# BEAMRobotics/beam_slam

Hardware: AMD Instinct MI355X
Metric: LM iterations/sec + ms/graph-solve, 200KF x 50k-landmark VIO window (higher is better)
Workload: dtype f64; 1 GPU; C2: 200-keyframe x 50000-landmark VIO window; n_obs=400690, n_imu_factors=199, solver_options=vio.yaml:7-17 (<= 10 iterations, tolerances 1.5e-7), max_solver_time lifted, parallelism=single GPU, n_ranks_seen=1

## Files before the change

beam_slam_amd/capi.py:

```python
import ctypes as C

import numpy as np

OK = 0
ERR_INVALID, ERR_DEVICE, ERR_UNSUPPORTED, ERR_NUMERIC = -1, -2, -3, -4

MANIFOLD_EUCLIDEAN, MANIFOLD_QUAT_RIGHT = 0, 1
LOSS_TRIVIAL, LOSS_CAUCHY, LOSS_HUBER = 0, 1, 2

F_REPROJ = 0
F_REPROJ_ONLINE_CALIB = 1
F_IMU_DELTA = 2
F_IMU_PRIOR = 3
F_RELPOSE_EXT = 4
F_RELPOSE = 5
F_ABSPOSE = 6
F_ABS_VEC3 = 7
F_REL_VEC3 = 8
F_GRAVITY = 9
F_IDP_REPROJ = 10
F_IDP_REPROJ_UNARY = 11
F_UNICYCLE = 12
F_NUM_TYPES = 13

LINEAR_AUTO, LINEAR_SCHUR_CHOLESKY, LINEAR_PCG, LINEAR_SCHUR_PCG = 0, 1, 2, 3
TR_LEVENBERG_MARQUARDT, TR_DOGLEG, TR_SUBSPACE_DOGLEG = 0, 1, 2
CONVERGENCE, NO_CONVERGENCE, FAILURE = 0, 1, 2


class Options(C.Structure):
    _fields_ = [
        ("max_num_iterations", C.c_int32),
        ("linear_solver_type", C.c_int32),
        ("jacobi_scaling", C.c_int32),
        ("max_num_consecutive_invalid_steps", C.c_int32),
        ("max_solver_time_in_seconds", C.c_double),
        ("function_tolerance", C.c_double),
        ("gradient_tolerance", C.c_double),
        ("parameter_tolerance", C.c_double),
        ("initial_trust_region_radius", C.c_double),
        ("max_trust_region_radius", C.c_double),
        ("min_trust_region_radius", C.c_double),
        ("min_relative_decrease", C.c_double),
        ("min_lm_diagonal", C.c_double),
        ("max_lm_diagonal", C.c_double),
        ("pcg_max_iterations", C.c_int32),
        ("trust_region_strategy_type", C.c_int32),
        ("pcg_tolerance", C.c_double),
    ]


class Summary(C.Structure):
    _fields_ = [
        ("termination_type", C.c_int32),
        ("is_solution_usable", C.c_int32),
        ("num_iterations", C.c_int32),
        ("num_successful_steps", C.c_int32),
        ("num_unsuccessful_steps", C.c_int32),
        ("num_parameters_tangent", C.c_int32),
        ("num_residuals", C.c_int32),
        ("linear_solver_used", C.c_int32),
        ("num_linear_solves", C.c_int32),
        ("num_inner_iterations", C.c_int32),
        ("initial_cost", C.c_double),
        ("final_cost", C.c_double),
        ("fixed_cost", C.c_double),
        ("total_time_in_seconds", C.c_double),
        ("device_time_in_seconds", C.c_double),
        ("time_eval_seconds", C.c_double),
        ("time_assemble_seconds", C.c_double),
        ("time_linear_solve_seconds", C.c_double),
        ("message", C.c_char * 160),
    ]


class Iteration(C.Structure):
    _fields_ = [
        ("iteration", C.c_int32),
        ("step_is_valid", C.c_int32),
        ("step_is_successful", C.c_int32),
        ("reserved0", C.c_int32),
        ("cost", C.c_double),
        ("cost_change", C.c_double),
        ("gradient_max_norm", C.c_double),
        ("gradient_norm", C.c_double),
        ("step_norm", C.c_double),
        ("relative_decrease", C.c_double),
        ("trust_region_radius", C.c_double),
        ("model_cost_change", C.c_double),
    ]


class Camera(C.Structure):
    _fields_ = [
        ("fx", C.c_double), ("fy", C.c_double), ("cx", C.c_double), ("cy", C.c_double),
        ("R_cam_baselink", C.c_double * 9),
        ("t_cam_baselink", C.c_double * 3),
    ]


SYMBOLS = [
    "nidx", "nconst", "nres", "options_default", "options_vio", "create", "create_error", "destroy",
    "last_error", "abi_version", "clear", "set_blocks", "set_values", "set_cameras", "add_factors", "add_factors_indirect", "sync_factors_indirect",
    "add_marginal",
    "finalize", "solve", "get_blocks", "reset_values", "num_iterations_recorded", "get_iteration",
    "evaluate", "num_residuals", "num_parameters_tangent", "tangent_offset", "covariance", "marginalize", "get_marginal",
    "reprojection_errors", "preintegrate", "triangulate", "time_reproj_jacobian_ms", "reproj_jacobian_bytes", "dense_solve", "plan_info",
    "profile_step", "time_eval_ms", "eval_bytes", "bsr_info", "covariance_joint", "update_marginal", "solve_batch", "batch_stats", "set_plan_preference",
    "covariance_requests", "localize_frames", "num_factorizations", "essential_ransac", "absolute_pose_ransac",
    "relative_pose_ransac", "inertial_alignment", "register_scans", "register_scans_error",
]

_dp = C.POINTER(C.c_double)
_ip = C.POINTER(C.c_int32)
_bp = C.POINTER(C.c_uint8)

RANSAC_OK, RANSAC_TOO_FEW, RANSAC_NO_MODEL = 0, 1, 2
RANSAC_MAX_MATCHES = 65536
ESSENTIAL_RANSAC_ARGTYPES = [C.c_void_p, C.c_int32, _ip, _dp, _dp, _dp, C.c_double, C.c_double, C.c_int32, C.c_uint64, _bp, _dp, _ip, _ip,
                             _ip, _ip]
ABSOLUTE_POSE_RANSAC_ARGTYPES = [C.c_void_p, C.c_int32, _ip, _dp, _dp, _ip, C.c_double, C.c_double, C.c_int32, C.c_uint64, C.c_int32, _bp,
                                 _dp, _dp, _dp, _ip, _ip, _ip, _ip]
RELATIVE_POSE_RANSAC_ARGTYPES = [C.c_void_p, C.c_int32, _ip, _dp, _dp, _ip, C.c_double, C.c_double, C.c_int32, C.c_uint64, C.c_int32,
                                 C.c_double, C.c_double, _bp, _dp, _dp, _dp, _dp, _bp, _dp, _ip, _ip, _ip, _ip, _ip]
ALIGN_OK, ALIGN_TOO_FEW_FRAMES, ALIGN_BAD_IMU, ALIGN_NOT_EXCITED, ALIGN_RANK_DEFICIENT, ALIGN_SCALE_REJECTED = 0, 1, 2, 3, 4, 5
ALIGN_MIN_EXCITATION, ALIGN_SCALE_MIN, ALIGN_SCALE_MAX, ALIGN_RANK_TOL = 0.25, 0.02, 1.0, 1e-10
INERTIAL_ALIGNMENT_ARGTYPES = [C.c_int, C.c_int32, _ip, _dp, _dp, _dp, _ip, _dp, _dp, _dp, C.c_int32, C.c_double, C.c_int32, C.c_double,
                               C.c_double, C.c_double, _dp, _dp, _dp, _dp, _ip, _dp, _dp, _dp, _dp, _ip]
ICP_MAX_ITERATIONS, ICP_TRANSFORM, ICP_ABS_MSE, ICP_REL_MSE, ICP_TOO_FEW_CORRESPONDENCES = 1, 2, 3, 4, 5
ICP_MAX_CELLS, ICP_MAX_ITER = 1 << 22, 1000
ICP_DEFAULTS = dict(max_corr=1.0, max_iter=50, t_eps=1e-8, fit_eps=1e-2, rotation_threshold=0.99999, rel_mse_eps=1e-5)
REGISTER_SCANS_ARGTYPES = [C.c_int, C.c_int32, _ip, _dp, _ip, _dp, _dp, C.c_double, C.c_int32, C.c_double, C.c_double, C.c_double,
                           C.c_double, _dp, _dp, _dp, _ip, _ip, _ip]


def _ptr(a, typ):
    return None if a is None else a.ctypes.data_as(typ)


class SolverError(RuntimeError):
    def __init__(self, code, msg):
        super().__init__(f"[{code}] {msg}")
        self.code = code


class Solver:

    def __init__(self, lib, prefix, device=0):
        self._lib, self._p = lib, prefix
        f = self._f
        f("create").restype = C.c_void_p
        f("create").argtypes = [C.c_int]
        f("destroy").argtypes = [C.c_void_p]
        f("last_error").restype = C.c_char_p
        f("last_error").argtypes = [C.c_void_p]
        f("set_blocks").argtypes = [C.c_void_p, C.c_int32, _dp, _ip, _bp, _bp, _bp]
        f("set_values").argtypes = [C.c_void_p, _dp, C.c_int64]
        f("set_cameras").argtypes = [C.c_void_p, C.c_int32, C.POINTER(Camera)]
        f("add_factors").argtypes = [C.c_void_p, C.c_int32, C.c_int32, _ip, _dp, _ip, _dp]
        f("add_marginal").argtypes = [C.c_void_p, C.c_int32, _ip, C.c_int32, _dp, _dp, _dp]
        f("marginalize").argtypes = [C.c_void_p, C.c_int32, _ip, _ip, _ip, _ip]
        f("get_marginal").argtypes = [C.c_void_p, _ip, _dp, _dp, _dp]
        f("finalize").argtypes = [C.c_void_p]
        f("clear").argtypes = [C.c_void_p]
        f("solve").argtypes = [C.c_void_p, C.POINTER(Options), C.POINTER(Summary)]
        f("get_blocks").argtypes = [C.c_void_p, _dp, C.c_int64]
        f("reset_values").argtypes = [C.c_void_p]
        f("num_iterations_recorded").argtypes = [C.c_void_p]
        f("get_iteration").argtypes = [C.c_void_p, C.c_int32, C.POINTER(Iteration)]
        f("evaluate").argtypes = [C.c_void_p, _dp, _dp, _dp, _dp]
        f("num_residuals").argtypes = [C.c_void_p]
        f("num_parameters_tangent").argtypes = [C.c_void_p]
        f("tangent_offset").argtypes = [C.c_void_p, C.c_int32]
        f("covariance").argtypes = [C.c_void_p, C.c_int32, C.c_int32, _dp]
        f("options_default").argtypes = [C.POINTER(Options)]
        f("options_vio").argtypes = [C.POINTER(Options)]
        self._ctx = f("create")(device)
        if not self._ctx:
            why = ""
            try:
                ce = f("create_error")
                ce.restype = C.c_char_p
                why = ce().decode()
            except AttributeError:
                pass
            raise SolverError(ERR_DEVICE, f"{prefix}create({device}) failed: {why}")
        self._nvalues = 0

    def _f(self, name):
        return getattr(self._lib, self._p + name)

    def has(self, name):
        return hasattr(self._lib, self._p + name)

    def _chk(self, rc):
        if rc != OK:
            raise SolverError(rc, self._f("last_error")(self._ctx).decode())

    def close(self):
        if getattr(self, "_ctx", None):
            self._f("destroy")(self._ctx)
            self._ctx = None

    def __del__(self):
        try:
            self.close()
        except Exception:
            pass

    def options_default(self):
        o = Options()
        self._f("options_default")(C.byref(o))
        return o

    def options_vio(self):
        o = Options()
        self._f("options_vio")(C.byref(o))
        return o

    def clear(self):
        self._chk(self._f("clear")(self._ctx))

    def set_blocks(self, values, offset, size, manifold, is_const):
        values = np.ascontiguousarray(values, np.float64)
        offset = np.ascontiguousarray(offset, np.int32)
        size = np.ascontiguousarray(size, np.uint8)
        manifold = np.ascontiguousarray(manifold, np.uint8)
        is_const = np.ascontiguousarray(is_const, np.uint8)
        self._nvalues = values.size
        self._chk(self._f("set_blocks")(self._ctx, offset.size, _ptr(values, _dp), _ptr(offset, _ip),
                                        _ptr(size, _bp), _ptr(manifold, _bp), _ptr(is_const, _bp)))

    def set_values(self, values):
        values = np.ascontiguousarray(values, np.float64)
        self._chk(self._f("set_values")(self._ctx, _ptr(values, _dp), values.size))

    def set_cameras(self, cams):
        arr = (Camera * len(cams))(*cams)
        self._chk(self._f("set_cameras")(self._ctx, len(cams), arr))

    def add_factors(self, ftype, block_idx, consts, loss_kind=None, loss_a=None):
        block_idx = np.ascontiguousarray(block_idx, np.int32)
        consts = np.ascontiguousarray(consts, np.float64)
        n = block_idx.shape[0] if block_idx.ndim == 2 else 0
        if loss_kind is not None:
            loss_kind = np.ascontiguousarray(np.broadcast_to(loss_kind, (n,)), np.int32)
        if loss_a is not None:
            loss_a = np.ascontiguousarray(np.broadcast_to(loss_a, (n,)), np.float64)
        self._chk(self._f("add_factors")(self._ctx, ftype, n, _ptr(block_idx, _ip), _ptr(consts, _dp),
                                         _ptr(loss_kind, _ip), _ptr(loss_a, _dp)))

    def add_factors_indirect(self, ftype, slot_idx, slot_to_block, consts, loss_kind=None, loss_a=None):
        slot_idx = np.ascontiguousarray(slot_idx, np.int32)
        slot_to_block = np.ascontiguousarray(slot_to_block, np.int32)
        consts = np.ascontiguousarray(consts, np.float64)
        n = slot_idx.shape[0] if slot_idx.ndim == 2 else 0
        if loss_kind is not None:
            loss_kind = np.ascontiguousarray(np.broadcast_to(loss_kind, (n,)), np.int32)
        if loss_a is not None:
            loss_a = np.ascontiguousarray(np.broadcast_to(loss_a, (n,)), np.float64)
        fn = self._f("add_factors_indirect")
        fn.argtypes = [C.c_void_p, C.c_int32, C.c_int32, _ip, C.c_int32, _ip, _dp, _ip, _dp]
        fn.restype = C.c_int
# ... 173 lines not shown
```

beam_slam_amd/csrc/bsgpu_api.cpp:

```cpp
#include <thread>

#include "bsgpu_ctx.h"
#include "bsgpu_env.h"

using namespace bsg;

namespace bsg {
int api_exception(bsgpu_ctx* c) noexcept {
  int code = BSGPU_ERR_INVALID;
  const char* what = "unexpected exception";
  try { throw; }
  catch (const std::bad_alloc&) { code = BSGPU_ERR_DEVICE; what = "out of host memory"; }
  catch (const std::exception& e) { what = e.what(); try { if (c) c->err = std::string("internal error: ") + what; } catch (...) {} return code; }
  catch (...) {}
  try { if (c) c->err = what; } catch (...) {}
  return code;
}
thread_local std::string g_create_error;
int invalidate_keep_values(bsgpu_ctx* c) {
  if (c->finalized && c->d_x && !c->h_x.empty()) {
    HIPCHK(c, hipSetDevice(c->device));
    HIPCHK(c, hipStreamSynchronize(c->stream));
    HIPCHK(c, hipMemcpy(c->h_x.data(), c->d_x, sizeof(double) * c->h_x.size(), hipMemcpyDeviceToHost));
  }
// ... 754 lines not shown

constexpr size_t kCovRowsBudget = (size_t)1 << 30;
int bsgpu_covariance_requests(bsgpu_ctx* c, int32_t n_req, const int32_t* pairs, int64_t* offsets, double* out) try {
  if (!c) return BSGPU_ERR_INVALID;
  if (n_req < 0 || (n_req > 0 && !pairs)) return fail(c, BSGPU_ERR_INVALID, "covariance_requests: bad argument");
  if (n_req == 0) { if (offsets) offsets[0] = 0; return BSGPU_OK; }
  int rc = finalize(c);
  if (rc != BSGPU_OK) return rc;
  for (int i = 0; i < 2 * n_req; ++i) {
    const int b = pairs[i];
    if (b < 0 || b >= c->nb) return fail(c, BSGPU_ERR_INVALID, "covariance_requests: block out of range");
    if (c->toff[b] < 0) return fail(c, BSGPU_ERR_INVALID, "covariance_requests: constant block");
    if (c->calib.on && c->is_lm[b])
      return fail(c, BSGPU_ERR_UNSUPPORTED, "covariance_requests: an eliminated landmark of a window with a free extrinsic pair (online calibration): "
                                            "pose-side blocks only");
  }
  std::vector<int64_t> off(n_req + 1, 0);
  for (int i = 0; i < n_req; ++i) off[i + 1] = off[i] + (int64_t)c->tsize[pairs[2 * i]] * c->tsize[pairs[2 * i + 1]];
  if (offsets) std::memcpy(offsets, off.data(), sizeof(int64_t) * off.size());
  if (!out) return BSGPU_OK;
  if (!c->dense_ok) return fail(c, BSGPU_ERR_UNSUPPORTED, "covariance_requests: reduced system above the dense limit (block-sparse PCG path has no factor)");
  const int n_pose = c->n_pose;
  auto kind_of = [&](int b) { return c->toff[b] < n_pose ? kCovUnit : (c->is_lm[b] == 2 ? kCovIdp : kCovLandmark); };
  auto lm_of = [&](int b) { return kind_of(b) == kCovIdp ? c->toff[b] - c->idp.to0 : (c->toff[b] - n_pose) / 3; };
  std::map<int, int> row_of;
  std::vector<CovRow> rows;
  std::vector<int> pass_entry{0}, pass_row{0};
  int n_rows = 0, in_pass = 0;
  for (int i = 0; i < 2 * n_req; ++i) {
    const int b = pairs[i];
    if (row_of.count(b)) continue;
    const int ts = c->tsize[b];
    if (in_pass + ts > 64) { pass_entry.push_back((int)rows.size()); pass_row.push_back(n_rows); in_pass = 0; }
    row_of[b] = n_rows;
    const int k = kind_of(b);
    if (k == kCovUnit) for (int r = 0; r < ts; ++r) rows.push_back(CovRow{kCovUnit, c->plan.spos(c->toff[b] + r), in_pass + r, 0});
    else rows.push_back(CovRow{k, lm_of(b), in_pass, 0});
    n_rows += ts; in_pass += ts;
  }
  pass_entry.push_back((int)rows.size()); pass_row.push_back(n_rows);
  const int n_pass = (int)pass_entry.size() - 1;
  const int ldy = c->npad, n_cols = c->plan.T * 64;
  if ((size_t)n_rows * ldy * sizeof(double) > kCovRowsBudget)
    return fail(c, BSGPU_ERR_UNSUPPORTED, "covariance_requests: the kept rows (" + std::to_string(n_rows) + " x " + std::to_string(ldy) +
                " doubles) exceed the 1 GiB device-memory budget of one call; split the requests");
  std::vector<CovReq> req(n_req);
  for (int i = 0; i < n_req; ++i) {
    const int a = pairs[2 * i], b = pairs[2 * i + 1];
    const int ka = kind_of(a), kb = kind_of(b);
    CovReq& q = req[i];
    q.ra = row_of[a]; q.ta = c->tsize[a]; q.rb = row_of[b]; q.tb = c->tsize[b];
    q.sign = ((ka != kCovUnit) != (kb != kCovUnit)) ? -1 : 1;
    q.lm_kind = (a == b && ka != kCovUnit) ? ka : kCovUnit;
    q.lm_index = q.lm_kind != kCovUnit ? lm_of(a) : 0;
    q.pad = 0;
    q.out = off[i];
  }
  HIPCHK(c, hipSetDevice(c->device));
  hipStream_t s = c->stream;
  const size_t y_bytes = (size_t)n_rows * ldy * sizeof(double), o_bytes = ((size_t)off[n_req] * sizeof(double) + 255) & ~(size_t)255;
  const size_t q_bytes = (sizeof(CovReq) * req.size() + 255) & ~(size_t)255, r_bytes = sizeof(CovRow) * rows.size();
  unsigned char* buf = nullptr;
  if (hipMalloc((void**)&buf, y_bytes + o_bytes + q_bytes + r_bytes) != hipSuccess) { (void)hipGetLastError(); return fail(c, BSGPU_ERR_DEVICE, "covariance_requests: out of device memory"); }
  struct Free { unsigned char* p; ~Free() { (void)hipFree(p); } } free_buf{buf};
  double* d_Y = reinterpret_cast<double*>(buf);
  double* d_out = reinterpret_cast<double*>(buf + y_bytes);
  CovReq* d_req = reinterpret_cast<CovReq*>(buf + y_bytes + o_bytes);
  CovRow* d_rows = reinterpret_cast<CovRow*>(buf + y_bytes + o_bytes + q_bytes);
  HIPCHK(c, hipMemcpyAsync(d_req, req.data(), sizeof(CovReq) * req.size(), hipMemcpyHostToDevice, s));
  HIPCHK(c, hipMemcpyAsync(d_rows, rows.data(), r_bytes, hipMemcpyHostToDevice, s));
  bsgpu_options o;
  bsgpu_options_default(&o);
  const bool was_pcg = c->use_pcg;
  c->use_pcg = false;
  *c->h_radius = 1e300;
  (void)hipMemcpyAsync(c->d_scal + SC_RADIUS, c->h_radius, sizeof(double), hipMemcpyHostToDevice, s);
  eval_all(c, c->d_x, true, SC_COST_X);
  c->spec_J = false;
  bool singular = false;
  for (int p = 0; p < n_pass && rc == BSGPU_OK && !singular; ++p) {
    const int n_ent = pass_entry[p + 1] - pass_entry[p], r0 = pass_row[p], nr = pass_row[p + 1] - r0;
    assemble(c, o, 1e300, true, true);
    for (int attempt = 0; attempt < 2; ++attempt) {
      launch_cov_rows(s, c->d_S, c->npad, c->plan.rhs_row, d_rows + pass_entry[p], n_ent, c->d_dpos, c->vis, c->idp);
      DenseDev D0{c->d_nreal, c->d_rows_flat, c->d_panels, c->d_Lp, c->d_Vinv,
                  c->d_bs_desc, c->d_chain_begin, c->d_chain_end, c->d_tile_sync, c->d_ftasks, c->d_fsync};
      D0.Winv = c->d_Winv; D0.tile_tot = c->d_tile_tot; D0.rhs_rows = nr;
      D0.ftasks_plain = c->d_ftasks_plain; D0.tile_tot_plain = c->d_tile_tot_plain; D0.n_ftasks_plain = c->n_ftasks_plain;
      dense_factor(s, c->plan, D0, c->d_S, c->d_scal);
      (void)hipMemcpyAsync(d_Y + (size_t)r0 * ldy, c->d_Lp + (size_t)c->plan.rhs_row * ldy, sizeof(double) * nr * ldy, hipMemcpyDeviceToDevice, s);
      rc = fetch_scalars(c);
      if (rc != BSGPU_OK || !(c->h_scal[SC_CHOL_FAIL] == 2.0 && c->d_ftasks)) break;
      c->d_ftasks = nullptr;
      assemble(c, o, 1e300, true, true);
    }
    if (rc == BSGPU_OK && c->h_scal[SC_CHOL_FAIL] > 0.0) singular = true;
  }
  c->use_pcg = was_pcg;
  if (rc != BSGPU_OK) return rc;
  if (singular) return fail(c, BSGPU_ERR_NUMERIC, "covariance_requests: J^T J is singular at the current values (gauge freedom or unobserved block)");
  launch_cov_gram(s, d_req, n_req, d_Y, ldy, n_cols, c->vis.Linv, c->idp.linv, d_out);
  HIPCHK(c, hipMemcpyAsync(out, d_out, sizeof(double) * off[n_req], hipMemcpyDeviceToHost, s));
  HIPCHK(c, hipStreamSynchronize(s));
  for (int64_t i = 0; i < off[n_req]; ++i)
    if (!std::isfinite(out[i])) return fail(c, BSGPU_ERR_NUMERIC, "covariance_requests: J^T J is singular at the current values (gauge freedom or unobserved block)");
  return BSGPU_OK;
} catch (...) { return api_exception(c); }

int bsgpu_update_marginal(bsgpu_ctx* c, int32_t index, int32_t n_rows, int32_t n_cols, int32_t n_xbar, const double* A, const double* b,
                          const double* xbar) try {
  if (!c) return BSGPU_ERR_INVALID;
  if (index < 0 || index >= (int)c->marginals.size() || !A || !b || !xbar) return fail(c, BSGPU_ERR_INVALID, "update_marginal: bad argument");
  HostMarginal& mg = c->marginals[index];
  if (n_rows != mg.rows || (size_t)n_rows * (size_t)std::max(0, n_cols) != mg.A.size() || (size_t)n_rows != mg.b.size() || (size_t)n_xbar != mg.xbar.size())
    return fail(c, BSGPU_ERR_INVALID, "update_marginal: the payload's shape is not that of the prior as it was added");
  std::memcpy(mg.A.data(), A, sizeof(double) * mg.A.size());
  std::memcpy(mg.b.data(), b, sizeof(double) * mg.b.size());
  std::memcpy(mg.xbar.data(), xbar, sizeof(double) * mg.xbar.size());
  if (!c->finalized) return BSGPU_OK;
  if (index >= (int)c->marg.size()) return fail(c, BSGPU_ERR_INVALID, "update_marginal: device table out of step");
  HIPCHK(c, hipSetDevice(c->device));
  const MargDev& d = c->marg[index].dev;
  HIPCHK(c, hipStreamSynchronize(c->stream));
  HIPCHK(c, hipMemcpy(const_cast<double*>(d.A), mg.A.data(), sizeof(double) * mg.A.size(), hipMemcpyHostToDevice));
  HIPCHK(c, hipMemcpy(const_cast<double*>(d.b), mg.b.data(), sizeof(double) * mg.b.size(), hipMemcpyHostToDevice));
  HIPCHK(c, hipMemcpy(const_cast<double*>(d.xbar), mg.xbar.data(), sizeof(double) * mg.xbar.size(), hipMemcpyHostToDevice));
  c->spec_J = false;
  return BSGPU_OK;
} catch (...) { return api_exception(c); }

int bsgpu_reprojection_errors(bsgpu_ctx* c, double* err) try {
  if (!c) return BSGPU_ERR_INVALID;
  if (!err) return fail(c, BSGPU_ERR_INVALID, "null argument");
  int rc = finalize(c);
  if (rc != BSGPU_OK) return rc;
  HIPCHK(c, hipSetDevice(c->device));
  const Visual& V = c->vis;
  if ((rc = ensure_vis_src(c)) != BSGPU_OK) return rc;
  const SmallGroup& D = c->small[T_REPROJ_DENSE];
  const int n0 = c->groups[BSGPU_F_REPROJ].n;
  if (V.n + D.n == 0) return BSGPU_OK;
  double* d_out = nullptr;
  HIPCHK(c, hipMalloc((void**)&d_out, sizeof(double) * (size_t)(V.n + D.n)));
  if (c->calib.on) launch_calib_refresh(c->stream, c->calib, c->d_x, c->d_cams);
  launch_reproj_errors(c->stream, V, D, c->d_x, c->d_cams, d_out, d_out + V.n);
  std::vector<double> h((size_t)V.n + D.n);
  const hipError_t e = hipMemcpyAsync(h.data(), d_out, sizeof(double) * h.size(), hipMemcpyDeviceToHost, c->stream);
  const hipError_t e2 = hipStreamSynchronize(c->stream);
  (void)hipFree(d_out);
  if (e != hipSuccess || e2 != hipSuccess) return fail(c, BSGPU_ERR_DEVICE, "reprojection_errors: device error");
  auto slot = [&](int src) { const int t = src >> 28, f = src & ((1 << 28) - 1); return (t == BSGPU_F_REPROJ ? 0 : n0) + f; };
  for (int i = 0; i < V.n; ++i) err[slot(c->vis_src[i])] = h[i];
  for (int i = 0; i < D.n; ++i) err[slot(c->dense_src[i])] = h[(size_t)V.n + i];
  return BSGPU_OK;
} catch (...) { return api_exception(c); }

double bsgpu_time_reproj_jacobian_ms(bsgpu_ctx* c, int32_t reps) {
  if (!c) return -1.0;
  if (finalize(c) != BSGPU_OK || c->vis.n == 0 || reps <= 0) return -1.0;
  if (hipSetDevice(c->device) != hipSuccess) return -1.0;
  hipEvent_t e0, e1;
  if (hipEventCreate(&e0) != hipSuccess || hipEventCreate(&e1) != hipSuccess) return -1.0;
  launch_reproj_jacobian_only(c->stream, c->vis, c->d_x, c->d_cams, c->d_losses);
  (void)hipEventRecord(e0, c->stream);
  for (int i = 0; i < reps; ++i) launch_reproj_jacobian_only(c->stream, c->vis, c->d_x, c->d_cams, c->d_losses);
  (void)hipEventRecord(e1, c->stream);
  if (hipEventSynchronize(e1) != hipSuccess) return -1.0;
  float ms = 0.f;
  (void)hipEventElapsedTime(&ms, e0, e1);
  (void)hipEventDestroy(e0); (void)hipEventDestroy(e1);
  return (double)ms / reps;
}
double bsgpu_time_eval_ms(bsgpu_ctx* c, int32_t reps) {
  if (!c) return -1.0;
  if (finalize(c) != BSGPU_OK || reps <= 0) return -1.0;
  if (hipSetDevice(c->device) != hipSuccess) return -1.0;
  hipEvent_t e0, e1;
  if (hipEventCreate(&e0) != hipSuccess || hipEventCreate(&e1) != hipSuccess) return -1.0;
  eval_all(c, c->d_x, true, SC_COST_X);
  (void)hipEventRecord(e0, c->stream);
  for (int i = 0; i < reps; ++i) eval_all(c, c->d_x, true, SC_COST_X);
  (void)hipEventRecord(e1, c->stream);
  if (hipEventSynchronize(e1) != hipSuccess) return -1.0;
  float ms = 0.f;
  (void)hipEventElapsedTime(&ms, e0, e1);
  (void)hipEventDestroy(e0); (void)hipEventDestroy(e1);
  c->spec_J = false;
  return (double)ms / reps;
}
int64_t bsgpu_eval_bytes(const bsgpu_ctx* c) {
  if (!c) return -1;
  static const struct { int idx, consts, res, jcols; } L[BSGPU_F_NUM_TYPES] = {
      {4, 3, 2, 9}, {6, 3, 2, 9}, {10, 287, 15, 30}, {5, 241, 15, 15}, {6, 43, 6, 12}, {4, 43, 6, 12}, {2, 43, 6, 6}, {1, 12, 3, 3},
      {2, 12, 3, 6}, {1, 7, 2, 3}, {6, 6, 2, 13}, {4, 6, 2, 7}, {10, 226, 15, 30}};
  int64_t b = (int64_t)c->vis.n * (c->vis.ja == kJACompact ? 152 : 200) + (int64_t)c->h_x.size() * 8;
  for (int t = 2; t < BSGPU_F_NUM_TYPES && t < kNumInternal; ++t)
    b += (int64_t)c->small[t].n * (4 * L[t].idx + 8 * (L[t].consts + L[t].res + L[t].res * L[t].jcols));
  return b;
}
int bsgpu_bsr_info(bsgpu_ctx* c, int32_t* block_rows, int32_t* nnz_blocks) try {
  if (!c) return BSGPU_ERR_INVALID;
  const int rc = finalize(c);
  if (rc != BSGPU_OK) return rc;
  if (block_rows) *block_rows = c->use_pcg ? c->nbr : 0;
  if (nnz_blocks) *nnz_blocks = c->use_pcg ? c->nblk : 0;
  return BSGPU_OK;
} catch (...) { return api_exception(c); }
int bsgpu_profile_step(bsgpu_ctx* c, const bsgpu_options* o, int32_t reps, double* ms_out, double* work_out) try {
  if (!c) return BSGPU_ERR_INVALID;
  if (!o || !ms_out || reps <= 0) return fail(c, BSGPU_ERR_INVALID, "profile_step: bad argument");
  return profile_step(c, *o, reps, ms_out, work_out);
} catch (...) { return api_exception(c); }
int64_t bsgpu_reproj_jacobian_bytes(const bsgpu_ctx* c) {
  if (!c) return -1;
  return (int64_t)c->vis.n * (c->vis.ja == kJACompact ? 152 : 200) + (int64_t)c->h_x.size() * 8;
}

int bsgpu_dense_solve(int device, int32_t n, const double* A, const double* b, double* x, int32_t max_chains, double* ms_out) try {
  if (n <= 0 || !A || !b || !x) return BSGPU_ERR_INVALID;
  if (hipSetDevice(device) != hipSuccess) return BSGPU_ERR_DEVICE;
  chol_prepare();
  const int T = (n + 63) / 64;
  std::vector<uint8_t> adj((size_t)T * T, 0);
  for (int i = 0; i < n; ++i) for (int j = 0; j < n; ++j) if (A[(size_t)i * n + j] != 0.0) adj[(size_t)(i / 64) * T + j / 64] = 1;
  DensePlan P;
  P.build(n, adj, std::max(1, (int)max_chains), 1, env_shared());
  const int npad = P.npad;
  std::vector<double> hS((size_t)npad * npad, 0.0);
  for (int i = 0; i < n; ++i) for (int j = 0; j < n; ++j) hS[(size_t)P.spos(i) * npad + P.spos(j)] = A[(size_t)i * n + j];
  for (int j = 0; j < n; ++j) hS[(size_t)P.rhs_row * npad + P.spos(j)] = b[j];
  std::vector<uint8_t> real(npad, 0);
  for (int j = 0; j < n; ++j) real[P.spos(j)] = 1;
  for (int i = 0; i < npad; ++i) if (!real[i]) hS[(size_t)i * npad + i] = 1.0;
  double *dS = nullptr, *dLp = nullptr, *dV = nullptr, *dy = nullptr, *dscal = nullptr;
  int *dnreal = nullptr, *drows = nullptr;
  PanelDesc *dpan = nullptr, *dsep = nullptr;
  int *dpot2 = nullptr, *dcb = nullptr, *dce = nullptr, *dsync = nullptr, *dfsync = nullptr, *dtot = nullptr;
  double* dW = nullptr;
  FusedTask* dft = nullptr;
  const bool fused = env_chol_fused() && !P.ftasks.empty();
  hipStream_t s;
  if (hipStreamCreate(&s) != hipSuccess) return BSGPU_ERR_DEVICE;
  auto up = [](const void* src, size_t bytes, void** dst) {
    if (hipMalloc(dst, bytes ? bytes : 8) != hipSuccess) return false;
    return bytes == 0 || hipMemcpy(*dst, src, bytes, hipMemcpyHostToDevice) == hipSuccess;
  };
  bool ok = hipMalloc(&dS, sizeof(double) * hS.size()) == hipSuccess && hipMalloc(&dLp, sizeof(double) * hS.size()) == hipSuccess && hipMemset(dLp, 0, sizeof(double) * hS.size()) == hipSuccess &&
            hipMalloc(&dV, sizeof(double) * chol_vinv_stride() * std::max(1, T)) == hipSuccess && hipMalloc(&dy, sizeof(double) * npad) == hipSuccess &&
            hipMalloc(&dscal, sizeof(double) * SC_NUM) == hipSuccess;
  std::vector<int> rf = P.rows_flat; if (rf.empty()) rf.push_back(0);
  ok = ok && up(P.nreal.data(), sizeof(int) * P.nreal.size(), (void**)&dnreal) &&
       up(rf.data(), sizeof(int) * rf.size(), (void**)&drows) &&
       up(P.panels.data(), sizeof(PanelDesc) * P.panels.size(), (void**)&dpan) &&
       up(P.bs_desc.data(), sizeof(int) * P.bs_desc.size(), (void**)&dpot2) &&
       up(P.chain_begin.data(), sizeof(int) * P.chain_begin.size(), (void**)&dcb) && up(P.chain_end.data(), sizeof(int) * P.chain_end.size(), (void**)&dce) &&
       up(P.tile_sync.data(), sizeof(int) * P.tile_sync.size(), (void**)&dsync);
  if (ok && fused) {
    const std::vector<int> zeros((size_t)P.fused_sync_words, 0);
    ok = up(P.ftasks.data(), sizeof(FusedTask) * P.ftasks.size(), (void**)&dft) && up(zeros.data(), sizeof(int) * zeros.size(), (void**)&dfsync) &&
         up(P.tile_tot.data(), sizeof(int) * P.tile_tot.size(), (void**)&dtot) && hipMalloc((void**)&dW, sizeof(double) * 4096 * std::max(1, T)) == hipSuccess;
  }
  int rc = BSGPU_OK;
  int *dbc = nullptr, *drc = nullptr, *dbu = nullptr, *dbur = nullptr;
  if (ok) {
    (void)hipMemcpy(dS, hS.data(), sizeof(double) * hS.size(), hipMemcpyHostToDevice);
    (void)hipMemset(dscal, 0, sizeof(double) * SC_NUM);
    hipEvent_t e0, e1;
    (void)hipEventCreate(&e0); (void)hipEventCreate(&e1);
    (void)hipEventRecord(e0, s);
    DenseDev D{dnreal, drows, dpan, dLp, dV, dpot2, dcb, dce, dsync, dft, dfsync};
    D.Winv = dW; D.tile_tot = dtot;
    if (P.bs_level_sync && !env_backsolve_legacy() &&
        up(P.bs_desc_chain.data(), sizeof(int) * P.bs_desc_chain.size(), (void**)&dbc) && up(P.rows_flat_chain.data(), sizeof(int) * P.rows_flat_chain.size(), (void**)&drc) &&
        up(P.bs_upd.data(), sizeof(int) * P.bs_upd.size(), (void**)&dbu) && up(P.bs_upd_rows.data(), sizeof(int) * P.bs_upd_rows.size(), (void**)&dbur)) {
      D.bs_desc_chain = dbc; D.rows_flat_chain = drc; D.bs_upd = dbu; D.bs_upd_rows = dbur;
    }
    dense_factor_solve(s, P, D, dS, dy, dscal);
    (void)hipEventRecord(e1, s);
    if (hipEventSynchronize(e1) != hipSuccess || hipGetLastError() != hipSuccess) rc = BSGPU_ERR_DEVICE;
    float ms = 0.f;
    (void)hipEventElapsedTime(&ms, e0, e1);
    if (ms_out) *ms_out = ms;
    double hscal[SC_NUM];
    std::vector<double> hy(npad);
    (void)hipMemcpy(hscal, dscal, sizeof(hscal), hipMemcpyDeviceToHost);
    (void)hipMemcpy(hy.data(), dy, sizeof(double) * npad, hipMemcpyDeviceToHost);
    for (int j = 0; j < n; ++j) x[j] = hy[P.spos(j)];
    if (rc == BSGPU_OK && hscal[SC_CHOL_FAIL] > 0.0) rc = BSGPU_ERR_NUMERIC;
    (void)hipEventDestroy(e0); (void)hipEventDestroy(e1);
  } else rc = BSGPU_ERR_DEVICE;
  (void)hipFree(dS); (void)hipFree(dLp); (void)hipFree(dV); (void)hipFree(dy); (void)hipFree(dscal);
  (void)hipFree(dnreal); (void)hipFree(drows); (void)hipFree(dpan);
  (void)hipFree(dsep); (void)hipFree(dpot2); (void)hipFree(dcb); (void)hipFree(dce); (void)hipFree(dsync);
  (void)hipFree(dft); (void)hipFree(dfsync); (void)hipFree(dtot); (void)hipFree(dW);
  (void)hipFree(dbc); (void)hipFree(drc); (void)hipFree(dbu); (void)hipFree(dbur);
  (void)hipStreamDestroy(s);
  return rc;
} catch (...) { return api_exception(nullptr); }

int bsgpu_plan_info(const bsgpu_ctx* c, int32_t* n_chains, int32_t* n_steps, int32_t* n_tiles) try {
  if (!c) return BSGPU_ERR_INVALID;
  if (!c->finalized) return BSGPU_ERR_INVALID;
  if (n_chains) *n_chains = c->plan.n_pieces;
  if (n_steps) *n_steps = c->plan.n_steps();
  if (n_tiles) *n_tiles = c->plan.T;
  return BSGPU_OK;
// ... 12 lines not shown
```

beam_slam_amd/csrc/bsgpu_finalize.cpp:

```cpp
#include <atomic>

#include "bsgpu_ctx.h"
#include "bsgpu_env.h"
#include "band_plan.h"
#include "dim_order.h"

namespace bsg {

int band_part_forced() {
  return env_int("BSGPU_BAND_PART", 0);
}

namespace {
void eigen_quat_to_rot(const double* q, double* R) {
  const double tx = 2 * q[1], ty = 2 * q[2], tz = 2 * q[3];
  const double twx = tx * q[0], twy = ty * q[0], twz = tz * q[0], txx = tx * q[1], txy = ty * q[1], txz = tz * q[1];
  const double tyy = ty * q[2], tyz = tz * q[2], tzz = tz * q[3];
  R[0] = 1 - (tyy + tzz); R[1] = txy - twz; R[2] = txz + twy;
  R[3] = txy + twz; R[4] = 1 - (txx + tzz); R[5] = tyz - twx;
  R[6] = txz - twy; R[7] = tyz + twx; R[8] = 1 - (txx + tyy);
}

}

// ... 326 lines not shown
      lap("count pair entries");
      const int chunk = pair_chunk(n_ent);
      for (uint64_t key = 0; key < ncp * ncp; ++key)
        for (int p0 = start[key]; p0 < start[key + 1]; p0 += chunk) { seg_ci.push_back((int)(key / ncp)); seg_cj.push_back((int)(key % ncp)); seg_start.push_back(p0); }
      std::vector<int> pos(start.begin(), start.end() - 1);
      for (int l = 0; l < nl; ++l) {
        if (b_cmin[l] >= 0) continue;
        for (int a = lm_start[l]; a < lm_start[l + 1]; ++a) {
          const uint64_t ra = (uint64_t)cam_pose[a] * ncp;
          for (int b = lm_start[l]; b < lm_start[l + 1]; ++b)
            if (cam_pose[a] <= cam_pose[b]) { const int p = pos[ra + cam_pose[b]]++; ent_fa[p] = a; ent_fb[p] = b; }
        }
      }
      for (int f = n_elim; f < nv; ++f) { const int p = pos[(uint64_t)cam_pose[f] * ncp + cam_pose[f]]++; ent_fa[p] = f; ent_fb[p] = f; }
      lap("fill pair entries");
    } else {
      struct Ent { uint64_t key; int fa, fb; };
      std::vector<Ent> ents;
      ents.reserve((size_t)nv * 5);
      for (int l = 0; l < nl; ++l) {
        if (b_cmin[l] >= 0) continue;
        for (int a = lm_start[l]; a < lm_start[l + 1]; ++a)
          for (int b = lm_start[l]; b < lm_start[l + 1]; ++b)
            if (cam_pose[a] <= cam_pose[b]) ents.push_back({(uint64_t)cam_pose[a] * ncp + cam_pose[b], a, b});
      }
      for (int f = n_elim; f < nv; ++f) ents.push_back({(uint64_t)cam_pose[f] * ncp + cam_pose[f], f, f});
      std::stable_sort(ents.begin(), ents.end(), [](const Ent& x, const Ent& y) { return x.key < y.key; });
      ent_fa.resize(ents.size()); ent_fb.resize(ents.size());
      const int chunk = pair_chunk(ents.size());
      for (size_t i = 0; i < ents.size(); ++i) {
        if (i == 0 || ents[i].key != ents[i - 1].key || (int)i - seg_start.back() >= chunk) {
          seg_ci.push_back((int)(ents[i].key / ncp)); seg_cj.push_back((int)(ents[i].key % ncp)); seg_start.push_back((int)i);
        }
        ent_fa[i] = ents[i].fa; ent_fb[i] = ents[i].fb;
      }
      lap("sort pair entries");
    }
    seg_start.push_back((int)ent_fa.size());
    V.n_seg = (int)seg_ci.size(); V.n_ent = (int)ent_fa.size();
    V.n_seg_c = 0; V.seg_ci_c = V.seg_cj_c = V.seg_start_c = nullptr;
    lap("segments");
    V.fac = c->upload(fac); V.pix = c->upload(pix); V.w = c->upload(w);
    V.cam_pose = c->upload(cam_pose); V.lm_of = c->upload(lm_of); V.lm_start = c->upload(lm_start);
    V.cp_tq = c->upload(cp_tq); V.cp_tp = c->upload(cp_tp);
    V.seg_ci = c->upload(seg_ci); V.seg_cj = c->upload(seg_cj); V.seg_start = c->upload(seg_start);
    V.ent_fa = c->upload(ent_fa); V.ent_fb = c->upload(ent_fb);
    V.band_lm = c->upload(b_lm); V.band_unit_start = c->upload(bu.unit_start); V.band_unit_cam = c->upload(bu.unit_cam);
    V.band_lm_id = c->upload(bu.lm);
    const int T = (c->n_pose + 63) / 64;
    c->tile_adj.assign((size_t)T * T, 0);
    auto touch = [&](int ra, int rb) {
      if (ra < 0 || rb < 0) return;
      for (int a = ra; a < ra + 3; a += 2) for (int b = rb; b < rb + 3; b += 2) {
        c->tile_adj[(size_t)(a / 64) * T + b / 64] = 1; c->tile_adj[(size_t)(b / 64) * T + a / 64] = 1;
      }
      if (bg.nbk) bg.add(ra, rb);
    };
    for (int s = 0; s < V.n_seg; ++s) {
      const int i = seg_ci[s], j = seg_cj[s];
      const int ri[2] = {cp_tq[i], cp_tp[i]}, rj[2] = {cp_tq[j], cp_tp[j]};
      for (int a = 0; a < 2; ++a) for (int b = 0; b < 2; ++b) touch(ri[a], rj[b]);
    }
    for (int i = 0; i < V.n_cam_pose && V.n_band_lm > 0; ++i)
      for (int d = 0; d < kBandCams; ++d) {
        if (!((bu.adj[i] >> d) & 1u)) continue;
        const int j = i + d;
        const int ri[2] = {cp_tq[i], cp_tp[i]}, rj[2] = {cp_tq[j], cp_tp[j]};
        for (int a = 0; a < 2; ++a) for (int b = 0; b < 2; ++b) touch(ri[a], rj[b]);
      }
    if (has_calib) {
      Calib& cb = c->calib;
      cb.on = 1;
      cb.xq = c->off[calib_bq]; cb.xp = c->off[calib_bp];
      cb.tq = c->toff[calib_bq]; cb.tp = c->toff[calib_bp];
      cb.n_cam = (int)calib_cams.size();
      cb.cam_id = c->upload(calib_cams);
      std::vector<unsigned char> has(std::max(1, nv), 0);
      for (int i = 0; i < nv; ++i) has[i] = vf[i].calib ? 1 : 0;
      cb.has = c->upload(has);
      std::vector<int> cnt(k + 1, 0), by_cp(nv);
      for (int i = 0; i < nv; ++i) cnt[cam_pose[i] + 1]++;
      for (int i = 0; i < k; ++i) cnt[i + 1] += cnt[i];
      {
        std::vector<int> pos(cnt.begin(), cnt.end() - 1);
        for (int i = 0; i < nv; ++i) by_cp[pos[cam_pose[i]]++] = i;
      }
      std::vector<int> sg_cp, sg_start;
      for (int i = 0; i < k; ++i)
        for (int p0 = cnt[i]; p0 < cnt[i + 1]; p0 += 256) { sg_cp.push_back(i); sg_start.push_back(p0); }
      sg_start.push_back(nv);
      cb.n_seg = (int)sg_cp.size();
      cb.seg_cp = c->upload(sg_cp); cb.seg_start = c->upload(sg_start); cb.seg_fac = c->upload(by_cp);
      const int re[2] = {cb.tq, cb.tp};
      for (int a = 0; a < 2; ++a) {
        for (int b = 0; b < 2; ++b) touch(re[a], re[b]);
        for (int i = 0; i < k; ++i) { touch(cp_tq[i], re[a]); touch(cp_tp[i], re[a]); }
      }
    }
  }
    return BSGPU_OK;
  };
  bool flattened_on_device = false;
  {
    const bool force_dev = env_flatten_is("device"), force_host = env_flatten_is("host");
    const HostGroup& g0 = c->groups[BSGPU_F_REPROJ];
    SlotMirror& mir = c->mirror0;
    const bool resident = mir.active && !mir.materialized && mir.dev_valid;
    if (!force_host && c->groups[BSGPU_F_REPROJ_ONLINE_CALIB].n == 0 && g0.n > 0 && (force_dev || g0.n >= kDeviceFlattenMin)) {
      bool ok = true;
      if (mir.active && !mir.materialized && !resident) { const int rc_m = materialize_mirror(c); if (rc_m != BSGPU_OK) return rc_m; }
      if (resident) { for (const auto& u : mir.loss_use) if (u.rows > 0 && ok) { get_loss(u.kind, u.a); ok = losses.size() <= 8; } }
      else for (int f = 0; f < g0.n && ok; ++f) { get_loss(g0.loss_kind[f], g0.loss_a[f]); ok = losses.size() <= 8; }
      if (ok) {
        std::vector<int> bx(c->off.begin(), c->off.end());
        std::vector<unsigned char> bc(c->is_const.begin(), c->is_const.end());
        const int* d_bx = c->upload(bx); const int* d_bt = c->upload(c->toff);
        const unsigned char* d_bc = c->upload(bc); const int* d_bl = c->upload(lm_index);
        const int T = (c->n_pose + 63) / 64;
        bool all_const = false;
        FlattenSegsHost segs_host;
        auto dalloc = [&](size_t bytes) -> void* { return c->alloc<unsigned char>(bytes); };
        const FlattenResident res = {mir.d_idx, mir.d_consts, mir.d_lk, mir.d_la, mir.d_s2b};
        const int st = flatten_visual_device(c->stream, dalloc, g0.n, g0.idx.data(), g0.consts.data(), g0.loss_kind.data(), g0.loss_a.data(),
                                             losses, nb, d_bx, d_bt, d_bc, d_bl, nl, T, c->vis, &c->d_vis_src, c->tile_adj, &all_const,
                                             resident ? &res : nullptr, bg.nbk ? &segs_host : nullptr, band_on);
        if (st < 0) return fail(c, BSGPU_ERR_DEVICE, "device error while flattening the reprojection factors");
        if (st == 0) {
          flattened_on_device = true;
          if (bg.nbk)
            for (size_t sgi = 0; sgi < segs_host.seg_ci.size(); ++sgi) {
              const int i = segs_host.seg_ci[sgi], j = segs_host.seg_cj[sgi];
              const int ri[2] = {segs_host.cp_tq[i], segs_host.cp_tp[i]}, rj[2] = {segs_host.cp_tq[j], segs_host.cp_tp[j]};
              for (int a = 0; a < 2; ++a) for (int b = 0; b < 2; ++b) if (ri[a] >= 0 && rj[b] >= 0) bg.add(ri[a], rj[b]);
            }
          if (all_const) { c->any_inactive = true; c->vis_any_inactive = true; }
          if (c->vis.n_cam_pose >= (1 << 20)) return fail(c, BSGPU_ERR_UNSUPPORTED, "too many camera poses");
        } else {
          c->vis = Visual();
        }
      }
    }
  }
  if (flattened_on_device) lap("flatten on device");
  else { const int rc_host = host_visual(); if (rc_host != BSGPU_OK) return rc_host; }
  Visual& V = c->vis;
  {
    const int nv = V.n;
    V.r = c->alloc<double2>(nv); V.J = c->alloc<double>((size_t)nv * (kJAStride + 6)); V.JB = V.J ? V.J + (size_t)nv * kJAStride : nullptr; V.CR = c->alloc<double>((size_t)nv * 8);
    V.Linv = c->alloc<double>((size_t)std::max(1, nl) * kLmRec); V.z = V.Linv ? V.Linv + 6 : nullptr;
    V.n_cost_part = (nv + 255) / 256;
    V.cost_part = c->alloc<double>(V.n_cost_part);
    V.cost_part_cand = c->alloc<double>(V.n_cost_part);
    V.mcc_part = c->alloc<double>(std::max(1, backsub_mcc_groups(V)));
    if (!V.J || !V.CR || !V.r) return fail(c, BSGPU_ERR_DEVICE, "out of device memory (visual tables)");
    if (c->calib.on) {
      c->calib.E = c->alloc<double>((size_t)std::max(1, nv) * 12); c->calib.Et = c->alloc<double>((size_t)std::max(1, nv) * 12);
      c->calib.part = c->alloc<double>((size_t)std::max(1, calib_border_blocks(V)) * kCalibPartStride);
      if (!c->calib.E || !c->calib.Et || !c->calib.part) return fail(c, BSGPU_ERR_DEVICE, "out of device memory (extrinsic border tables)");
    }
    V.no_cr = !env_zero("BSGPU_NO_CR") && V.n_band_units > 0 && V.n_seg == 0 && V.n_ent == 0 && V.n == V.n_elim && V.band_lm_id != nullptr && V.Linv && V.z;
    V.ja = V.no_cr && !env_zero("BSGPU_COMPACT_J") ? kJACompact : kJAStride;
  }
  lap("visual upload + alloc");
  size_t part_max = std::max<size_t>(V.n_cost_part, 2 * ((size_t)nb + 255) / 256 + 2);
  int* d_toff_asm[kNumInternal] = {nullptr};
  for (int t = 2; t < kNumInternal; ++t) {
    const HostGroup& g = c->groups[t];
    const TypeInfo& ti = kTypes[t];
    SmallGroup& sg = c->small[t];
    sg = SmallGroup();
    sg.type = t; sg.n = g.n; sg.m = ti.m; sg.nv = ti.nvar; sg.nc = ti.nconst;
    sg.w_last = ti.amb[ti.nvar - 1] == 4 ? 3 : ti.amb[ti.nvar - 1];
    if (!g.n) continue;
    std::vector<int> xoff((size_t)g.n * ti.nvar), toff((size_t)g.n * ti.nvar), loss(g.n);
    std::vector<unsigned char> active(g.n, 0), inactive(g.n, 0);
    for (int f = 0; f < g.n; ++f) {
      const int32_t* idx = &g.idx[(size_t)f * ti.nidx];
      for (int sl = 0; sl < ti.nvar; ++sl) {
        xoff[(size_t)f * ti.nvar + sl] = c->off[idx[sl]];
        toff[(size_t)f * ti.nvar + sl] = c->toff[idx[sl]];
        if (c->toff[idx[sl]] >= c->n_pose && !(c->is_lm[idx[sl]] == 2 && sl == ti.nvar - 1 && (t == BSGPU_F_IDP_REPROJ || t == BSGPU_F_IDP_REPROJ_UNARY)))
          return fail(c, BSGPU_ERR_UNSUPPORTED, "internal: landmark in a pose-only factor");
        if (!c->is_const[idx[sl]]) active[f] = 1;
      }
      inactive[f] = !active[f];
      if (!active[f]) c->any_inactive = true;
      loss[f] = get_loss(g.loss_kind[f], g.loss_a[f]);
      if (active[f] && !skip_generic_assembly(t)) {
        const int T = (c->n_pose + 63) / 64;
        for (int sa = 0; sa < ti.nvar; ++sa)
          for (int sb = 0; sb < ti.nvar; ++sb) {
            const int ra = c->toff[idx[sa]], rb = c->toff[idx[sb]];
            if (ra < 0 || rb < 0 || ra >= c->n_pose || rb >= c->n_pose) continue;
            const int wa = c->tsize[idx[sa]], wb = c->tsize[idx[sb]];
            for (int a = ra; a < ra + wa; a += std::max(1, wa - 1)) for (int b = rb; b < rb + wb; b += std::max(1, wb - 1)) c->tile_adj[(size_t)(a / 64) * T + b / 64] = 1;
            if (bg.nbk && sb < sa) bg.add(ra, rb);
          }
      }
    }
    if (timing && g.n > 10000) lap("  group: per-factor loop");
    sg.xoff = c->upload(xoff); sg.toff = c->upload(toff); sg.consts = c->upload(g.consts); sg.loss = c->upload(loss);
    d_toff_asm[t] = nullptr;
    if (n_rho > 0 && (t == BSGPU_F_IDP_REPROJ || t == BSGPU_F_IDP_REPROJ_UNARY)) {
      std::vector<int> tm(toff);
      bool any = false;
      for (int& v : tm) if (v >= c->n_pose) { v = -1; any = true; }
      if (any) d_toff_asm[t] = c->upload(tm);
    }
    sg.active = c->upload(active);
    if (has_camera(t)) {
      std::vector<int> camv(g.n);
      for (int f = 0; f < g.n; ++f) camv[f] = g.idx[(size_t)f * ti.nidx + ti.nvar];
      sg.cam = c->upload(camv);
    }
    c->d_small_inactive[t] = c->upload(inactive);
    c->h_small_active[t] = active;
    if (timing && g.n > 10000) lap("  group: uploads");
    sg.r = c->alloc<double>((size_t)g.n * ti.m);
    sg.J = c->alloc<double>((size_t)g.n * ti.m * 3 * ti.nvar);
    c->d_small_part[t] = c->alloc<double>((size_t)g.n * ti.m);
    c->d_small_part_cand[t] = c->alloc<double>(g.n);
    c->d_small_part_mcc[t] = c->alloc<double>((size_t)g.n * ti.m);
    part_max = std::max(part_max, (size_t)g.n * ti.m);
    if (timing && g.n > 10000) lap("  group: allocations");
  }
  lap("pose-only group tables");
  {
    constexpr int kSegChunk = 64;
    struct Contrib { int ra, rb, tf, ss; };
    std::vector<Contrib> cl, tmp;
    std::vector<int> cnt;
    std::vector<AsmGroup> asm_grp;
    size_t asm_nfac = 0;
    auto sort_by_block = [&](size_t lo, size_t hi) {
      const size_t n = hi - lo;
      if (n < 2) return;
      tmp.resize(n);
      for (int pass = 0; pass < 2; ++pass) {
        cnt.assign((size_t)c->n_pose + 2, 0);
        for (size_t i = lo; i < hi; ++i) cnt[(pass == 0 ? cl[i].rb : cl[i].ra) + 1]++;
        for (size_t k = 1; k < cnt.size(); ++k) cnt[k] += cnt[k - 1];
        for (size_t i = lo; i < hi; ++i) tmp[cnt[pass == 0 ? cl[i].rb : cl[i].ra]++] = cl[i];
        std::copy(tmp.begin(), tmp.begin() + n, cl.begin() + lo);
      }
    };
    for (int t = 0; t < kNumInternal; ++t) {
      c->small_factorwise[t] = c->small[t];
      if (t < 2) c->small_factorwise[t].n = 0;
      if (d_toff_asm[t]) c->small_factorwise[t].toff = d_toff_asm[t];
      if (skip_generic_assembly(t)) c->small_factorwise[t].n = 0;
    }
    for (int t = 2; t < kNumInternal; ++t) {
      const SmallGroup& sg = c->small[t];
      if (!sg.n || skip_generic_assembly(t)) continue;
      const int nv = sg.nv;
      std::vector<int> toffs((size_t)sg.n * nv);
      HIPCHK(c, hipStreamSynchronize(c->stream));
      HIPCHK(c, hipMemcpy(toffs.data(), sg.toff, sizeof(int) * toffs.size(), hipMemcpyDeviceToHost));
      for (int& v : toffs) if (v >= c->n_pose) v = -1;
      std::vector<uint8_t> grouped(sg.n, 0);
      bool any_group = false;
      constexpr int kGroupMin = 4;
      if (sg.w_last == 3 && nv * 3 <= 18 && sg.m <= 6 && (sg.m * nv * 3) % 2 == 0 && sg.n >= 64 && !env_set("BSGPU_NO_GROUP_ASSEMBLY")) {
        std::vector<int> order;
        order.reserve(sg.n);
        for (int f = 0; f < sg.n; ++f) if (c->h_small_active[t][f]) order.push_back(f);
        auto key_less = [&](int a, int b) {
          const int* ka = &toffs[(size_t)a * nv]; const int* kb = &toffs[(size_t)b * nv];
          for (int i = 0; i < nv; ++i) if (ka[i] != kb[i]) return ka[i] < kb[i];
          return a < b;
        };
        std::sort(order.begin(), order.end(), key_less);
        for (size_t i = 0; i < order.size();) {
          size_t j = i + 1;
          while (j < order.size() && std::equal(&toffs[(size_t)order[i] * nv], &toffs[(size_t)order[i] * nv] + nv, &toffs[(size_t)order[j] * nv])) ++j;
          if ((int)(j - i) >= kGroupMin) {
            const size_t n_in = j - i, pieces = (n_in + kAsmGroupMax - 1) / kAsmGroupMax;
            size_t q0 = i;
            for (size_t pc = 0; pc < pieces; ++pc) {
              AsmGroup rec{};
              rec.type = t; rec.count = (int)(n_in / pieces + (pc < n_in % pieces ? 1 : 0)); rec.m = sg.m; rec.nv = nv;
              rec.te = 0;
              for (int sl = 0; sl < 6; ++sl) {
                rec.toff[sl] = sl < nv ? toffs[(size_t)order[i] * nv + sl] : -1;
                if (rec.toff[sl] >= 0) rec.te = 3 * (sl + 1);
              }
              rec.J = sg.J; rec.r = sg.r;
              for (int q = 0; q < kAsmGroupMax; ++q) rec.fac[q] = order[q0 + std::min(q, rec.count - 1)];
              asm_grp.push_back(rec);
              q0 += rec.count;
            }
            for (size_t q = i; q < j; ++q) grouped[order[q]] = 1;
            asm_nfac += j - i;
            any_group = true;
          }
          i = j;
        }
      }
      const size_t first = cl.size();
      for (int f = 0; f < sg.n; ++f) {
        if (!c->h_small_active[t][f] || grouped[f]) continue;
        for (int sa = 0; sa < nv; ++sa) for (int sb = 0; sb < nv; ++sb) {
          const int ra = toffs[(size_t)f * nv + sa], rb = toffs[(size_t)f * nv + sb];
          if (ra < 0 || rb < 0) continue;
          if (ra < rb) continue;
          cl.push_back({ra, rb, (t << 24) | f, (sa << 8) | sb});
        }
// ... 719 lines not shown
```

beam_slam_amd/csrc/bsgpu_internal.h:

```cpp
#pragma once
#include <hip/hip_runtime.h>
#include <stdint.h>

#include <functional>
#include <cstring>
#include <vector>

#include "dense_plan.h"

struct bsgpu_options;

namespace bsg {

struct DevCamera {
  double fx, fy, cx, cy;
  double R[9];
  double t[3];
};
struct DevLoss {
  int kind;
  int pad;
  double a;
};

constexpr int kJAStride = 12;
constexpr int kJACompact = 6;

constexpr int kPairChunk = 256;
inline int pair_chunk(size_t n_ent) { return n_ent <= 100000 ? 64 : n_ent <= 1000000 ? 128 : kPairChunk; }
constexpr int kBandCams = 13;
constexpr int kBandMinFactors = 150000;

constexpr int kMetaCamBits = 12, kMetaLossBits = 12;
constexpr int kLmRec = 10;
constexpr int kFlagQConst = 1, kFlagPConst = 2, kFlagLConst = 4;
__host__ __device__ inline int meta_pack(int cam, int loss, int flags) {
  return cam | (loss << kMetaCamBits) | (flags << (kMetaCamBits + kMetaLossBits));
}

enum {
  SC_COST_X = 0,
  SC_COST_CAND = 1,
  SC_MCC = 2,
  SC_STEP_NORM2 = 3,
  SC_X_NORM2 = 4,
  SC_GRAD_MAX = 5,
  SC_GRAD_NORM2 = 6,
  SC_CHOL_FAIL = 7,
  SC_FIXED_COST = 8,
  SC_CHOL_FAIL_SEEN = 9,
  SC_RADIUS = 12,
  SC_DEC_GO = 13,
  SC_DEC_RADIUS = 14,
  SC_SEQ = 15,
  SC_NUM = 16
};

struct SmallGroup {
  int type = 0, n = 0, m = 0, nv = 0, nc = 0;
  int* xoff = nullptr;
  int* toff = nullptr;
  double* consts = nullptr;
  int* loss = nullptr;
  unsigned char* active = nullptr;
  double* r = nullptr;
  double* J = nullptr;
  int w_last = 3;
  int* cam = nullptr;
  const DevCamera* cams = nullptr;
};

constexpr int kSetMax = 4;
struct SmallGroupSet {
  SmallGroup g[kSetMax];
  double* part[kSetMax];
  int first[kSetMax + 1];
  int n;
};

struct MargDev {
  int rows = 0, cols = 0, nblk = 0;
  const int* blk_xoff = nullptr;
  const int* blk_size = nullptr;
  const int* blk_quat = nullptr;
  const int* blk_col = nullptr;
  const int* blk_amb = nullptr;
  const int* col_t = nullptr;
  const int* col_blk = nullptr;
  const double* A = nullptr;
  const double* b = nullptr;
  const double* xbar = nullptr;
  double* delta = nullptr;
  double* D = nullptr;
  double* r = nullptr;
  double* J = nullptr;
};

struct Visual {
  int n = 0;
  int n_elim = 0;
  int n_lm = 0;
  int4* fac = nullptr;
  double2* pix = nullptr;
  double* w = nullptr;
  int* cam_pose = nullptr;
  int* lm_of = nullptr;
  int* lm_start = nullptr;
  int n_cam_pose = 0;
  int* cp_tq = nullptr;
  int* cp_tp = nullptr;
  int n_seg = 0, n_ent = 0;
  int* seg_ci = nullptr; int* seg_cj = nullptr; int* seg_start = nullptr;
  int* ent_fa = nullptr; int* ent_fb = nullptr;
  int n_seg_c = 0;
  int* seg_ci_c = nullptr; int* seg_cj_c = nullptr; int* seg_start_c = nullptr;
  int n_band_units = 0, n_band_lm = 0;
  int* band_unit_start = nullptr; int* band_unit_cam = nullptr; int4* band_lm = nullptr;
  int* band_lm_id = nullptr;
  bool no_cr = false;
  int ja = kJAStride;
  double2* r = nullptr;
  double* J = nullptr;
  double* JB = nullptr;
  double* CR = nullptr;
  double* Linv = nullptr;
  double* z = nullptr;
  double* cost_part = nullptr;
  double* cost_part_cand = nullptr;
  double* mcc_part = nullptr;
  int n_cost_part = 0;
};

constexpr int kCalibPartStride = 40;
struct Calib {
  int on = 0;
  int xq = 0, xp = 0;
  int tq = -1, tp = -1;
  int n_cam = 0;
  const int* cam_id = nullptr;
  const unsigned char* has = nullptr;
  double* E = nullptr;
  double* Et = nullptr;
  double* part = nullptr;
  int n_seg = 0;
  const int* seg_cp = nullptr; const int* seg_start = nullptr; const int* seg_fac = nullptr;
};
void launch_calib_refresh(hipStream_t s, const Calib& cb, const double* x, DevCamera* cams);
void launch_calib_E(hipStream_t s, const Visual& v, const Calib& cb, const double* x, const DevCamera* cams, const DevLoss* losses);
int calib_border_blocks(const Visual& v);
void launch_calib_border(hipStream_t s, const Visual& v, const Calib& cb, double* S, int ld, int rhs_row, double* grad, double* hdiag, const int* perm,
                         bool grad_only);
void launch_calib_backsub_mcc(hipStream_t s, const Visual& v, const Calib& cb, int n_pose, const double* y_pose, double* delta, double* mcc_part);

struct IdpElim {
  int n_lm = 0;
  int to0 = 0;
  int n_fac = 0;
  int n_view = 0;
  int* order = nullptr;
  int* lm_start = nullptr;
  int* view_start = nullptr;
  int2* fview = nullptr;
  int* view_lm = nullptr;
  int* view_cp = nullptr;
  int* view_code = nullptr;
  int direct = 0;
  int n_cam_pose = 0;
  int* cp_tq = nullptr;
  int* cp_tp = nullptr;
  int n_seg = 0, n_ent = 0;
  int* seg_ci = nullptr; int* seg_cj = nullptr; int* seg_start = nullptr;
  int* ent_va = nullptr; int* ent_vb = nullptr; int* ent_code = nullptr;
  double* U = nullptr;
  double* VD = nullptr;
  double* linv = nullptr;
  double* z = nullptr;
  double* C = nullptr;
};
void launch_idp_landmark(hipStream_t s, const IdpElim& e, const SmallGroup& g, const double* radius_ptr, double radius_val, int compute_scale,
                         int compute_dcl, int jacobi, double lm_lo, double lm_hi, double* scale, double* dcl, double* grad);
void launch_idp_pairs(hipStream_t s, const IdpElim& e, const SmallGroup& g, double* S, int ld, int rhs_row, double* grad, double* hdiag,
                      const int* perm, bool grad_only);
void launch_idp_backsub(hipStream_t s, const IdpElim& e, const double* y_pose, double* delta);

struct UpdateRide {
  int n_blocks = 0;
  const int* blocks = nullptr;
  const int* xoff = nullptr; const int* toff = nullptr; const unsigned char* size = nullptr; const unsigned char* manifold = nullptr;
  const int* lm_xoff = nullptr;
  const double* x = nullptr; double* x_cand = nullptr;
  double* part = nullptr;
};
struct ReduceEntry {
  const double* ptr;
  int n, stride, offset, slot;
  int op = 0;
};

struct LmDecide {
  int on = 0;
  int check_grad = 0;
  int x_from_scal = 0;
  double radius = 0.0, x_cost = 0.0;
  double min_relative_decrease = 0.0, max_radius = 0.0, function_tolerance = 0.0, parameter_tolerance = 0.0, gradient_tolerance = 0.0;
};
constexpr int kDecSlots = 256, kDecStride = 520;
struct GoWord { const double* p = nullptr; };

struct ReduceRide {
  const ReduceEntry* entries = nullptr;
  int n_entries = 0, n_slots = 0;
  double* scal = nullptr; double* host_scal = nullptr; int* counter = nullptr;
  double seq = 0.0;
  int skip_slot = -1;
  int defer_slot = -1;
  int only_slot = -1;
  ReduceEntry early[4];
  int n_early = 0;
  double* dec = nullptr;
  double* dec_next = nullptr;
  LmDecide lmd;
};

struct LaunchCtx {
  hipStream_t stream;
};

void launch_reproj_eval(hipStream_t s, const Visual& v, const double* x, const DevCamera* cams,
                        const DevLoss* losses, bool with_J, double* cost_part_out, bool count_inactive = false);
void launch_visual_imu_eval(hipStream_t s, const Visual& v, const SmallGroup& delta, const SmallGroup& prior, const double* x, const DevCamera* cams,
                            const DevLoss* losses, bool with_J, double* cost_part_vis, double* part_delta, double* part_prior,
                            const ReduceRide* red = nullptr );
void launch_relpose_imu_eval(hipStream_t s, const SmallGroup& g, const SmallGroup& delta, const SmallGroup& prior, const double* x,
                             const DevLoss* losses, bool with_J, double* cost_part, double* part_delta, double* part_prior, const ReduceRide* red = nullptr);
void launch_imu_eval(hipStream_t s, const SmallGroup& delta, const SmallGroup& prior, const double* x, const DevLoss* losses, bool with_J,
                     double* part_delta, double* part_prior);
int small_cost_parts(const SmallGroup& g);
void launch_small_eval(hipStream_t s, const SmallGroup& g, const double* x, const DevLoss* losses, bool with_J,
                       double* cost_part );
bool launch_small_eval_set(hipStream_t s, const SmallGroup* groups, double* const* parts, int n_groups, const double* x, const DevLoss* losses, bool with_J);
bool launch_small_eval_set_marg(hipStream_t s, const SmallGroup* groups, double* const* parts, int n_groups, const double* x, const DevLoss* losses, bool with_J,
                                const MargDev& m, double* marg_part);
constexpr int kBatchMaxWin = 64;
enum { BL_ALL = 0, BL_FULL = 1, BL_ACC = 2, BL_REJ = 3, BL_BS_FUSED = 4 , BL_BS_CHAIN = 6 , BL_DIAG = 8 , BL_CLEAR = 9 , BL_NUM = 10 };
struct BatchDyn {
  int n[BL_NUM];
  int idx[BL_NUM][kBatchMaxWin];
  double radius[kBatchMaxWin];
  double seq[kBatchMaxWin];
  int first[kBatchMaxWin], new_J[kBatchMaxWin], grad_only[kBatchMaxWin];
};
struct LmDiag {
  const double* hdiag = nullptr;
  double* scale = nullptr; double* dcl = nullptr;
  const int* inat = nullptr;
  double inv_radius = 0.0, lm_lo = 0.0, lm_hi = 0.0;
  int compute_scale = 0, compute_dcl = 0, jacobi = 0;
};
struct GradNormRide {
  int nb = 0;
  const int* xoff = nullptr; const int* toff = nullptr; const unsigned char* size = nullptr; const unsigned char* manifold = nullptr;
  const double* x = nullptr; const double* grad = nullptr; double* gpart = nullptr;
};
struct DenseDev {
  const int *nreal, *rows_flat;
  const PanelDesc* panels;
  double *Lp, *Vinv;
  const int *bs_desc, *chain_begin, *chain_end;
  int* tile_sync;
  const FusedTask* ftasks = nullptr;
  int* fsync = nullptr;
  const int *bs_desc_chain = nullptr, *rows_flat_chain = nullptr, *bs_upd = nullptr, *bs_upd_rows = nullptr;
  const int *bs_chain_group = nullptr, *bs_grp_nchains = nullptr, *bs_grp_nitems = nullptr, *bs_items4 = nullptr, *bs_tile_updated = nullptr;
  int* bs_sync = nullptr;
  double* scal = nullptr;
  double* Winv = nullptr;
  const int* bs_order = nullptr;
  const int* tile_tot = nullptr;
  int rhs_rows = 0;
  LmDiag diag;
  GradNormRide gn;
  const FusedTask* ftasks_plain = nullptr; const int* tile_tot_plain = nullptr; int n_ftasks_plain = 0;
};
struct BatchArgTable {
  std::vector<unsigned char> host;
  size_t stride = 0, lds = 0;
  int max_grid = 0;
  void* dev = nullptr;
  template <class A> void push(const A& a) {
    stride = sizeof(A);
    const size_t o = host.size();
    host.resize(o + sizeof(A));
    std::memcpy(&host[o], &a, sizeof(A));
    if (a.bsg_grid > max_grid) max_grid = a.bsg_grid;
  }
};
struct ZeroStep {
  double* S = nullptr; int ld = 0; const int* tiles = nullptr; int n_tiles = 0;
  double* a = nullptr; int na = 0; double* b = nullptr; int nb = 0; double* c = nullptr; int nc = 0;
  double* radius_slot = nullptr; double radius = 0.0;
};
struct Visual; struct SmallGroup; struct SmallGroupSet; struct UpdateRide; struct ReduceEntry; struct DevCamera; struct DevLoss;
void batchargs_visual_imu_eval(BatchArgTable& t, const Visual& v, const SmallGroup& delta, const SmallGroup& prior, const double* x, const DevCamera* cams,
                               const DevLoss* losses, double* cost_part_vis, double* part_delta, double* part_prior);
void launch_visual_imu_eval_batch(hipStream_t s, const BatchArgTable& t, const BatchDyn* dyn, int list, int n, bool with_J);
void batchargs_landmark(BatchArgTable& t, BatchArgTable& t_tail, const Visual& v, int n_pose, int jacobi, double lm_lo, double lm_hi, double* scale, double* dcl,
                        double* grad, const ZeroStep& zero);
void launch_landmark_batch(hipStream_t s, const BatchArgTable& t, const BatchArgTable& t_tail, const BatchDyn* dyn, int list, int n);
void batchargs_pairs(BatchArgTable& t, const Visual& v, double* S, int ld, int rhs_row, double* grad, double* hdiag, const int* perm, const SmallGroupSet* small,
                     int n_small_units);
void launch_pairs_batch(hipStream_t s, const BatchArgTable& t, const BatchDyn* dyn, int list, int n);
void batchargs_pairs_band(BatchArgTable& t, const Visual& v, double* S, int ld, int rhs_row, double* grad, double* hdiag, const int* perm, const SmallGroupSet* small,
                          int n_small_units);
void launch_pairs_band_batch(hipStream_t s, const BatchArgTable& t, const BatchDyn* dyn, int list, int n);
void batchargs_backsub_mcc(BatchArgTable& t, const Visual& v, int n_pose, const double* y_pose, double* delta, double* mcc_part, const SmallGroupSet* small,
                           int n_small_units, const UpdateRide* upd);
void launch_backsub_mcc_batch(hipStream_t s, const BatchArgTable& t, const BatchDyn* dyn, int list, int n);
void batchargs_grad_norms_pose_diag(BatchArgTable& t, int nb, const int* blk_xoff, const int* blk_toff, const unsigned char* blk_size,
                                    const unsigned char* blk_manifold, const double* x, const double* grad, double* gpart, int n_pose, double* S, int ld,
                                    const double* hdiag, int jacobi, double lm_lo, double lm_hi, double* scale, double* dcl, int npad, const int* iperm);
void launch_grad_norms_pose_diag_batch(hipStream_t s, const BatchArgTable& t, const BatchDyn* dyn, int list, int n);
void batchargs_final_reduce(BatchArgTable& t, const ReduceEntry* entries, int n_entries, int n_slots, double* scal, double* host_scal, int* counter);
void launch_final_reduce_batch(hipStream_t s, const BatchArgTable& t, const BatchDyn* dyn, int list, int n);
void batchargs_copy(BatchArgTable& t, const double* src, double* dst, int64_t n);
void launch_copy_batch(hipStream_t s, const BatchArgTable& t, const BatchDyn* dyn, int list, int n);
void batchargs_chol_fused(BatchArgTable& t, double* S, double* Lp, int ld, const FusedTask* tasks_dev, int n_tasks, const int* tile_tot_dev, const int* nreal_dev,
                          double* Vinv, double* scal, int* sync_dev, double* Winv, int rhs_rows, const LmDiag& diag, const GradNormRide& gn, bool diag_tasks_in_list);
void launch_chol_fused_batch(hipStream_t s, const BatchArgTable& t, const BatchDyn* dyn, int list, int n);
struct AsmGroup;
void batchargs_relpose_imu_eval(BatchArgTable& t, const SmallGroup* g, const SmallGroup& delta, const SmallGroup& prior, const double* x, const DevLoss* losses,
                                double* cost_part, double* part_delta, double* part_prior);
void launch_relpose_imu_eval_batch(hipStream_t s, const BatchArgTable& t, const BatchDyn* dyn, int list, int n, bool with_J);
bool batchargs_small_eval_set(BatchArgTable& t, const SmallGroup* groups, double* const* parts, int n_groups, const double* x, const DevLoss* losses);
void launch_small_eval_set_batch(hipStream_t s, const BatchArgTable& t, const BatchDyn* dyn, int list, int n, bool with_J);
void batchargs_unicycle_eval(BatchArgTable& t, const SmallGroup& g, const double* x, const DevLoss* losses, double* part);
void launch_unicycle_eval_batch(hipStream_t s, const BatchArgTable& t, const BatchDyn* dyn, int list, int n, bool with_J);
bool batchargs_small_assemble_set(BatchArgTable& t, const SmallGroup* groups, int n_groups, double* S, int ld, int rhs_row, double* grad, double* hdiag, const int* perm);
void launch_small_assemble_set_batch(hipStream_t s, const BatchArgTable& t, const BatchDyn* dyn, int list, int n);
void batchargs_small_assemble_seg(BatchArgTable& t, const SmallGroup* groups_dev, int n_seg, const int* seg_start, const int* seg_ra, const int* seg_rb, const int2* contrib,
                                  double* S, int ld, int rhs_row, double* grad, double* hdiag, const int* perm, const SmallGroupSet* fw, int n_fw_units, int n_grp,
                                  const AsmGroup* grp);
void launch_small_assemble_seg_batch(hipStream_t s, const BatchArgTable& t, const BatchDyn* dyn, int list, int n);
bool batchargs_small_mcc(BatchArgTable& t, const SmallGroup* groups, double* const* parts, int n_groups, const double* delta, const UpdateRide* upd, const ZeroStep* zero);
void launch_small_mcc_batch(hipStream_t s, const BatchArgTable& t, const BatchDyn* dyn, int list, int n);
void batchargs_zero_tiles_multi(BatchArgTable& t, const ZeroStep* zs);
void launch_zero_tiles_multi_batch(hipStream_t s, const BatchArgTable& t, const BatchDyn* dyn, int list, int n);
struct MargDev;
bool batchargs_marg_eval(BatchArgTable& t, const MargDev* m, const double* x, double* cost_part);
void launch_marg_eval_batch(hipStream_t s, const BatchArgTable& t, const BatchDyn* dyn, int list, int n, bool with_J);
void batchargs_marg_assemble(BatchArgTable& t, const MargDev* m, double* S, int ld, int rhs_row, double* grad, double* hdiag, const int* perm);
void launch_marg_assemble_batch(hipStream_t s, const BatchArgTable& t, const BatchDyn* dyn, int list, int n);
void batchargs_marg_mcc(BatchArgTable& t, const MargDev* m, const double* delta_tan, double* part);
void launch_marg_mcc_batch(hipStream_t s, const BatchArgTable& t, const BatchDyn* dyn, int list, int n);
struct IdpElim;
void batchargs_idp_landmark(BatchArgTable& t, BatchArgTable& t_view, const IdpElim& e, const SmallGroup& g, int jacobi, double lm_lo, double lm_hi, double* scale, double* dcl, double* grad);
void launch_idp_landmark_batch(hipStream_t s, const BatchArgTable& t, const BatchArgTable& t_view, const BatchDyn* dyn, int list, int n);
void batchargs_idp_pairs(BatchArgTable& t, const IdpElim& e, const SmallGroup& g, double* S, int ld, int rhs_row, double* grad, double* hdiag, const int* perm);
void launch_idp_pairs_batch(hipStream_t s, const BatchArgTable& t, const BatchDyn* dyn, int list, int n);
void batchargs_idp_backsub(BatchArgTable& t, const IdpElim& e, const double* y_pose, double* delta);
void launch_idp_backsub_batch(hipStream_t s, const BatchArgTable& t, const BatchDyn* dyn, int list, int n);
int batchargs_backsolve(BatchArgTable* tabs, const DensePlan& P, const DenseDev& D, double* y, const int* iperm, int n_pose, double* y_tan, double* delta);
void launch_backsolve_batch(hipStream_t s, const BatchArgTable* tabs, const BatchDyn* dyn, const int* n_in_form);
void launch_landmark(hipStream_t s, const Visual& v, int n_pose, const double* radius_ptr, int compute_scale,
                     int compute_dcl, int jacobi, double lm_lo, double lm_hi, double* scale, double* dcl,
                     double* grad, const ZeroStep* zero = nullptr, double radius_val = 0.0, const ReduceRide* red = nullptr );
void launch_pairs(hipStream_t s, const Visual& v, double* S, int ld, int rhs_row, double* grad, double* hdiag, const int* perm,
                  bool grad_only, const SmallGroupSet* small = nullptr, int n_small_units = 0, GoWord go = GoWord());
bool band_available();
void launch_pairs_band(hipStream_t s, const Visual& v, double* S, int ld, int rhs_row, double* grad, double* hdiag, const int* perm,
                       bool grad_only, const SmallGroupSet* small = nullptr, int n_small_units = 0, bool lower_only = false ,
                       GoWord go = GoWord());
int small_assemble_first_set(const SmallGroup* groups, int n_groups, SmallGroupSet* set, int* n_taken);
void launch_small_assemble_set(hipStream_t s, const SmallGroup* groups, int n_groups, double* S, int ld, int rhs_row, double* grad,
                               double* hdiag, const int* perm);
constexpr int kAsmGroupMax = 24;
struct AsmGroup {
  int type, count, m, nv;
  int toff[6];
  int te;
  int pad;
  const double* J;
  const double* r;
  int fac[kAsmGroupMax];
};
bool launch_small_assemble_seg(hipStream_t s, const SmallGroup* groups_dev, int n_seg, const int* seg_start, const int* seg_ra, const int* seg_rb,
                               const int2* contrib, double* S, int ld, int rhs_row, double* grad, double* hdiag, const int* perm,
                               const SmallGroupSet* fw = nullptr, int n_fw_units = 0, int n_grp = 0, const AsmGroup* grp = nullptr,
                               const MargDev* marg = nullptr, const ReduceRide* red = nullptr ,
                               bool* red_carried = nullptr);
void launch_pose_diag(hipStream_t s, int n_pose, double* S, int ld, const double* hdiag, const double* radius_ptr,
                      int compute_scale, int compute_dcl, int jacobi, double lm_lo, double lm_hi, double* scale,
                      double* dcl, int npad, const int* iperm, double radius_val = 0.0 );
void launch_grad_norms(hipStream_t s, int nb, const int* blk_xoff, const int* blk_toff, const unsigned char* blk_size,
                       const unsigned char* blk_manifold, const double* x, const double* grad, double* gpart );
void launch_grad_norms_pose_diag(hipStream_t s, int nb, const int* blk_xoff, const int* blk_toff, const unsigned char* blk_size,
                                 const unsigned char* blk_manifold, const double* x, const double* grad, double* gpart, int n_pose, double* S,
                                 int ld, const double* hdiag, const double* radius_ptr, int compute_scale, int compute_dcl, int jacobi,
                                 double lm_lo, double lm_hi, double* scale, double* dcl, int npad, const int* iperm, double radius_val = 0.0);
struct PanelDesc;
struct FusedTask;
void launch_chol_fused(hipStream_t s, double* S, double* Lp, int ld, const FusedTask* tasks_dev, int n_tasks, const int* tile_tot_dev, const int* nreal_dev,
                       double* Vinv, double* scal, int* sync_dev, double* Winv, int rhs_rows ,
                       const LmDiag& diag = LmDiag(), const GradNormRide& gn = GradNormRide(),
                       bool diag_tasks_in_list = false );
void launch_chol_potrf_tiles(hipStream_t s, double* S, double* Lp, int ld, const int* tiles_dev, int n_tiles, const int* nreal_dev,
                             double* Vinv, double* scal);
void launch_chol_panel_step(hipStream_t s, double* S, double* Lp, int ld, const PanelDesc* descs_dev, int n_panels, int max_rows,
                            const int* rows_flat_dev, const int* nreal_dev, double* Vinv, double* scal, int* tile_sync_dev,
                            const PanelDesc* descs_host = nullptr, const int* rows_flat_host = nullptr);
void launch_chol_backsolve_chains(hipStream_t s, const double* S, const double* Lp, const double* Vinv, int ld,
                                  const int* bs_desc_dev, const int* chain_begin_dev,
                                  const int* chain_end_dev, int n_chains, const int* rows_flat_dev, double* y,
                                  int npad, int max_chain_len, const double* y_init = nullptr, const int* iperm_dev = nullptr, int n_pose = 0,
                                  double* y_tan = nullptr, double* delta = nullptr, int max_rows = 0, const double* Winv = nullptr);
void launch_chol_backsolve_update(hipStream_t s, const double* Lp, int ld, const int* items_dev, int n_items, const int* upd_rows_dev, double* y);
bool launch_chol_backsolve_fused(hipStream_t s, const double* Lp, const double* Winv, int ld, const int* bs_desc_dev, const int* chain_begin_dev,
                                 const int* chain_end_dev, const int* rows_flat_dev, int n_chains, const int* chain_group_dev,
                                 const int* grp_nchains_dev, const int* grp_nitems_dev, int G, const int* items_dev, int n_items,
                                 const int* upd_rows_dev, const int* tile_updated_dev, double* y, int npad, int max_chain_len, int max_rows,
                                 const double* y_init, const int* iperm_dev, int n_pose, double* y_tan, double* delta, int* sync_dev, double* scal,
                                 const int* order_dev);
size_t chol_backsolve_chain_lds(int npad, int max_chain_len);
void launch_marg_schur(hipStream_t s, const double* S, int ld, int rhs_row, const int* spos_dev, int n, int m, double rel_tol,
                       double* M, double* g, double* diag0, int* pivot_ok, double* status, double* A, double* b);
void launch_cov_units(hipStream_t s, double* S, int ld, int rhs_row, const int* cols_dev, int n);
void launch_cov_dots(hipStream_t s, const double* Lp, int ld, int rhs_row, int n_cols, int ta, int row_b0, int tb, double* out);
enum CovRowKind { kCovUnit = 0, kCovLandmark = 1, kCovIdp = 2 };
struct CovRow {
  int kind;
  int index;
  int row;
  int pad;
};
struct CovReq {
  int ra, ta, rb, tb;
  int sign;
  int lm_kind;
  int lm_index;
  int pad;
  int64_t out;
};
void launch_cov_rows(hipStream_t s, double* S, int ld, int rhs_row, const CovRow* rows, int n_rows, const int* dpos, const Visual& v, const IdpElim& e);
void launch_cov_gram(hipStream_t s, const CovReq* req, int n_req, const double* Y, int ldy, int n_cols, const double* lm_linv, const double* idp_linv,
                     double* out);
void launch_marg_eval(hipStream_t s, const MargDev& m, const double* x, bool with_J, double* cost_part );
void launch_marg_assemble(hipStream_t s, const MargDev& m, double* S, int ld, int rhs_row, double* grad, double* hdiag, const int* perm);
void launch_marg_mcc(hipStream_t s, const MargDev& m, const double* delta_tan, double* part );
void launch_reproj_errors(hipStream_t s, const Visual& v, const SmallGroup& dense, const double* x, const DevCamera* cams, double* out_vis,
                          double* out_dense);
void launch_preintegrate(hipStream_t s, int n_int, const int* sample_start, const double* ts, const double* wm, const double* am,
                         const double* t_end, const double* bg, const double* ba, const double* covs, double info_weight, double* out);
void launch_inertial_alignment(hipStream_t s, int n_paths, const int* frame_start, const double* t_frame, const double* q_frame,
                               const double* p_frame, const int* imu_range, const double* t, const double* w, const double* a,
                               int bridge_gap, double min_excitation, int apply_scale, double scale_min, double scale_max, double rank_tol,
                               double* gravity, double* bg, double* scale, double* excitation, int* gyro_rank, double* velocity,
                               double* q_out, double* p_out, double* v_out, int* status, int* own, double* fs, double* ps);
struct IcpGrid; struct IcpParams;
constexpr int kIcpScanTile = 1024;
void launch_register_scans(hipStream_t s, int n_pairs, int max_targets, int n_targets, int max_chunks, int n_tiles, const int* ref_start,
                           const double* ref, const int* tgt_start, const double* tgt, const double* T_init, const int* chunk_start,
                           const IcpGrid* grids, double max_corr, const IcpParams& P, double* T, double* T_ref_tgt, double* mse, int* n_corr,
                           int* n_iters, int* status, double* tq, int* tcell, int* cells, int* tile_sum, double* rec, double* part,
                           double* mse_prev, int* done);
void launch_triangulate(hipStream_t s, int n_tracks, const int* track_start, const int2* pose_off, const double2* pix, const double* x,
                        const DevCamera& cam, bool truncate, double max_dist, double max_reproj, double* points, int* status);
constexpr int kLocOutStride = 45;
void launch_localize(hipStream_t s, int n_frames, const int* obs_start, const double2* pix, const double* pts, const int* pt_off,
                     const double* x, const DevCamera* cams, const int* cam_of, const double* pose_in, int loss_kind, double loss_a,
                     double sqrt_info, int truncate, int min_points, int width, int height, const bsgpu_options& opt, double* out,
                     int* out_i);
constexpr int kRansacOutInts = 8;
void launch_essential_ransac(hipStream_t s, int n_sets, const int* match_start, const double2* px_prev, const double2* px_cur,
                             const double* K, double prob, double threshold_px, int max_iters, uint64_t seed, unsigned char* mask,
                             double* out_E, int* out_i);
constexpr int kP3pOutDoubles = 19;
constexpr int kP3pOutInts = 6;
void launch_absolute_pose_ransac(hipStream_t s, int n_frames, const int* obs_start, const double2* pix, const double* pts,
                                 const DevCamera* cams, const int* cam_of, double prob, double threshold_px, int max_iters, uint64_t seed,
                                 int truncate, unsigned char* mask, double* out_d, int* out_i);
constexpr int kRelposeOutDoubles = 27;
constexpr int kRelposeOutInts = 11;
void launch_relative_pose_ransac(hipStream_t s, int n_sets, const int* match_start, const double2* pix_first, const double2* pix_last,
                                 const DevCamera* cams, const int* cam_of, double prob, double threshold_px, int max_iters, uint64_t seed,
                                 int truncate, double validate_px, double min_inlier_ratio, unsigned char* mask, unsigned char* valid_mask,
                                 double* points, double* out_d, int* out_i);
struct FlattenResident { const int* idx; const double* consts; const int* loss_kind; const double* loss_a; const int* slot_map; };
struct FlattenSegsHost { std::vector<int> seg_ci, seg_cj, cp_tq, cp_tp; };
void launch_patch_factor_rows(hipStream_t s, int n_ch, const int* rows, const int* idx4, const double* consts3, const int* lk, const double* la,
                              int* dst_idx, double* dst_consts, int* dst_lk, double* dst_la);
int flatten_visual_device(hipStream_t s, const std::function<void*(size_t)>& dalloc, int n, const int* h_idx, const double* h_consts,
                          const int* h_loss_kind, const double* h_loss_a, const std::vector<DevLoss>& losses, int nb, const int* d_blk_xoff,
                          const int* d_blk_toff, const unsigned char* d_blk_const, const int* d_blk_lm, int nl, int T, Visual& V,
                          int** d_vis_src, std::vector<unsigned char>& tile_adj, bool* any_all_const, const FlattenResident* res = nullptr,
                          FlattenSegsHost* segs_out = nullptr, bool band_enabled = true);
int chol_vinv_stride();
void chol_prepare();
void launch_bsr_assemble(hipStream_t s, const SmallGroup& g, const int* slots, double* val);
void launch_bsr_assemble_seg(hipStream_t s, const SmallGroup* groups_dev, int n_seg, const int* seg_start, const int* seg_slot, const int* seg_row,
                             const int2* contrib, double* val, double* rhs, double* grad, double* hdiag);
void launch_bsr_finish_diag(hipStream_t s, int nbr, const int* diag_slot, const int* pair_slot, double* val, const double* hdiag, double radius,
                            int compute_scale, int compute_dcl, int jacobi, double lm_lo, double lm_hi, double* scale,
                            double* dcl, double* Minv);
int pcg_spmv_grid(int nbr);
struct PcgPersistDev {
  int G = 0, max_cols = 0;
  int paired = 0;
  const int *wg_row = nullptr, *wg_colptr = nullptr, *wg_cols = nullptr, *lcol = nullptr;
  unsigned long long* slots = nullptr;
  int* abort_w = nullptr;
  double* zg = nullptr;
  size_t sync_bytes = 0;
  int n_coarse = 0;
  const int4* co = nullptr;
  double centre[3] = {0.0, 0.0, 0.0};
  double *W = nullptr, *E = nullptr, *Einv = nullptr;
  unsigned* counter = nullptr;
};
size_t pcg_coarse_scratch_doubles(int nbr);
void launch_pcg_coarse(hipStream_t s, const PcgPersistDev& P, int nbr, const int* row_ptr, const int* col, const double* val, const double* x);
size_t pcg_persistent_lds(int max_cols);
size_t pcg_persistent_lds_limit();
int pcg_persistent_max_rows();
size_t pcg_persistent_slot_words(int G);
size_t pcg_persistent_z_words(int nbr);
bool launch_pcg_persistent(hipStream_t s, const PcgPersistDev& P, int nbr, const int* row_ptr, const double* val, const double* Minv, const double* b,
                           double* x, double* zg, double* sc, double tol2, int max_it);
void launch_pcg_init(hipStream_t s, int nbr, const double* b, const double* Minv, double* x, double* r, double* z, double* p0, double* p1,
                     double* part, double* sc);
void launch_pcg_iteration(hipStream_t s, int k, int nbr, const int* row_ptr, const int* col, const double* val, const double* Minv,
                          double* x, double* r, double* z, double* p0, double* p1, double* q, double* part_pq, double* part, double* sc,
                          double tol2);
int pcg_num_scalars();
int pcg_rows_grid(int nbr);
void launch_spcg_prepare(hipStream_t s, int T, const double* S, int ld, double* Minv);
void launch_spcg_init(hipStream_t s, int T, const double* b, const double* Minv, double* x, double* r, double* z, double* p0, double* p1,
                      double* part, double* sc);
void launch_spcg_iteration(hipStream_t s, int k, int T, const double* S, int ld, int n_chunks, const int* chunk_row, const int* chunk_ptr,
                           const int* row_chunk_ptr, const int* tcol, const double* Minv, double* x, double* r, double* z, double* p0,
                           double* p1, double* qpart, double* part_pq, double* part, double* sc, double tol2);
int spcg_chunk_tiles();
void launch_spcg_finish(hipStream_t s, int T, const double* x, const int* iperm, int n_pose, double* y_tan, double* delta);
int pcg_done_slot();
int pcg_iters_slot();
int backsub_mcc_groups(const Visual& v);
bool launch_backsub_mcc(hipStream_t s, const Visual& v, int n_pose, const double* y_pose, double* delta, double* mcc_part,
                        const SmallGroupSet* small = nullptr, int n_small_units = 0, const UpdateRide* upd = nullptr, const MargDev* marg = nullptr,
                        double* marg_part = nullptr);
int small_mcc_first_set(const SmallGroup* groups, double* const* parts, int n_groups, SmallGroupSet* set, int* n_taken);
void launch_negate_pose(hipStream_t s, int n_pose, const double* y, double* delta);
void launch_update_ride_only(hipStream_t s, const double* delta, const UpdateRide& upd);
bool launch_small_mcc_set(hipStream_t s, const SmallGroup* groups, double* const* parts, int n_groups, const double* delta, const UpdateRide* upd = nullptr,
                          const ZeroStep* zero = nullptr );
void launch_update(hipStream_t s, int nb, const int* blk_xoff, const int* blk_toff, const unsigned char* blk_size,
                   const unsigned char* blk_manifold, const double* x, const double* delta, double* x_cand,
                   double* part , int* n_part);
void launch_sum(hipStream_t s, const double* part, int n, double* out, int accumulate);
void launch_zero(hipStream_t s, double* p, int64_t n);
void launch_dl_vec(hipStream_t s, int n_tan, const double* g, const double* dcl, const double* delta_gn, double* v, double* gn_keep, double* part,
                   double* out3 );
void launch_dl_step(hipStream_t s, int n_tan, const double* v, const double* gn, double a, double b, const double* dcl, double* delta, double* part,
                    double* out1 );
int dl_jv_records(const Visual& vis, const SmallGroup* small, int n_small, const MargDev* marg, int n_marg);
void launch_dl_jv(hipStream_t s, const Visual& vis, int n_pose, const SmallGroup* small, int n_small, const MargDev* marg, int n_marg, const double* u,
                  double* part, double* out2 );
void launch_dl_sum(hipStream_t s, const double* part, int n, int k, double* out);
void launch_zero4(hipStream_t s, double* p0, int64_t n0, double* p1, int64_t n1, double* p2, int64_t n2, double* p3, int64_t n3);
void launch_zero_tiles_multi(hipStream_t s, double* S, int ld, const int* tiles_dev, int n_tiles, double* a, int na, double* b, int nb, double* c,
                             int nc, double* radius_slot, double radius);
void launch_copy(hipStream_t s, const double* src, double* dst, int64_t n, int nzero_after);
void launch_final_reduce(hipStream_t s, const ReduceEntry* entries, int n_entries, int n_slots, double* scal, double* host_scal,
                         int* counter = nullptr, double seq = 0.0);

void launch_reproj_jacobian_only(hipStream_t s, const Visual& v, const double* x, const DevCamera* cams,
                                 const DevLoss* losses);

}
```

beam_slam_amd/csrc/k_reproj.hip:

```cpp
#include "bsgpu_device.h"
#include "marg_body.h"
#include "reproj_body.h"

namespace bsg {

template <bool WITH_J>
__global__ __launch_bounds__(256) void reproj_eval_kernel(int n, const int4* __restrict__ fac,
                                                          const double2* __restrict__ pix,
                                                          const double* __restrict__ wgt, const double* __restrict__ x,
                                                          const DevCamera* __restrict__ cams,
                                                          const DevLoss* __restrict__ losses,
                                                          double2* __restrict__ r_out, double* __restrict__ J_out, int ja,
                                                          double* __restrict__ JB_out, double* __restrict__ cost_part, int count_inactive) {
  __shared__ __attribute__((aligned(16))) double sJ[kReprojStage<WITH_J>];
  reproj_eval_body<WITH_J>((int)blockIdx.x, n, fac, pix, wgt, x, cams, losses, r_out, J_out, ja, JB_out, cost_part, count_inactive, sJ);
}

void launch_reproj_eval(hipStream_t s, const Visual& v, const double* x, const DevCamera* cams,
                        const DevLoss* losses, bool with_J, double* cost_part_out, bool count_inactive) {
  if (v.n == 0) return;
  const int grid = (v.n + 255) / 256;
  if (with_J)
    hipLaunchKernelGGL(reproj_eval_kernel<true>, dim3(grid), dim3(256), 0, s, v.n, v.fac, v.pix, v.w, x, cams, losses,
                       v.r, v.J, v.ja, v.JB, cost_part_out, count_inactive ? 1 : 0);
// ... 323 lines not shown
#pragma unroll
      for (int it = 0; it < 6; ++it) { sAa[it * 64 + lane] = va[it]; sAb[it * 64 + lane] = vb[it]; }
#pragma unroll
      for (int it = 0; it < 4; ++it) sCa[it * 64 + lane] = vc[it];
#pragma unroll
      for (int it = 0; it < 3; ++it) sCb[it * 64 + lane] = vd[it];
    }
    __builtin_amdgcn_wave_barrier();
    const double2* Ja = sAa + lane * 6;
    const double2* Jb = sAb + lane * 6;
    const double2* Ca2 = sCa + lane * 4;
    const double2* Cb2 = sCb + lane * 3;
    double A0[6], A1[6], B0[6], B1[6], Ca[8], Cb[6];
    {
      const double2 a0 = Ja[0], a1 = Ja[1], a2 = Ja[2], a3 = Ja[3], a4 = Ja[4], a5 = Ja[5];
      A0[0] = a0.x; A0[1] = a0.y; A0[2] = a1.x; A0[3] = a1.y; A0[4] = a2.x; A0[5] = a2.y;
      A1[0] = a3.x; A1[1] = a3.y; A1[2] = a4.x; A1[3] = a4.y; A1[4] = a5.x; A1[5] = a5.y;
      const double2 b0 = Jb[0], b1 = Jb[1], b2 = Jb[2], b3 = Jb[3], b4 = Jb[4], b5 = Jb[5];
      B0[0] = b0.x; B0[1] = b0.y; B0[2] = b1.x; B0[3] = b1.y; B0[4] = b2.x; B0[5] = b2.y;
      B1[0] = b3.x; B1[1] = b3.y; B1[2] = b4.x; B1[3] = b4.y; B1[4] = b5.x; B1[5] = b5.y;
      const double2 c0 = Ca2[0], c1 = Ca2[1], c2 = Ca2[2], c3 = Ca2[3];
      Ca[0] = c0.x; Ca[1] = c0.y; Ca[2] = c1.x; Ca[3] = c1.y; Ca[4] = c2.x; Ca[5] = c2.y; Ca[6] = c3.x; Ca[7] = c3.y;
      const double2 d0 = Cb2[0], d1 = Cb2[1], d2 = Cb2[2];
      Cb[0] = d0.x; Cb[1] = d0.y; Cb[2] = d1.x; Cb[3] = d1.y; Cb[4] = d2.x; Cb[5] = d2.y;
    }
    __builtin_amdgcn_wave_barrier();
    if (!live) continue;
    const double same = (fa == fb) ? 1.0 : 0.0;
    const double t00 = same - (Ca[0] * Cb[0] + Ca[1] * Cb[1] + Ca[2] * Cb[2]);
    const double t01 = -(Ca[0] * Cb[3] + Ca[1] * Cb[4] + Ca[2] * Cb[5]);
    const double t10 = -(Ca[3] * Cb[0] + Ca[4] * Cb[1] + Ca[5] * Cb[2]);
    const double t11 = same - (Ca[3] * Cb[3] + Ca[4] * Cb[4] + Ca[5] * Cb[5]);
#pragma unroll
    for (int c = 0; c < 6; ++c) {
      const double u0 = t00 * B0[c] + t01 * B1[c];
      const double u1 = t10 * B0[c] + t11 * B1[c];
#pragma unroll
      for (int a = 0; a < 6; ++a) blk[a * 6 + c] += A0[a] * u0 + A1[a] * u1;
    }
    if (fa == fb) {
      const double2 rf = r[fa];
      const double p0 = Ca[6], p1 = Ca[7];
#pragma unroll
      for (int a = 0; a < 6; ++a) {
        gr[a] += A0[a] * p0 + A1[a] * p1;
        gg[a] += A0[a] * rf.x + A1[a] * rf.y;
        hd[a] += A0[a] * A0[a] + A1[a] * A1[a];
      }
    }
  }
  double v[64];
#pragma unroll
  for (int i = 0; i < 36; ++i) v[i] = blk[i];
#pragma unroll
  for (int i = 0; i < 6; ++i) { v[36 + i] = gr[i]; v[42 + i] = gg[i]; v[48 + i] = hd[i]; }
#pragma unroll
  for (int i = 54; i < 64; ++i) v[i] = 0.0;
  wave_sum_transpose64(v);
  const double total = v[0];
  const int tqi = cp_tq[ci], tpi = cp_tp[ci], tqj = cp_tq[cj], tpj = cp_tp[cj];
  if (lane < 36) {
    const int a = lane / 6, c = lane % 6;
    const int row = (a < 3) ? (tqi < 0 ? -1 : tqi + a) : (tpi < 0 ? -1 : tpi + a - 3);
    const int col = (c < 3) ? (tqj < 0 ? -1 : tqj + c) : (tpj < 0 ? -1 : tpj + c - 3);
    if (row >= 0 && col >= 0) {
      const int sr = perm[row], sc = perm[col];
      atomicAdd(&S[(size_t)sr * ld + sc], total);
      if (!diag) atomicAdd(&S[(size_t)sc * ld + sr], total);
    }
  } else if (diag && lane < 54) {
    const int a = (lane - 36) % 6, which = (lane - 36) / 6;
    const int row = (a < 3) ? (tqi < 0 ? -1 : tqi + a) : (tpi < 0 ? -1 : tpi + a - 3);
    if (row >= 0) {
      if (which == 0) atomicAdd(&S[(size_t)rhs_row * ld + perm[row]], total);
      else if (which == 1) atomicAdd(&grad[row], total);
      else atomicAdd(&hdiag[row], total);
    }
  }
}
__global__ __launch_bounds__(64) void pairs_kernel(int n_seg, const int* __restrict__ seg_ci, const int* __restrict__ seg_cj, const int* __restrict__ seg_start, const int* __restrict__ ent_fa, const int* __restrict__ ent_fb, const double* __restrict__ J, const double2* __restrict__ r, const double* __restrict__ CR, const int* __restrict__ cp_tq, const int* __restrict__ cp_tp, double* __restrict__ S, int ld, int rhs_row, double* __restrict__ grad, double* __restrict__ hdiag, const int* __restrict__ perm, int grad_only, int n_pair_blocks, SmallGroupSet small, int n_small_units, GoWord go) {
  if (go.p && !(__hip_atomic_load(go.p, __ATOMIC_RELAXED, __HIP_MEMORY_SCOPE_AGENT) > 0.0)) return;
  pairs_kernel_body((int)blockIdx.x, (int)gridDim.x, n_seg, seg_ci, seg_cj, seg_start, ent_fa, ent_fb, J, r, CR, cp_tq, cp_tp, S, ld, rhs_row, grad, hdiag, perm, grad_only, n_pair_blocks, small, n_small_units);
}
struct pairs_kernel_Args {
  int bsg_grid;
  int n_seg;
  const int* seg_ci;
  const int* seg_cj;
  const int* seg_start;
  const int* ent_fa;
  const int* ent_fb;
  const double* J;
  const double2* r;
  const double* CR;
  const int* cp_tq;
  const int* cp_tp;
  double* S;
  int ld;
  int rhs_row;
  double* grad;
  double* hdiag;
  const int* perm;
  int grad_only;
  int n_pair_blocks;
  SmallGroupSet small;
  int n_small_units;
};
struct pairs_kernel_ArgsG {
  int bsg_grid;
  int n_seg;
  const int __attribute__((address_space(1)))* seg_ci;
  const int __attribute__((address_space(1)))* seg_cj;
  const int __attribute__((address_space(1)))* seg_start;
  const int __attribute__((address_space(1)))* ent_fa;
  const int __attribute__((address_space(1)))* ent_fb;
  const double __attribute__((address_space(1)))* J;
  const double2 __attribute__((address_space(1)))* r;
  const double __attribute__((address_space(1)))* CR;
  const int __attribute__((address_space(1)))* cp_tq;
  const int __attribute__((address_space(1)))* cp_tp;
  double __attribute__((address_space(1)))* S;
  int ld;
  int rhs_row;
  double __attribute__((address_space(1)))* grad;
  double __attribute__((address_space(1)))* hdiag;
  const int __attribute__((address_space(1)))* perm;
  int grad_only;
  int n_pair_blocks;
  SmallGroupSet small;
  int n_small_units;
};
static_assert(sizeof(pairs_kernel_ArgsG) == sizeof(pairs_kernel_Args), "layout");

__global__ __launch_bounds__(64) __attribute__((amdgpu_waves_per_eu(2, 2))) void pairs_kernel_batch(const pairs_kernel_Args* __restrict__ bsg_A, const BatchDyn* __restrict__ bsg_dyn, int bsg_list) {
  const int bsg_w = bsg_dyn->idx[bsg_list][blockIdx.y];
  const pairs_kernel_ArgsG& a = reinterpret_cast<const pairs_kernel_ArgsG*>(bsg_A)[bsg_w];
  if ((int)blockIdx.x >= a.bsg_grid) return;
  pairs_kernel_body((int)blockIdx.x, a.bsg_grid, a.n_seg, (const int*)a.seg_ci, (const int*)a.seg_cj, (const int*)a.seg_start, (const int*)a.ent_fa, (const int*)a.ent_fb, (const double*)a.J, (const double2*)a.r, (double*)a.CR, (const int*)a.cp_tq, (const int*)a.cp_tp, (double*)a.S, a.ld, a.rhs_row, (double*)a.grad, (double*)a.hdiag, (const int*)a.perm, bsg_dyn->grad_only[bsg_w], a.n_pair_blocks, a.small, a.n_small_units);
}

constexpr size_t kPairsLds = sizeof(double2) * 64 * (6 + 6 + 4 + 3) + sizeof(int) * 128;
void launch_pairs(hipStream_t s, const Visual& v, double* S, int ld, int rhs_row, double* grad, double* hdiag, const int* perm,
                  bool grad_only, const SmallGroupSet* small, int n_small_units, GoWord go) {
  if (v.n_seg == 0) return;
  const int pair_blocks = 8 * ((v.n_seg + 7) / 8);
  SmallGroupSet none;
  none.n = 0;
  const int small_blocks = small ? 8 * ((n_small_units * kPairRiderParts + 7) / 8) : 0;
  hipLaunchKernelGGL(pairs_kernel, dim3(pair_blocks + small_blocks), dim3(64), kPairsLds, s, v.n_seg, v.seg_ci, v.seg_cj, v.seg_start, v.ent_fa,
                     v.ent_fb, v.J, v.r, v.CR, v.cp_tq, v.cp_tp, S, ld, rhs_row, grad, hdiag, perm, grad_only ? 1 : 0, pair_blocks, small ? *small : none,
                     small_blocks, go);
}

BSG_DEV void pose_part(const double* __restrict__ Jf_row, int tq, int tp, const double* __restrict__ y_pose, double& j0, double& j1) {
  const double2* J2 = reinterpret_cast<const double2*>(Jf_row);
  const double2 v0 = J2[0], v1 = J2[1], v2 = J2[2], v3 = J2[3], v4 = J2[4], v5 = J2[5];
  const double Jf[12] = {v0.x, v0.y, v1.x, v1.y, v2.x, v2.y, v3.x, v3.y, v4.x, v4.y, v5.x, v5.y};
  j0 = 0.0; j1 = 0.0;
  if (tq >= 0) {
#pragma unroll
    for (int k = 0; k < 3; ++k) { const double yv = y_pose[tq + k]; j0 += Jf[k] * yv; j1 += Jf[6 + k] * yv; }
  }
  if (tp >= 0) {
#pragma unroll
    for (int k = 0; k < 3; ++k) { const double yv = y_pose[tp + k]; j0 += Jf[3 + k] * yv; j1 += Jf[9 + k] * yv; }
  }
}
BSG_DEV void pose_part_compact(const double* __restrict__ Jf_row, const double (&B)[6], int tq, int tp, const double* __restrict__ y_pose, double& j0, double& j1) {
  const double2* J2 = reinterpret_cast<const double2*>(Jf_row);
  const double2 v0 = J2[0], v1 = J2[1], v2 = J2[2];
  const double Jf[6] = {v0.x, v0.y, v1.x, v1.y, v2.x, v2.y};
  j0 = 0.0; j1 = 0.0;
  if (tq >= 0) {
#pragma unroll
    for (int k = 0; k < 3; ++k) { const double yv = y_pose[tq + k]; j0 += Jf[k] * yv; j1 += Jf[3 + k] * yv; }
  }
  if (tp >= 0) {
#pragma unroll
    for (int k = 0; k < 3; ++k) { const double yv = y_pose[tp + k]; j0 += (-B[k]) * yv; j1 += (-B[3 + k]) * yv; }
  }
}
__device__ __forceinline__ void backsub_mcc_kernel_body(const int bsg_bx, const int bsg_gx, int n_lm, int n_lm_groups, int n_elim, int n, const int* __restrict__ lm_start, const double* __restrict__ J, int ja, const double* __restrict__ JB, const double2* __restrict__ r, const double* __restrict__ CR, const int* __restrict__ cam_pose, const int* __restrict__ cp_tq, const int* __restrict__ cp_tp, const double* __restrict__ Linv, const double* __restrict__ z, int n_pose, const double* __restrict__ y_pose, double* __restrict__ delta, double* __restrict__ mcc_part, int n_vis_blocks, const SmallGroupSet& small, int n_small_units, const UpdateRide& up, int first_update_block) {
  __shared__ double sred[4];
  if (up.n_blocks > 0 && bsg_bx >= first_update_block) {
    const int unit = bsg_bx - first_update_block, i = unit * 256 + (int)threadIdx.x;
    double d2 = 0.0, x2 = 0.0;
    if (i < up.n_blocks) update_block(up.blocks[i], up.xoff, up.toff, up.size, up.manifold, up.x, delta, up.x_cand, d2, x2);
    const double a = block_sum_256(d2, sred);
    const double c = block_sum_256(x2, sred);
    if (threadIdx.x == 0) { up.part[2 * unit] = a; up.part[2 * unit + 1] = c; }
    return;
  }
  if (bsg_bx >= n_vis_blocks) {
    const int unit = 2 * (bsg_bx - n_vis_blocks) + ((int)threadIdx.x >> 7);
    if (unit < n_small_units) small_mcc_unit(small, unit, threadIdx.x & 127, delta, sred + 2 * (threadIdx.x >> 7));
    else __syncthreads();
    return;
  }
  double acc = 0.0, upd_d2 = 0.0, upd_x2 = 0.0;
  if (bsg_bx < n_lm_groups) {
    const int gid = bsg_bx * 256 + threadIdx.x;
    const int l = gid >> 3, sub = gid & 7;
    const bool valid = l < n_lm;
    int beg = 0, end = 0;
    if (valid) { beg = lm_start[l]; end = lm_start[l + 1]; }
    const int lc = valid ? l : 0;
    const double* Li = Linv + (size_t)lc * kLmRec;
    const double Li0 = Li[0], Li1 = Li[1], Li2 = Li[2], Li3 = Li[3], Li4 = Li[4], Li5 = Li[5];
    const double* zl = z + (size_t)lc * kLmRec;
    const double zl0 = zl[0], zl1 = zl[1], zl2 = zl[2];
    double a0 = 0, a1 = 0, a2 = 0;
    double jk0[2] = {0.0, 0.0}, jk1[2] = {0.0, 0.0};
    int it = 0;
    const bool no_cr = CR == nullptr;
    const bool compact = ja == kJACompact;
    for (int f = beg + sub; f < end; f += 8, ++it) {
      const double2* C2 = no_cr ? reinterpret_cast<const double2*>(JB + (size_t)f * 6) : reinterpret_cast<const double2*>(CR + (size_t)f * 8);
      const double2 ca = C2[0], cb = C2[1], cc = C2[2];
      const double C[6] = {ca.x, ca.y, cb.x, cb.y, cc.x, cc.y};
      const int cp = cam_pose[f];
      double j0, j1;
      if (compact) pose_part_compact(J + (size_t)f * kJACompact, C, cp_tq[cp], cp_tp[cp], y_pose, j0, j1);
      else pose_part(J + (size_t)f * kJAStride, cp_tq[cp], cp_tp[cp], y_pose, j0, j1);
      if (it == 0) { jk0[0] = j0; jk1[0] = j1; } else if (it == 1) { jk0[1] = j0; jk1[1] = j1; }
      a0 += C[0] * j0 + C[3] * j1; a1 += C[1] * j0 + C[4] * j1; a2 += C[2] * j0 + C[5] * j1;
    }
#pragma unroll
    for (int o = 4; o > 0; o >>= 1) { a0 += __shfl_xor(a0, o, 8); a1 += __shfl_xor(a1, o, 8); a2 += __shfl_xor(a2, o, 8); }
    if (no_cr) {
      const double b0 = a0, b1 = a1, b2 = a2;
      a0 = Li0 * b0; a1 = Li1 * b0 + Li2 * b1; a2 = Li3 * b0 + Li4 * b1 + Li5 * b2;
    }
    if (valid) {
      const double w0 = zl0 - a0, w1 = zl1 - a1, w2 = zl2 - a2;
      const double y0 = Li0 * w0 + Li1 * w1 + Li3 * w2;
      const double y1 = Li2 * w1 + Li4 * w2;
      const double y2 = Li5 * w2;
      if (sub == 0) {
        const int to = n_pose + 3 * l;
        delta[to] = -y0; delta[to + 1] = -y1; delta[to + 2] = -y2;
        if (up.n_blocks > 0) {
          const int xo = up.lm_xoff[l];
          const double x0 = up.x[xo], x1 = up.x[xo + 1], x2v = up.x[xo + 2];
          const double c0 = x0 + (-y0), c1 = x1 + (-y1), c2 = x2v + (-y2);
          up.x_cand[xo] = c0; up.x_cand[xo + 1] = c1; up.x_cand[xo + 2] = c2;
          const double e0 = x0 - c0, e1 = x1 - c1, e2 = x2v - c2;
          upd_d2 = e0 * e0 + e1 * e1 + e2 * e2; upd_x2 = x0 * x0 + x1 * x1 + x2v * x2v;
        }
      }
      it = 0;
      for (int f = beg + sub; f < end; f += 8, ++it) {
        const double2* B2 = reinterpret_cast<const double2*>(JB + (size_t)f * 6);
        const double2 ba = B2[0], bb = B2[1], bc = B2[2];
        const double Bf[6] = {ba.x, ba.y, bb.x, bb.y, bc.x, bc.y};
        double j0, j1;
        if (it == 0) { j0 = jk0[0]; j1 = jk1[0]; }
        else if (it == 1) { j0 = jk0[1]; j1 = jk1[1]; }
        else if (compact) { const int cp = cam_pose[f]; pose_part_compact(J + (size_t)f * kJACompact, Bf, cp_tq[cp], cp_tp[cp], y_pose, j0, j1); }
        else { const int cp = cam_pose[f]; pose_part(J + (size_t)f * kJAStride, cp_tq[cp], cp_tp[cp], y_pose, j0, j1); }
        const double d0 = -(j0 + Bf[0] * y0 + Bf[1] * y1 + Bf[2] * y2), d1 = -(j1 + Bf[3] * y0 + Bf[4] * y1 + Bf[5] * y2);
        const double2 rf = r[f];
        acc -= d0 * (rf.x + 0.5 * d0) + d1 * (rf.y + 0.5 * d1);
      }
    }
  } else {
    const int f = n_elim + (bsg_bx - n_lm_groups) * 256 + (int)threadIdx.x;
    if (f < n) {
      const int cp = cam_pose[f];
      double j0, j1;
      pose_part(J + (size_t)f * kJAStride, cp_tq[cp], cp_tp[cp], y_pose, j0, j1);
      const double2 rf = r[f];
      acc = -((-j0) * (rf.x - 0.5 * j0) + (-j1) * (rf.y - 0.5 * j1));
    }
  }
  const double tot = block_sum_256(acc, sred);
  if (threadIdx.x == 0) mcc_part[bsg_bx] = tot;
  if (up.n_blocks > 0 && bsg_bx < n_lm_groups) {
    const double a = block_sum_256(upd_d2, sred);
    const double c = block_sum_256(upd_x2, sred);
    const int slot = (up.n_blocks + 255) / 256 + bsg_bx;
    if (threadIdx.x == 0) { up.part[2 * slot] = a; up.part[2 * slot + 1] = c; }
  }
}
__global__ __launch_bounds__(256) void backsub_mcc_kernel(int n_lm, int n_lm_groups, int n_elim, int n, const int* __restrict__ lm_start, const double* __restrict__ J, int ja, const double* __restrict__ JB, const double2* __restrict__ r, const double* __restrict__ CR, const int* __restrict__ cam_pose, const int* __restrict__ cp_tq, const int* __restrict__ cp_tp, const double* __restrict__ Linv, const double* __restrict__ z, int n_pose, const double* __restrict__ y_pose, double* __restrict__ delta, double* __restrict__ mcc_part, int n_vis_blocks, SmallGroupSet small, int n_small_units, UpdateRide up, int first_update_block) {
  backsub_mcc_kernel_body((int)blockIdx.x, (int)gridDim.x, n_lm, n_lm_groups, n_elim, n, lm_start, J, ja, JB, r, CR, cam_pose, cp_tq, cp_tp, Linv, z, n_pose, y_pose, delta, mcc_part, n_vis_blocks, small, n_small_units, up, first_update_block);
}
struct backsub_mcc_kernel_Args {
  int bsg_grid;
  int n_lm;
  int n_lm_groups;
  int n_elim;
  int n;
  const int* lm_start;
  const double* J;
  int ja;
  const double* JB;
  const double2* r;
  const double* CR;
  const int* cam_pose;
  const int* cp_tq;
  const int* cp_tp;
  const double* Linv;
  const double* z;
  int n_pose;
  const double* y_pose;
  double* delta;
  double* mcc_part;
  int n_vis_blocks;
  SmallGroupSet small;
  int n_small_units;
  UpdateRide up;
  int first_update_block;
};
struct backsub_mcc_kernel_ArgsG {
  int bsg_grid;
  int n_lm;
  int n_lm_groups;
  int n_elim;
  int n;
  const int __attribute__((address_space(1)))* lm_start;
  const double __attribute__((address_space(1)))* J;
  int ja;
  const double __attribute__((address_space(1)))* JB;
  const double2 __attribute__((address_space(1)))* r;
  const double __attribute__((address_space(1)))* CR;
  const int __attribute__((address_space(1)))* cam_pose;
  const int __attribute__((address_space(1)))* cp_tq;
  const int __attribute__((address_space(1)))* cp_tp;
  const double __attribute__((address_space(1)))* Linv;
  const double __attribute__((address_space(1)))* z;
  int n_pose;
  const double __attribute__((address_space(1)))* y_pose;
  double __attribute__((address_space(1)))* delta;
  double __attribute__((address_space(1)))* mcc_part;
  int n_vis_blocks;
  SmallGroupSet small;
  int n_small_units;
  UpdateRide up;
  int first_update_block;
};
static_assert(sizeof(backsub_mcc_kernel_ArgsG) == sizeof(backsub_mcc_kernel_Args), "layout");

__global__ __launch_bounds__(256) void backsub_mcc_kernel_batch(const backsub_mcc_kernel_Args* __restrict__ bsg_A, const BatchDyn* __restrict__ bsg_dyn, int bsg_list) {
  const int bsg_w = bsg_dyn->idx[bsg_list][blockIdx.y];
  const backsub_mcc_kernel_ArgsG& a = reinterpret_cast<const backsub_mcc_kernel_ArgsG*>(bsg_A)[bsg_w];
  if ((int)blockIdx.x >= a.bsg_grid) return;
  backsub_mcc_kernel_body((int)blockIdx.x, a.bsg_grid, a.n_lm, a.n_lm_groups, a.n_elim, a.n, (const int*)a.lm_start, (const double*)a.J, a.ja, (const double*)a.JB, (const double2*)a.r, (double*)a.CR, (const int*)a.cam_pose, (const int*)a.cp_tq, (const int*)a.cp_tp, (const double*)a.Linv, (const double*)a.z, a.n_pose, (const double*)a.y_pose, (double*)a.delta, (double*)a.mcc_part, a.n_vis_blocks, a.small, a.n_small_units, a.up, a.first_update_block);
}

void batchargs_landmark(BatchArgTable& t, BatchArgTable& t_tail, const Visual& v, int n_pose, int jacobi, double lm_lo, double lm_hi, double* scale, double* dcl,
                        double* grad, const ZeroStep& zero ) {
  landmark_kernel_Args a;
  const int grid = (v.n_lm * 8 + 255) / 256, zero_blocks = std::max(1, std::min(zero.n_tiles, 1024));
  a.bsg_grid = v.n_lm > 0 ? grid + zero_blocks : 0;
  a.n_lm = v.n_lm; a.lm_start = v.lm_start; a.JB = v.JB; a.r = v.r; a.n_pose = n_pose; a.radius_ptr = nullptr; a.compute_scale = 0; a.compute_dcl = 0;
  a.jacobi = jacobi; a.lm_lo = lm_lo; a.lm_hi = lm_hi; a.scale = scale; a.dcl = dcl; a.grad = grad; a.Linv_out = v.Linv; a.z_out = v.z; a.CR = v.no_cr ? nullptr : v.CR;
  a.lm_blocks = grid; a.zs = zero; a.radius_val = 0.0;
  t.push(a);
  landmark_tail_kernel_Args b;
  b.bsg_grid = v.n > v.n_elim ? (v.n - v.n_elim + 255) / 256 : 0;
  b.first = v.n_elim; b.n = v.n; b.r = v.r; b.CR = v.CR;
  t_tail.push(b);
}
void launch_landmark_batch(hipStream_t s, const BatchArgTable& t, const BatchArgTable& t_tail, const BatchDyn* dyn, int list, int n) {
  if (n <= 0) return;
  if (t.max_grid > 0) hipLaunchKernelGGL(landmark_kernel_batch, dim3(t.max_grid, n), dim3(256), 0, s, static_cast<const landmark_kernel_Args*>(t.dev), dyn, list);
  if (t_tail.max_grid > 0) hipLaunchKernelGGL(landmark_tail_kernel_batch, dim3(t_tail.max_grid, n), dim3(256), 0, s, static_cast<const landmark_tail_kernel_Args*>(t_tail.dev), dyn, list);
}
void batchargs_pairs(BatchArgTable& t, const Visual& v, double* S, int ld, int rhs_row, double* grad, double* hdiag, const int* perm, const SmallGroupSet* small,
                     int n_small_units) {
  pairs_kernel_Args a;
  const int pair_blocks = 8 * ((v.n_seg + 7) / 8), small_blocks = small ? 8 * ((n_small_units * kPairRiderParts + 7) / 8) : 0;
  SmallGroupSet none;
  none.n = 0;
  a.bsg_grid = v.n_seg > 0 ? pair_blocks + small_blocks : 0;
  a.n_seg = v.n_seg; a.seg_ci = v.seg_ci; a.seg_cj = v.seg_cj; a.seg_start = v.seg_start; a.ent_fa = v.ent_fa; a.ent_fb = v.ent_fb; a.J = v.J; a.r = v.r; a.CR = v.CR;
  a.cp_tq = v.cp_tq; a.cp_tp = v.cp_tp; a.S = S; a.ld = ld; a.rhs_row = rhs_row; a.grad = grad; a.hdiag = hdiag; a.perm = perm; a.grad_only = 0;
  a.n_pair_blocks = pair_blocks; a.small = small ? *small : none; a.n_small_units = small_blocks;
  t.push(a);
}
void launch_pairs_batch(hipStream_t s, const BatchArgTable& t, const BatchDyn* dyn, int list, int n) {
  if (n <= 0 || t.max_grid <= 0) return;
  hipLaunchKernelGGL(pairs_kernel_batch, dim3(t.max_grid, n), dim3(64), kPairsLds, s, static_cast<const pairs_kernel_Args*>(t.dev), dyn, list);
}
int backsub_mcc_groups(const Visual& v);
void batchargs_backsub_mcc(BatchArgTable& t, const Visual& v, int n_pose, const double* y_pose, double* delta, double* mcc_part, const SmallGroupSet* small,
                           int n_small_units, const UpdateRide* upd) {
  backsub_mcc_kernel_Args a;
  const int g_lm = (v.n_lm * 8 + 255) / 256, grid = backsub_mcc_groups(v);
  const int extra = small ? (n_small_units + 1) / 2 : 0;
  const int upd_units = (upd && upd->n_blocks > 0) ? (upd->n_blocks + 255) / 256 : 0;
  a.bsg_grid = grid > 0 ? grid + extra + upd_units : 0;
  a.n_lm = v.n_lm; a.n_lm_groups = g_lm; a.n_elim = v.n_elim; a.n = v.n; a.lm_start = v.lm_start; a.J = v.J; a.ja = v.ja; a.JB = v.JB; a.r = v.r; a.CR = v.no_cr ? nullptr : v.CR; a.cam_pose = v.cam_pose;
  a.cp_tq = v.cp_tq; a.cp_tp = v.cp_tp; a.Linv = v.Linv; a.z = v.z; a.n_pose = n_pose; a.y_pose = y_pose; a.delta = delta; a.mcc_part = mcc_part; a.n_vis_blocks = grid;
  a.small = small ? *small : SmallGroupSet(); a.n_small_units = small ? n_small_units : 0; a.up = upd_units ? *upd : UpdateRide(); a.first_update_block = grid + extra;
  t.push(a);
}
void launch_backsub_mcc_batch(hipStream_t s, const BatchArgTable& t, const BatchDyn* dyn, int list, int n) {
  if (n <= 0 || t.max_grid <= 0) return;
  hipLaunchKernelGGL(backsub_mcc_kernel_batch, dim3(t.max_grid, n), dim3(256), 0, s, static_cast<const backsub_mcc_kernel_Args*>(t.dev), dyn, list);
}
int backsub_mcc_groups(const Visual& v) { return (v.n_lm * 8 + 255) / 256 + (v.n - v.n_elim + 255) / 256; }
__global__ __launch_bounds__(256) void backsub_mcc_marg_kernel(int n_lm, int n_lm_groups, int n_elim, int n, const int* __restrict__ lm_start, const double* __restrict__ J, int ja, const double* __restrict__ JB, const double2* __restrict__ r, const double* __restrict__ CR, const int* __restrict__ cam_pose, const int* __restrict__ cp_tq, const int* __restrict__ cp_tp, const double* __restrict__ Linv, const double* __restrict__ z, int n_pose, const double* __restrict__ y_pose, double* __restrict__ delta, double* __restrict__ mcc_part, int n_vis_blocks, SmallGroupSet small, int n_small_units, UpdateRide up, int first_update_block, MargDev m, double* __restrict__ marg_part, int first_marg_block) {
  if ((int)blockIdx.x >= first_marg_block) { marg_mcc_kernel_body(4 * ((int)blockIdx.x - first_marg_block), m, delta, marg_part); return; }
  backsub_mcc_kernel_body((int)blockIdx.x, first_marg_block, n_lm, n_lm_groups, n_elim, n, lm_start, J, ja, JB, r, CR, cam_pose, cp_tq, cp_tp, Linv, z, n_pose, y_pose, delta, mcc_part, n_vis_blocks, small, n_small_units, up, first_update_block);
}
bool launch_backsub_mcc(hipStream_t s, const Visual& v, int n_pose, const double* y_pose, double* delta, double* mcc_part,
                        const SmallGroupSet* small, int n_small_units, const UpdateRide* upd, const MargDev* marg, double* marg_part) {
  const int g_lm = (v.n_lm * 8 + 255) / 256, grid = backsub_mcc_groups(v);
  if (grid == 0) return false;
  const int extra = small ? (n_small_units + 1) / 2 : 0;
  const int upd_units = (upd && upd->n_blocks > 0) ? (upd->n_blocks + 255) / 256 : 0;
  if (marg && marg_part && marg->rows > 0) {
    const int own = grid + extra + upd_units;
    hipLaunchKernelGGL(backsub_mcc_marg_kernel, dim3(own + (marg->rows + 3) / 4), dim3(256), 0, s, v.n_lm, g_lm, v.n_elim, v.n, v.lm_start, v.J, v.ja, v.JB, v.r, v.no_cr ? nullptr : v.CR, v.cam_pose,
                       v.cp_tq, v.cp_tp, v.Linv, v.z, n_pose, y_pose, delta, mcc_part, grid, small ? *small : SmallGroupSet(), small ? n_small_units : 0,
                       upd_units ? *upd : UpdateRide(), grid + extra, *marg, marg_part, own);
    return true;
  }
  hipLaunchKernelGGL(backsub_mcc_kernel, dim3(grid + extra + upd_units), dim3(256), 0, s, v.n_lm, g_lm, v.n_elim, v.n, v.lm_start, v.J, v.ja, v.JB, v.r, v.no_cr ? nullptr : v.CR, v.cam_pose,
                     v.cp_tq, v.cp_tp, v.Linv, v.z, n_pose, y_pose, delta, mcc_part, grid, small ? *small : SmallGroupSet(), small ? n_small_units : 0,
                     upd_units ? *upd : UpdateRide(), grid + extra);
  return false;
}

}
```

beam_slam_amd/gpu.py:

```python
import ctypes
import os

from . import capi

_HERE = os.path.dirname(os.path.abspath(__file__))
LIB_PATH = os.path.join(_HERE, "csrc", "libbsgpu.so")
_LIB = None


class GpuLibraryMissing(RuntimeError):
    pass


def lib():
    global _LIB
    if _LIB is None:
        if not os.path.exists(LIB_PATH):
            raise GpuLibraryMissing(
                f"{LIB_PATH} is missing: build it with `python -c 'import __graft_entry__ as g; g.build()'` "
                "(hipcc --offload-arch=gfx950).  beam_slam_amd has no CPU fallback.")
        _LIB = ctypes.CDLL(LIB_PATH)
        _LIB.bsgpu_time_reproj_jacobian_ms.restype = ctypes.c_double
        _LIB.bsgpu_time_reproj_jacobian_ms.argtypes = [ctypes.c_void_p, ctypes.c_int32]
        _LIB.bsgpu_time_eval_ms.restype = ctypes.c_double
        _LIB.bsgpu_time_eval_ms.argtypes = [ctypes.c_void_p, ctypes.c_int32]
        _LIB.bsgpu_eval_bytes.restype = ctypes.c_int64
        _LIB.bsgpu_eval_bytes.argtypes = [ctypes.c_void_p]
        _LIB.bsgpu_reproj_jacobian_bytes.restype = ctypes.c_int64
        _LIB.bsgpu_reproj_jacobian_bytes.argtypes = [ctypes.c_void_p]
        _LIB.bsgpu_dense_solve.argtypes = [ctypes.c_int, ctypes.c_int32, ctypes.c_void_p, ctypes.c_void_p, ctypes.c_void_p,
                                           ctypes.c_int32, ctypes.POINTER(ctypes.c_double)]
    return _LIB


def dense_solve(A, b, device=0, max_chains=4):
    import numpy as np
    A = np.ascontiguousarray(A, np.float64)
    b = np.ascontiguousarray(b, np.float64)
    x = np.empty_like(b)
    ms = ctypes.c_double(0.0)
    rc = lib().bsgpu_dense_solve(device, A.shape[0], A.ctypes.data, b.ctypes.data, x.ctypes.data, int(max_chains),
                                 ctypes.byref(ms))
    if rc != 0:
        raise capi.SolverError(rc, "bsgpu_dense_solve failed")
    return x, ms.value


def preintegrate(sample_start, t, w, a, t_end, bg, ba, cov_w, cov_a, cov_bg, cov_ba, info_weight=1.0, device=0):
    import numpy as np
    f64 = lambda x: np.ascontiguousarray(x, np.float64)
    ss = np.ascontiguousarray(sample_start, np.int32)
    n = ss.size - 1
    t, w, a, t_end, bg, ba = f64(t), f64(w), f64(a), f64(t_end), f64(bg), f64(ba)
    covs = [f64(np.asarray(c, float) * (np.eye(3) if np.ndim(c) == 0 else 1.0)) for c in (cov_w, cov_a, cov_bg, cov_ba)]
    out = np.empty((n, 287))
    fn = lib().bsgpu_preintegrate
    fn.argtypes = [ctypes.c_int, ctypes.c_int32] + [ctypes.c_void_p] * 11 + [ctypes.c_double, ctypes.c_void_p]
    rc = fn(device, n, ss.ctypes.data, t.ctypes.data, w.ctypes.data, a.ctypes.data, t_end.ctypes.data, bg.ctypes.data, ba.ctypes.data,
            covs[0].ctypes.data, covs[1].ctypes.data, covs[2].ctypes.data, covs[3].ctypes.data, float(info_weight), out.ctypes.data)
    if rc != 0:
        raise capi.SolverError(rc, "bsgpu_preintegrate failed")
    return out


def inertial_alignment(frame_start, t_frame, q_frame, p_frame, imu_range, t, w, a, bridge_gap=False,
                       min_excitation=capi.ALIGN_MIN_EXCITATION, apply_scale=True, scale_min=capi.ALIGN_SCALE_MIN,
                       scale_max=capi.ALIGN_SCALE_MAX, rank_tol=capi.ALIGN_RANK_TOL, device=0):
    import numpy as np
    f64 = lambda x, shape: np.ascontiguousarray(x, np.float64).reshape(shape)
    fs = np.ascontiguousarray(frame_start, np.int32).reshape(-1)
    P = fs.size - 1
    ir = np.ascontiguousarray(imu_range, np.int32).reshape(-1, 2)
    tf, qf, pf = f64(t_frame, (-1,)), f64(q_frame, (-1, 4)), f64(p_frame, (-1, 3))
    t, w, a = f64(t, (-1,)), f64(w, (-1, 3)), f64(a, (-1, 3))
    F = tf.size
    if P < 0 or ir.shape[0] != P or qf.shape[0] != F or pf.shape[0] != F or w.shape[0] != t.size or a.shape[0] != t.size:
        raise capi.SolverError(capi.ERR_INVALID, "inertial_alignment: array sizes do not agree")
    if P > 0 and (int(fs.max()) > F or int(ir.max()) > t.size):
        raise capi.SolverError(capi.ERR_INVALID, "inertial_alignment: frame_start / imu_range name more frames or samples than were passed")
    out = dict(gravity=np.zeros((P, 3)), bg=np.zeros((P, 3)), scale=np.zeros(P), excitation=np.zeros(P), gyro_rank=np.zeros(P, np.int32),
               velocity=np.zeros((F, 3)), q_out=np.zeros((F, 4)), p_out=np.zeros((F, 3)), v_out=np.zeros((F, 3)), status=np.zeros(P, np.int32))
    fn = lib().bsgpu_inertial_alignment
    fn.argtypes = capi.INERTIAL_ALIGNMENT_ARGTYPES
    _dp, _ip = capi._dp, capi._ip
    d = lambda x: x.ctypes.data_as(_dp)
    rc = fn(device, P, fs.ctypes.data_as(_ip), d(tf), d(qf), d(pf), ir.ctypes.data_as(_ip), d(t), d(w), d(a), int(bool(bridge_gap)),
            float(min_excitation), int(bool(apply_scale)), float(scale_min), float(scale_max), float(rank_tol), d(out["gravity"]),
            d(out["bg"]), d(out["scale"]), d(out["excitation"]), out["gyro_rank"].ctypes.data_as(_ip), d(out["velocity"]), d(out["q_out"]),
            d(out["p_out"]), d(out["v_out"]), out["status"].ctypes.data_as(_ip))
    if rc != 0:
        raise capi.SolverError(rc, "bsgpu_inertial_alignment failed")
    return out


def register_scans(ref_start, ref_points, tgt_start, tgt_points, T_init=None, max_corr=capi.ICP_DEFAULTS["max_corr"],
                   max_iter=capi.ICP_DEFAULTS["max_iter"], t_eps=capi.ICP_DEFAULTS["t_eps"], fit_eps=capi.ICP_DEFAULTS["fit_eps"],
                   rotation_threshold=capi.ICP_DEFAULTS["rotation_threshold"], rel_mse_eps=capi.ICP_DEFAULTS["rel_mse_eps"], device=0):
    import numpy as np
    rs = np.ascontiguousarray(ref_start, np.int32).reshape(-1)
    ts = np.ascontiguousarray(tgt_start, np.int32).reshape(-1)
    rp = np.ascontiguousarray(ref_points, np.float64).reshape(-1, 3)
    tp = np.ascontiguousarray(tgt_points, np.float64).reshape(-1, 3)
    P = rs.size - 1
    ti = None if T_init is None else np.ascontiguousarray(T_init, np.float64).reshape(-1, 3, 4)
    if P < 0 or ts.size != P + 1 or (ti is not None and ti.shape[0] != P):
        raise capi.SolverError(capi.ERR_INVALID, "register_scans: array sizes do not agree")
    if int(rs.max()) > rp.shape[0] or int(ts.max()) > tp.shape[0]:
        raise capi.SolverError(capi.ERR_INVALID, "register_scans: ref_start / tgt_start name more points than were passed")
    out = dict(T_refest_ref=np.zeros((P, 3, 4)), T_ref_tgt=np.zeros((P, 3, 4)), mse=np.zeros(P), n_corr=np.zeros(P, np.int32),
               n_iters=np.zeros(P, np.int32), status=np.zeros(P, np.int32))
    fn = lib().bsgpu_register_scans
    fn.argtypes = capi.REGISTER_SCANS_ARGTYPES
    _dp, _ip = capi._dp, capi._ip
    d = lambda x: None if x is None else x.ctypes.data_as(_dp)
    i = lambda x: x.ctypes.data_as(_ip)
    rc = fn(device, P, i(rs), d(rp), i(ts), d(tp), d(ti), float(max_corr), int(max_iter), float(t_eps), float(fit_eps),
            float(rotation_threshold), float(rel_mse_eps), d(out["T_refest_ref"]), d(out["T_ref_tgt"]), d(out["mse"]), i(out["n_corr"]),
            i(out["n_iters"]), i(out["status"]))
    if rc != 0:
        raise capi.SolverError(rc, register_scans_error())
    return out


def register_scans_error():
    fn = lib().bsgpu_register_scans_error
    fn.restype = ctypes.c_char_p
    fn.argtypes = []
    return fn().decode()


class GpuSolver(capi.Solver):

    def __init__(self, device=0):
        super().__init__(lib(), "bsgpu_", device)

    def reprojection_errors(self, n):
        import numpy as np
        out = np.zeros(n)
        fn = lib().bsgpu_reprojection_errors
        fn.argtypes = [ctypes.c_void_p, ctypes.c_void_p]
        self._chk(fn(self._ctx, out.ctypes.data))
        return out

    def triangulate(self, track_start, q_block, p_block, pixels, camera=0, truncate_pixels=True, max_dist=-1.0, max_reproj=-1.0):
        import numpy as np
        ts = np.ascontiguousarray(track_start, np.int32)
        qb, pb = np.ascontiguousarray(q_block, np.int32), np.ascontiguousarray(p_block, np.int32)
        px = np.ascontiguousarray(pixels, np.float64)
        n = ts.size - 1
        pts, st = np.zeros((n, 3)), np.zeros(n, np.int32)
        fn = lib().bsgpu_triangulate
        fn.argtypes = [ctypes.c_void_p, ctypes.c_int32] + [ctypes.c_void_p] * 4 + [ctypes.c_int32, ctypes.c_int32, ctypes.c_double,
                                                                                  ctypes.c_double, ctypes.c_void_p, ctypes.c_void_p]
        self._chk(fn(self._ctx, n, ts.ctypes.data, qb.ctypes.data, pb.ctypes.data, px.ctypes.data, int(camera), int(bool(truncate_pixels)),
                     float(max_dist), float(max_reproj), pts.ctypes.data, st.ctypes.data))
        return pts, st

    def essential_ransac(self, match_start, px_prev, px_cur, K, prob=0.99, threshold_px=1.0, max_iters=1000, seed=0):
        import numpy as np
        ms = np.ascontiguousarray(match_start, np.int32)
        S = ms.size - 1
        p1 = np.ascontiguousarray(px_prev, np.float64).reshape(-1, 2)
        p2 = np.ascontiguousarray(px_cur, np.float64).reshape(-1, 2)
        Ks = np.ascontiguousarray(np.broadcast_to(np.asarray(K, np.float64).reshape(-1, 4), (S, 4)))
        if p1.shape != p2.shape or (ms.size and p1.shape[0] < int(ms.max())):
            raise capi.SolverError(capi.ERR_INVALID, "essential_ransac: match_start names more matches than were passed")
        out = dict(mask=np.zeros(p1.shape[0], np.uint8), E=np.zeros((S, 3, 3)), n_inliers=np.zeros(S, np.int32), n_iters=np.zeros(S, np.int32),
                   best_sample=np.zeros((S, 5), np.int32), status=np.zeros(S, np.int32))
        fn = lib().bsgpu_essential_ransac
        fn.argtypes = capi.ESSENTIAL_RANSAC_ARGTYPES
        _dp, _ip, _bp = capi._dp, capi._ip, capi._bp
        self._chk(fn(self._ctx, S, ms.ctypes.data_as(_ip), p1.ctypes.data_as(_dp), p2.ctypes.data_as(_dp), Ks.ctypes.data_as(_dp),
                     float(prob), float(threshold_px), int(max_iters), int(seed) & ((1 << 64) - 1), out["mask"].ctypes.data_as(_bp),
                     out["E"].ctypes.data_as(_dp), out["n_inliers"].ctypes.data_as(_ip), out["n_iters"].ctypes.data_as(_ip),
                     out["best_sample"].ctypes.data_as(_ip), out["status"].ctypes.data_as(_ip)))
        return out

    def absolute_pose_ransac(self, obs_start, pixels, points, camera=0, prob=0.0, threshold_px=5.0, max_iters=100, seed=0,
                             truncate_pixels=False):
        import numpy as np
        os_ = np.ascontiguousarray(obs_start, np.int32)
        F = os_.size - 1
        pix = np.ascontiguousarray(pixels, np.float64).reshape(-1, 2)
        pts = np.ascontiguousarray(points, np.float64).reshape(-1, 3)
        cam = np.ascontiguousarray(np.broadcast_to(np.asarray(camera, np.int32), (F,)))
        if pix.shape[0] != pts.shape[0] or (os_.size and pix.shape[0] < int(os_.max())):
            raise capi.SolverError(capi.ERR_INVALID, "absolute_pose_ransac: obs_start names more pairs than were passed")
        out = dict(mask=np.zeros(pix.shape[0], np.uint8), q=np.zeros((F, 4)), p=np.zeros((F, 3)), T_cam_world=np.zeros((F, 3, 4)),
                   n_inliers=np.zeros(F, np.int32), n_iters=np.zeros(F, np.int32), best_sample=np.zeros((F, 3), np.int32),
                   status=np.zeros(F, np.int32))
        fn = lib().bsgpu_absolute_pose_ransac
        fn.argtypes = capi.ABSOLUTE_POSE_RANSAC_ARGTYPES
        _dp, _ip, _bp = capi._dp, capi._ip, capi._bp
        self._chk(fn(self._ctx, F, os_.ctypes.data_as(_ip), pix.ctypes.data_as(_dp), pts.ctypes.data_as(_dp), cam.ctypes.data_as(_ip),
                     float(prob), float(threshold_px), int(max_iters), int(seed) & ((1 << 64) - 1), int(bool(truncate_pixels)),
                     out["mask"].ctypes.data_as(_bp), out["q"].ctypes.data_as(_dp), out["p"].ctypes.data_as(_dp),
                     out["T_cam_world"].ctypes.data_as(_dp), out["n_inliers"].ctypes.data_as(_ip), out["n_iters"].ctypes.data_as(_ip),
                     out["best_sample"].ctypes.data_as(_ip), out["status"].ctypes.data_as(_ip)))
        return out

    def relative_pose_ransac(self, match_start, px_first, px_last, camera=0, prob=0.0, threshold_px=5.0, max_iters=100, seed=0,
                             truncate_pixels=False, validate_px=10.0, min_inlier_ratio=0.8):
        import numpy as np
        ms = np.ascontiguousarray(match_start, np.int32)
        S = ms.size - 1
        p0 = np.ascontiguousarray(px_first, np.float64).reshape(-1, 2)
        p1 = np.ascontiguousarray(px_last, np.float64).reshape(-1, 2)
        cam = np.ascontiguousarray(np.broadcast_to(np.asarray(camera, np.int32), (S,)))
        if p0.shape != p1.shape or (ms.size and p0.shape[0] < int(ms.max())):
            raise capi.SolverError(capi.ERR_INVALID, "relative_pose_ransac: match_start names more matches than were passed")
        n = p0.shape[0]
        out = dict(mask=np.zeros(n, np.uint8), T_last_first=np.zeros((S, 3, 4)), q=np.zeros((S, 2, 4)), p=np.zeros((S, 2, 3)),
                   points=np.zeros((n, 3)), valid_mask=np.zeros(n, np.uint8), inlier_ratio=np.zeros(S), pair_valid=np.zeros(S, np.int32),
                   n_inliers=np.zeros(S, np.int32), n_iters=np.zeros(S, np.int32), best_sample=np.zeros((S, 7), np.int32),
                   status=np.zeros(S, np.int32))
        fn = lib().bsgpu_relative_pose_ransac
        fn.argtypes = capi.RELATIVE_POSE_RANSAC_ARGTYPES
        _dp, _ip, _bp = capi._dp, capi._ip, capi._bp
        self._chk(fn(self._ctx, S, ms.ctypes.data_as(_ip), p0.ctypes.data_as(_dp), p1.ctypes.data_as(_dp), cam.ctypes.data_as(_ip),
                     float(prob), float(threshold_px), int(max_iters), int(seed) & ((1 << 64) - 1), int(bool(truncate_pixels)),
                     float(validate_px), float(min_inlier_ratio), out["mask"].ctypes.data_as(_bp), out["T_last_first"].ctypes.data_as(_dp),
                     out["q"].ctypes.data_as(_dp), out["p"].ctypes.data_as(_dp), out["points"].ctypes.data_as(_dp),
                     out["valid_mask"].ctypes.data_as(_bp), out["inlier_ratio"].ctypes.data_as(_dp), out["pair_valid"].ctypes.data_as(_ip),
                     out["n_inliers"].ctypes.data_as(_ip), out["n_iters"].ctypes.data_as(_ip), out["best_sample"].ctypes.data_as(_ip),
                     out["status"].ctypes.data_as(_ip)))
        return out

    @staticmethod
    def batch_stats():
        w, r = ctypes.c_int64(0), ctypes.c_int64(0)
        lib().bsgpu_batch_stats(ctypes.byref(w), ctypes.byref(r))
        return w.value, r.value

    def time_reproj_jacobian_ms(self, reps=20):
        ms = lib().bsgpu_time_reproj_jacobian_ms(self._ctx, int(reps))
        if ms < 0:
            raise capi.SolverError(capi.ERR_DEVICE, "bsgpu_time_reproj_jacobian_ms failed")
        return ms

    def time_eval_ms(self, reps=20):
        ms = lib().bsgpu_time_eval_ms(self._ctx, int(reps))
        if ms < 0:
            raise capi.SolverError(capi.ERR_DEVICE, "bsgpu_time_eval_ms failed")
        return ms

    def eval_bytes(self):
        return lib().bsgpu_eval_bytes(self._ctx)

    def bsr_info(self):
        a, b = ctypes.c_int32(0), ctypes.c_int32(0)
        self._chk(lib().bsgpu_bsr_info(ctypes.c_void_p(self._ctx), ctypes.byref(a), ctypes.byref(b)))
        return a.value, b.value

    PHASES = ("eval_reproj", "eval_other", "landmark", "pairs", "assemble_other", "factor", "backsolve", "backsub", "candidate")

    def profile_step(self, options=None, reps=10):
        import numpy as np
        opt = options if options is not None else self.options_default()
        ms, work = np.zeros(len(self.PHASES)), np.zeros(len(self.PHASES))
        fn = lib().bsgpu_profile_step
        fn.argtypes = [ctypes.c_void_p, ctypes.c_void_p, ctypes.c_int32, ctypes.c_void_p, ctypes.c_void_p]
        self._chk(fn(self._ctx, ctypes.byref(opt), int(reps), ms.ctypes.data, work.ctypes.data))
        return {name: (float(ms[i]), float(work[i])) for i, name in enumerate(self.PHASES)}

    def set_plan_preference(self, throughput):
        fn = lib().bsgpu_set_plan_preference
        fn.argtypes = [ctypes.c_void_p, ctypes.c_int32]
        self._chk(fn(self._ctx, 1 if throughput else 0))

    def plan_info(self):
        a, b, c = ctypes.c_int32(0), ctypes.c_int32(0), ctypes.c_int32(0)
        self.finalize()
        lib().bsgpu_plan_info(ctypes.c_void_p(self._ctx), ctypes.byref(a), ctypes.byref(b), ctypes.byref(c))
        return a.value, b.value, c.value

    def reproj_jacobian_bytes(self):
        return lib().bsgpu_reproj_jacobian_bytes(self._ctx)
```

include/bsgpu.h:

```cpp
#ifndef BSGPU_H_
#define BSGPU_H_

#include <stdint.h>

#ifdef __cplusplus
extern "C" {
#endif

#define BSGPU_ABI_VERSION 1

enum {
  BSGPU_OK = 0,
  BSGPU_ERR_INVALID = -1,
  BSGPU_ERR_DEVICE = -2,
  BSGPU_ERR_UNSUPPORTED = -3,
  BSGPU_ERR_NUMERIC = -4
};

enum {
  BSGPU_MANIFOLD_EUCLIDEAN = 0,
  BSGPU_MANIFOLD_QUAT_RIGHT = 1
};

enum {
// ... 22 lines not shown
int bsgpu_nidx(int type);
int bsgpu_nconst(int type);
int bsgpu_nres(int type);

enum {
  BSGPU_LINEAR_AUTO = 0,
  BSGPU_LINEAR_SCHUR_CHOLESKY = 1,
  BSGPU_LINEAR_PCG = 2,
  BSGPU_LINEAR_SCHUR_PCG = 3
};

enum {
  BSGPU_TR_LEVENBERG_MARQUARDT = 0,
  BSGPU_TR_DOGLEG = 1,
  BSGPU_TR_SUBSPACE_DOGLEG = 2
};

enum {
  BSGPU_CONVERGENCE = 0,
  BSGPU_NO_CONVERGENCE = 1,
  BSGPU_FAILURE = 2
};

typedef struct bsgpu_options {
  int32_t max_num_iterations;
  int32_t linear_solver_type;
  int32_t jacobi_scaling;
  int32_t max_num_consecutive_invalid_steps;
  double max_solver_time_in_seconds;
  double function_tolerance;
  double gradient_tolerance;
  double parameter_tolerance;
  double initial_trust_region_radius;
  double max_trust_region_radius;
  double min_trust_region_radius;
  double min_relative_decrease;
  double min_lm_diagonal;
  double max_lm_diagonal;
  int32_t pcg_max_iterations;
  int32_t trust_region_strategy_type;
  double pcg_tolerance;
} bsgpu_options;

void bsgpu_options_default(bsgpu_options* o);
void bsgpu_options_vio(bsgpu_options* o);

typedef struct bsgpu_summary {
  int32_t termination_type;
  int32_t is_solution_usable;
  int32_t num_iterations;
  int32_t num_successful_steps;
  int32_t num_unsuccessful_steps;
  int32_t num_parameters_tangent;
  int32_t num_residuals;
  int32_t linear_solver_used;
  int32_t num_linear_solves;
  int32_t num_inner_iterations;
  double initial_cost;
  double final_cost;
  double fixed_cost;
  double total_time_in_seconds;
  double device_time_in_seconds;
  double time_eval_seconds;
  double time_assemble_seconds;
  double time_linear_solve_seconds;
  char message[160];
} bsgpu_summary;

typedef struct bsgpu_iteration {
  int32_t iteration;
  int32_t step_is_valid;
  int32_t step_is_successful;
  int32_t reserved0;
  double cost;
  double cost_change;
  double gradient_max_norm;
  double gradient_norm;
  double step_norm;
  double relative_decrease;
  double trust_region_radius;
  double model_cost_change;
} bsgpu_iteration;

typedef struct bsgpu_camera {
  double fx, fy, cx, cy;
  double R_cam_baselink[9];
  double t_cam_baselink[3];
} bsgpu_camera;

typedef struct bsgpu_ctx bsgpu_ctx;

bsgpu_ctx* bsgpu_create(int device);
const char* bsgpu_create_error(void);
void bsgpu_destroy(bsgpu_ctx* ctx);
const char* bsgpu_last_error(const bsgpu_ctx* ctx);
int bsgpu_abi_version(void);

int bsgpu_clear(bsgpu_ctx* ctx);

int bsgpu_set_blocks(bsgpu_ctx* ctx, int32_t n_blocks, const double* values,
                     const int32_t* offset, const uint8_t* size,
                     const uint8_t* manifold, const uint8_t* is_const);

int bsgpu_set_values(bsgpu_ctx* ctx, const double* values, int64_t n_values);

int bsgpu_set_cameras(bsgpu_ctx* ctx, int32_t n_cameras, const bsgpu_camera* cams);

int bsgpu_add_factors(bsgpu_ctx* ctx, int32_t type, int32_t n,
                      const int32_t* block_idx, const double* consts,
                      const int32_t* loss_kind, const double* loss_a);
int bsgpu_add_factors_indirect(bsgpu_ctx* ctx, int32_t type, int32_t n, const int32_t* slot_idx, int32_t n_slots,
                               const int32_t* slot_to_block, const double* consts, const int32_t* loss_kind,
                               const double* loss_a);
int bsgpu_sync_factors_indirect(bsgpu_ctx* ctx, int32_t type, int32_t n, const int32_t* slot_idx, int32_t n_slots,
                                const int32_t* slot_to_block, const double* consts, const int32_t* loss_kind,
                                const double* loss_a, int32_t n_changed, const int32_t* changed_rows);

int bsgpu_add_marginal(bsgpu_ctx* ctx, int32_t n_blocks, const int32_t* blocks, int32_t n_rows,
                       const double* A, const double* b, const double* xbar);
int bsgpu_update_marginal(bsgpu_ctx* ctx, int32_t index, int32_t n_rows, int32_t n_cols, int32_t n_xbar, const double* A, const double* b,
                          const double* xbar);

int bsgpu_finalize(bsgpu_ctx* ctx);

int bsgpu_solve(bsgpu_ctx* ctx, const bsgpu_options* options, bsgpu_summary* summary);
int bsgpu_solve_batch(bsgpu_ctx* const* ctxs, int32_t n, const bsgpu_options* options, int32_t options_stride,
                      bsgpu_summary* summaries);
int bsgpu_batch_stats(int64_t* windows_batched, int64_t* rounds);

int bsgpu_get_blocks(bsgpu_ctx* ctx, double* values, int64_t n_values);

int bsgpu_reset_values(bsgpu_ctx* ctx);

int bsgpu_num_iterations_recorded(const bsgpu_ctx* ctx);
int bsgpu_get_iteration(const bsgpu_ctx* ctx, int32_t i, bsgpu_iteration* out);
int bsgpu_num_factorizations(const bsgpu_ctx* ctx);

int bsgpu_evaluate(bsgpu_ctx* ctx, double* cost, double* residuals,
                   double* gradient, double* jacobian);
int bsgpu_num_residuals(const bsgpu_ctx* ctx);
int bsgpu_num_parameters_tangent(const bsgpu_ctx* ctx);
int bsgpu_tangent_offset(const bsgpu_ctx* ctx, int32_t block);

int bsgpu_marginalize(bsgpu_ctx* ctx, int32_t n_marg, const int32_t* marg_blocks,
                      int32_t* n_kept, int32_t* n_rows, int32_t* n_cols);
int bsgpu_get_marginal(const bsgpu_ctx* ctx, int32_t* kept_blocks, double* A, double* b, double* xbar);

int bsgpu_covariance(bsgpu_ctx* ctx, int32_t block_a, int32_t block_b, double* out);
int bsgpu_covariance_joint(bsgpu_ctx* ctx, int32_t n_blocks, const int32_t* blocks, double* out);
int bsgpu_covariance_requests(bsgpu_ctx* ctx, int32_t n_requests, const int32_t* block_pairs, int64_t* offsets, double* out);

int bsgpu_reprojection_errors(bsgpu_ctx* ctx, double* err);

int bsgpu_preintegrate(int device, int32_t n_intervals, const int32_t* sample_start, const double* t, const double* w,
                       const double* a, const double* t_end, const double* bg, const double* ba, const double* cov_w,
                       const double* cov_a, const double* cov_bg, const double* cov_ba, double info_weight,
                       double* consts_out);

enum { BSGPU_ALIGN_OK = 0, BSGPU_ALIGN_TOO_FEW_FRAMES = 1, BSGPU_ALIGN_BAD_IMU = 2, BSGPU_ALIGN_NOT_EXCITED = 3,
       BSGPU_ALIGN_RANK_DEFICIENT = 4, BSGPU_ALIGN_SCALE_REJECTED = 5 };
int bsgpu_inertial_alignment(int device, int32_t n_paths, const int32_t* frame_start, const double* t_frame, const double* q_frame,
                             const double* p_frame, const int32_t* imu_range, const double* t, const double* w, const double* a,
                             int32_t bridge_gap, double min_excitation, int32_t apply_scale, double scale_min, double scale_max,
                             double rank_tol, double* gravity, double* bg, double* scale, double* excitation, int32_t* gyro_rank,
                             double* velocity, double* q_out, double* p_out, double* v_out, int32_t* status);

enum { BSGPU_ICP_MAX_ITERATIONS = 1, BSGPU_ICP_TRANSFORM = 2, BSGPU_ICP_ABS_MSE = 3, BSGPU_ICP_REL_MSE = 4,
       BSGPU_ICP_TOO_FEW_CORRESPONDENCES = 5 };
#define BSGPU_ICP_MAX_CELLS (1 << 22)
#define BSGPU_ICP_MAX_ITER 1000
int bsgpu_register_scans(int device, int32_t n_pairs, const int32_t* ref_start, const double* ref_points, const int32_t* tgt_start,
                         const double* tgt_points, const double* T_init, double max_corr, int32_t max_iter, double t_eps,
                         double fit_eps, double rotation_threshold, double rel_mse_eps, double* T_refest_ref, double* T_ref_tgt,
                         double* mse, int32_t* n_corr, int32_t* n_iters, int32_t* status);
const char* bsgpu_register_scans_error(void);

int bsgpu_triangulate(bsgpu_ctx* ctx, int32_t n_tracks, const int32_t* track_start, const int32_t* q_block,
                      const int32_t* p_block, const double* pixels, int32_t camera, int32_t truncate_pixels,
                      double max_dist, double max_reproj, double* points, int32_t* status);

int bsgpu_localize_frames(bsgpu_ctx* ctx, int32_t n_frames, const int32_t* obs_start, const double* pixels, const double* points,
                          const int32_t* lm_block, const int32_t* camera, const double* q_init, const double* p_init,
                          int32_t loss_kind, double loss_a, double sqrt_info, int32_t truncate_pixels, int32_t min_points,
                          int32_t image_width, int32_t image_height, const bsgpu_options* options, double* q_out, double* p_out,
                          double* cov_out, double* avg_reproj, double* final_cost, int32_t* iterations, int32_t* status);

enum { BSGPU_RANSAC_OK = 0, BSGPU_RANSAC_TOO_FEW = 1, BSGPU_RANSAC_NO_MODEL = 2 };
#define BSGPU_RANSAC_MAX_MATCHES 65536
int bsgpu_essential_ransac(bsgpu_ctx* ctx, int32_t n_sets, const int32_t* match_start, const double* px_prev, const double* px_cur,
                           const double* K, double prob, double threshold_px, int32_t max_iters, uint64_t seed, uint8_t* mask,
                           double* E, int32_t* n_inliers, int32_t* n_iters, int32_t* best_sample, int32_t* status);

int bsgpu_absolute_pose_ransac(bsgpu_ctx* ctx, int32_t n_frames, const int32_t* obs_start, const double* pixels,
                               const double* points, const int32_t* camera, double prob, double threshold_px,
                               int32_t max_iters, uint64_t seed, int32_t truncate_pixels, uint8_t* mask,
                               double* q_out, double* p_out, double* T_cam_world, int32_t* n_inliers,
                               int32_t* n_iters, int32_t* best_sample, int32_t* status);

int bsgpu_relative_pose_ransac(bsgpu_ctx* ctx, int32_t n_sets, const int32_t* match_start, const double* px_first,
                               const double* px_last, const int32_t* camera, double prob, double threshold_px,
                               int32_t max_iters, uint64_t seed, int32_t truncate_pixels, double validate_px,
                               double min_inlier_ratio, uint8_t* mask, double* T_last_first, double* q_out, double* p_out,
                               double* points, uint8_t* valid_mask, double* inlier_ratio, int32_t* pair_valid,
                               int32_t* n_inliers, int32_t* n_iters, int32_t* best_sample, int32_t* status);

double bsgpu_time_reproj_jacobian_ms(bsgpu_ctx* ctx, int32_t reps);
double bsgpu_time_eval_ms(bsgpu_ctx* ctx, int32_t reps);
int64_t bsgpu_eval_bytes(const bsgpu_ctx* ctx);
int bsgpu_bsr_info(bsgpu_ctx* ctx, int32_t* block_rows, int32_t* nnz_blocks);
int64_t bsgpu_reproj_jacobian_bytes(const bsgpu_ctx* ctx);
enum {
  BSGPU_PHASE_EVAL_REPROJ = 0,
  BSGPU_PHASE_EVAL_OTHER = 1,
  BSGPU_PHASE_LANDMARK = 2,
  BSGPU_PHASE_PAIRS = 3,
  BSGPU_PHASE_ASSEMBLE_OTHER = 4,
  BSGPU_PHASE_FACTOR = 5,
  BSGPU_PHASE_BACKSOLVE = 6,
  BSGPU_PHASE_BACKSUB = 7,
  BSGPU_PHASE_CANDIDATE = 8,
  BSGPU_PHASE_NUM = 9
};
int bsgpu_profile_step(bsgpu_ctx* ctx, const bsgpu_options* options, int32_t reps, double* ms_out, double* work_out);

int bsgpu_dense_solve(int device, int32_t n, const double* A, const double* b, double* x,
                      int32_t max_chains, double* ms_out);
int bsgpu_plan_info(const bsgpu_ctx* ctx, int32_t* n_chains, int32_t* n_steps, int32_t* n_tiles);
enum { BSGPU_PLAN_LATENCY = 0, BSGPU_PLAN_THROUGHPUT = 1 };
int bsgpu_set_plan_preference(bsgpu_ctx* ctx, int32_t preference);

#ifdef __cplusplus
}
#endif
#endif
```

Before: 3765 LM iterations/s.

## Precompute per-factor tangent offsets and stage pose update in LDS for back-substitution

Adds a per-factor int2 table built once at finalize, so back-substitution does one load instead of the cam_pose to cp_tq/cp_tp double indirection. The pose update vector y_pose is staged into dynamic shared memory when it fits (up to 4096 entries), which cuts scattered global reads. The first two observations per landmark are prefetched and pinned in registers with empty asm, and the marg kernel gets a waves-per-EU hint. The cost is extra device memory for the table, LDS use that may lower occupancy, a __syncthreads, and a new debug API for checking the table.

```diff
diff --git a/beam_slam_amd/capi.py b/beam_slam_amd/capi.py
--- a/beam_slam_amd/capi.py
+++ b/beam_slam_amd/capi.py
@@ -108,7 +108,7 @@
     "reprojection_errors", "preintegrate", "triangulate", "time_reproj_jacobian_ms", "reproj_jacobian_bytes", "dense_solve", "plan_info",
     "profile_step", "time_eval_ms", "eval_bytes", "bsr_info", "covariance_joint", "update_marginal", "solve_batch", "batch_stats", "set_plan_preference",
     "covariance_requests", "localize_frames", "num_factorizations", "essential_ransac", "absolute_pose_ransac",
-    "relative_pose_ransac", "inertial_alignment", "register_scans", "register_scans_error",
+    "relative_pose_ransac", "inertial_alignment", "register_scans", "register_scans_error", "backsub_tangent_table",
 ]
 
 _dp = C.POINTER(C.c_double)
diff --git a/beam_slam_amd/csrc/bsgpu_api.cpp b/beam_slam_amd/csrc/bsgpu_api.cpp
--- a/beam_slam_amd/csrc/bsgpu_api.cpp
+++ b/beam_slam_amd/csrc/bsgpu_api.cpp
@@ -930,6 +930,33 @@
   auto slot = [&](int src) { const int t = src >> 28, f = src & ((1 << 28) - 1); return (t == BSGPU_F_REPROJ ? 0 : n0) + f; };
   for (int i = 0; i < V.n; ++i) err[slot(c->vis_src[i])] = h[i];
   for (int i = 0; i < D.n; ++i) err[slot(c->dense_src[i])] = h[(size_t)V.n + i];
+  return BSGPU_OK;
+} catch (...) { return api_exception(c); }
+
+int bsgpu_backsub_tangent_table(bsgpu_ctx* c, int32_t* fac_t, int32_t* joined) try {
+  if (!c) return BSGPU_ERR_INVALID;
+  if (!fac_t || !joined) return fail(c, BSGPU_ERR_INVALID, "null argument");
+  int rc = finalize(c);
+  if (rc != BSGPU_OK) return rc;
+  HIPCHK(c, hipSetDevice(c->device));
+  const Visual& V = c->vis;
+  if ((rc = ensure_vis_src(c)) != BSGPU_OK) return rc;
+  if (V.n == 0) return BSGPU_OK;
+  std::vector<int2> ft(V.n);
+  std::vector<int> cam_pose(V.n), cp_tq(V.n_cam_pose), cp_tp(V.n_cam_pose);
+  HIPCHK(c, hipStreamSynchronize(c->stream));
+  HIPCHK(c, hipMemcpy(ft.data(), V.fac_t, sizeof(int2) * V.n, hipMemcpyDeviceToHost));
+  HIPCHK(c, hipMemcpy(cam_pose.data(), V.cam_pose, sizeof(int) * V.n, hipMemcpyDeviceToHost));
+  HIPCHK(c, hipMemcpy(cp_tq.data(), V.cp_tq, sizeof(int) * V.n_cam_pose, hipMemcpyDeviceToHost));
+  HIPCHK(c, hipMemcpy(cp_tp.data(), V.cp_tp, sizeof(int) * V.n_cam_pose, hipMemcpyDeviceToHost));
+  const int n0 = c->groups[BSGPU_F_REPROJ].n;
+  for (int i = 0; i < V.n; ++i) {
+    const int t = c->vis_src[i] >> 28, f = c->vis_src[i] & ((1 << 28) - 1);
+    const size_t o = 2 * (size_t)((t == BSGPU_F_REPROJ ? 0 : n0) + f);
+    if (cam_pose[i] < 0 || cam_pose[i] >= V.n_cam_pose) return fail(c, BSGPU_ERR_DEVICE, "backsub_tangent_table: camera-pose id out of range");
+    fac_t[o] = ft[i].x; fac_t[o + 1] = ft[i].y;
+    joined[o] = cp_tq[cam_pose[i]]; joined[o + 1] = cp_tp[cam_pose[i]];
+  }
   return BSGPU_OK;
 } catch (...) { return api_exception(c); }
 
diff --git a/beam_slam_amd/csrc/bsgpu_finalize.cpp b/beam_slam_amd/csrc/bsgpu_finalize.cpp
--- a/beam_slam_amd/csrc/bsgpu_finalize.cpp
+++ b/beam_slam_amd/csrc/bsgpu_finalize.cpp
@@ -502,7 +502,9 @@
     V.cost_part = c->alloc<double>(V.n_cost_part);
     V.cost_part_cand = c->alloc<double>(V.n_cost_part);
     V.mcc_part = c->alloc<double>(std::max(1, backsub_mcc_groups(V)));
-    if (!V.J || !V.CR || !V.r) return fail(c, BSGPU_ERR_DEVICE, "out of device memory (visual tables)");
+    V.fac_t = c->alloc<int2>(nv);
+    if (!V.J || !V.CR || !V.r || !V.fac_t) return fail(c, BSGPU_ERR_DEVICE, "out of device memory (visual tables)");
+    launch_fac_t(c->stream, V);
     if (c->calib.on) {
       c->calib.E = c->alloc<double>((size_t)std::max(1, nv) * 12); c->calib.Et = c->alloc<double>((size_t)std::max(1, nv) * 12);
       c->calib.part = c->alloc<double>((size_t)std::max(1, calib_border_blocks(V)) * kCalibPartStride);
diff --git a/beam_slam_amd/csrc/bsgpu_internal.h b/beam_slam_amd/csrc/bsgpu_internal.h
--- a/beam_slam_amd/csrc/bsgpu_internal.h
+++ b/beam_slam_amd/csrc/bsgpu_internal.h
@@ -109,6 +109,7 @@
   int n_cam_pose = 0;
   int* cp_tq = nullptr;
   int* cp_tp = nullptr;
+  int2* fac_t = nullptr;
   int n_seg = 0, n_ent = 0;
   int* seg_ci = nullptr; int* seg_cj = nullptr; int* seg_start = nullptr;
   int* ent_fa = nullptr; int* ent_fb = nullptr;
@@ -285,6 +286,7 @@
 struct BatchArgTable {
   std::vector<unsigned char> host;
   size_t stride = 0, lds = 0;
+  bool lds_over = false;
   int max_grid = 0;
   void* dev = nullptr;
   template <class A> void push(const A& a) {
@@ -543,6 +545,7 @@
 int pcg_done_slot();
 int pcg_iters_slot();
 int backsub_mcc_groups(const Visual& v);
+void launch_fac_t(hipStream_t s, const Visual& v);
 bool launch_backsub_mcc(hipStream_t s, const Visual& v, int n_pose, const double* y_pose, double* delta, double* mcc_part,
                         const SmallGroupSet* small = nullptr, int n_small_units = 0, const UpdateRide* upd = nullptr, const MargDev* marg = nullptr,
                         double* marg_part = nullptr);
diff --git a/beam_slam_amd/csrc/k_reproj.hip b/beam_slam_amd/csrc/k_reproj.hip
--- a/beam_slam_amd/csrc/k_reproj.hip
+++ b/beam_slam_amd/csrc/k_reproj.hip
@@ -499,35 +499,174 @@
                      small_blocks, go);
 }
 
-BSG_DEV void pose_part(const double* __restrict__ Jf_row, int tq, int tp, const double* __restrict__ y_pose, double& j0, double& j1) {
-  const double2* J2 = reinterpret_cast<const double2*>(Jf_row);
-  const double2 v0 = J2[0], v1 = J2[1], v2 = J2[2], v3 = J2[3], v4 = J2[4], v5 = J2[5];
-  const double Jf[12] = {v0.x, v0.y, v1.x, v1.y, v2.x, v2.y, v3.x, v3.y, v4.x, v4.y, v5.x, v5.y};
+extern __shared__ __attribute__((aligned(16))) double bsg_backsub_y[];
+constexpr int kBacksubStageMax = 4096;
+static size_t backsub_stage_bytes(int n_pose) {
+  if (n_pose <= 0 || n_pose > kBacksubStageMax) return 0;
+  const int n2 = (n_pose + 1) >> 1;
+  return (size_t)4096 * (n2 <= 512 ? 2 : n2 <= 1024 ? 4 : 8);
+}
+template <bool Y_LDS> BSG_DEV double backsub_y(const double* __restrict__ y_pose, int i) {
+  if constexpr (Y_LDS) return bsg_backsub_y[i]; else return y_pose[i];
+}
+template <bool COMPACT> BSG_DEV void pose_row_load(const double* __restrict__ J, int f, double (&A)[COMPACT ? 6 : 12]) {
+  if constexpr (COMPACT) {
+    const double2* J2 = reinterpret_cast<const double2*>(J + (size_t)f * kJACompact);
+    const double2 v0 = J2[0], v1 = J2[1], v2 = J2[2];
+    A[0] = v0.x; A[1] = v0.y; A[2] = v1.x; A[3] = v1.y; A[4] = v2.x; A[5] = v2.y;
+  } else {
+    const double2* J2 = reinterpret_cast<const double2*>(J + (size_t)f * kJAStride);
+    const double2 v0 = J2[0], v1 = J2[1], v2 = J2[2], v3 = J2[3], v4 = J2[4], v5 = J2[5];
+    A[0] = v0.x; A[1] = v0.y; A[2] = v1.x; A[3] = v1.y; A[4] = v2.x; A[5] = v2.y;
+    A[6] = v3.x; A[7] = v3.y; A[8] = v4.x; A[9] = v4.y; A[10] = v5.x; A[11] = v5.y;
+  }
+}
+template <bool Y_LDS, bool COMPACT>
+BSG_DEV void pose_row_dot(const double (&A)[COMPACT ? 6 : 12], const double (&B)[6], int tq, int tp, const double* __restrict__ y_pose, double& j0, double& j1) {
   j0 = 0.0; j1 = 0.0;
-  if (tq >= 0) {
-#pragma unroll
-    for (int k = 0; k < 3; ++k) { const double yv = y_pose[tq + k]; j0 += Jf[k] * yv; j1 += Jf[6 + k] * yv; }
-  }
-  if (tp >= 0) {
-#pragma unroll
-    for (int k = 0; k < 3; ++k) { const double yv = y_pose[tp + k]; j0 += Jf[3 + k] * yv; j1 += Jf[9 + k] * yv; }
-  }
-}
-BSG_DEV void pose_part_compact(const double* __restrict__ Jf_row, const double (&B)[6], int tq, int tp, const double* __restrict__ y_pose, double& j0, double& j1) {
-  const double2* J2 = reinterpret_cast<const double2*>(Jf_row);
-  const double2 v0 = J2[0], v1 = J2[1], v2 = J2[2];
-  const double Jf[6] = {v0.x, v0.y, v1.x, v1.y, v2.x, v2.y};
-  j0 = 0.0; j1 = 0.0;
-  if (tq >= 0) {
-#pragma unroll
-    for (int k = 0; k < 3; ++k) { const double yv = y_pose[tq + k]; j0 += Jf[k] * yv; j1 += Jf[3 + k] * yv; }
-  }
-  if (tp >= 0) {
-#pragma unroll
-    for (int k = 0; k < 3; ++k) { const double yv = y_pose[tp + k]; j0 += (-B[k]) * yv; j1 += (-B[3 + k]) * yv; }
-  }
-}
-__device__ __forceinline__ void backsub_mcc_kernel_body(const int bsg_bx, const int bsg_gx, int n_lm, int n_lm_groups, int n_elim, int n, const int* __restrict__ lm_start, const double* __restrict__ J, int ja, const double* __restrict__ JB, const double2* __restrict__ r, const double* __restrict__ CR, const int* __restrict__ cam_pose, const int* __restrict__ cp_tq, const int* __restrict__ cp_tp, const double* __restrict__ Linv, const double* __restrict__ z, int n_pose, const double* __restrict__ y_pose, double* __restrict__ delta, double* __restrict__ mcc_part, int n_vis_blocks, const SmallGroupSet& small, int n_small_units, const UpdateRide& up, int first_update_block) {
+  if constexpr (COMPACT) {
+    if (tq >= 0) {
+#pragma unroll
+      for (int k = 0; k < 3; ++k) { const double yv = backsub_y<Y_LDS>(y_pose, tq + k); j0 += A[k] * yv; j1 += A[3 + k] * yv; }
+    }
+    if (tp >= 0) {
+#pragma unroll
+      for (int k = 0; k < 3; ++k) { const double yv = backsub_y<Y_LDS>(y_pose, tp + k); j0 += (-B[k]) * yv; j1 += (-B[3 + k]) * yv; }
+    }
+  } else {
+    if (tq >= 0) {
+#pragma unroll
+      for (int k = 0; k < 3; ++k) { const double yv = backsub_y<Y_LDS>(y_pose, tq + k); j0 += A[k] * yv; j1 += A[6 + k] * yv; }
+    }
+    if (tp >= 0) {
+#pragma unroll
+      for (int k = 0; k < 3; ++k) { const double yv = backsub_y<Y_LDS>(y_pose, tp + k); j0 += A[3 + k] * yv; j1 += A[9 + k] * yv; }
+    }
+  }
+}
+template <int K> BSG_DEV void backsub_stage_y(const double* __restrict__ y_pose, int n2) {
+  const double2* y2 = reinterpret_cast<const double2*>(y_pose);
+  double2* s2 = reinterpret_cast<double2*>(bsg_backsub_y);
+  double2 ys[K];
+#pragma unroll
+  for (int k = 0; k < K; ++k) { const int i = (int)threadIdx.x + 256 * k; ys[k] = y2[i < n2 ? i : n2 - 1]; }
+#pragma unroll
+  for (int k = 0; k < K; ++k) s2[(int)threadIdx.x + 256 * k] = ys[k];
+}
+template <int N> BSG_DEV void pin(double (&a)[N]) {
+#pragma unroll
+  for (int k = 0; k + 1 < N; k += 2) asm volatile("" : "+v"(a[k]), "+v"(a[k + 1]));
+}
+BSG_DEV void pin(double2& a, int2& b) { asm volatile("" : "+v"(a.x), "+v"(a.y), "+v"(b.x), "+v"(b.y)); }
+BSG_DEV void row6_load(const double* __restrict__ base, int pitch, int f, double (&R)[6]) {
+  const double2* p = reinterpret_cast<const double2*>(base + (size_t)f * pitch);
+  const double2 a = p[0], b = p[1], c = p[2];
+  R[0] = a.x; R[1] = a.y; R[2] = b.x; R[3] = b.y; R[4] = c.x; R[5] = c.y;
+}
+template <bool Y_LDS, bool COMPACT>
+BSG_DEV void backsub_lm_group(const int bsg_bx, int n_lm, const int* __restrict__ lm_start, const double* __restrict__ J, const double* __restrict__ JB, const double2* __restrict__ r, const double* __restrict__ CR, const int2* __restrict__ fac_t, const double* __restrict__ Linv, const double* __restrict__ z, int n_pose, const double* __restrict__ y_pose, double* __restrict__ delta, const UpdateRide& up, double& acc, double& upd_d2, double& upd_x2) {
+  const int gid = bsg_bx * 256 + threadIdx.x;
+  const int l = gid >> 3, sub = gid & 7;
+  const bool valid = l < n_lm;
+  int beg = 0, end = 0;
+  if (valid) { beg = lm_start[l]; end = lm_start[l + 1]; }
+  const int lc = valid ? l : 0;
+  const double* Li = Linv + (size_t)lc * kLmRec;
+  const double Li0 = Li[0], Li1 = Li[1], Li2 = Li[2], Li3 = Li[3], Li4 = Li[4], Li5 = Li[5];
+  const double* zl = z + (size_t)lc * kLmRec;
+  const double zl0 = zl[0], zl1 = zl[1], zl2 = zl[2];
+  if constexpr (Y_LDS) {
+    const int n2 = (n_pose + 1) >> 1;
+    if (n2 <= 512) backsub_stage_y<2>(y_pose, n2); else if (n2 <= 1024) backsub_stage_y<4>(y_pose, n2); else backsub_stage_y<8>(y_pose, n2);
+  }
+  const bool no_cr = COMPACT || CR == nullptr;
+  constexpr int kA = COMPACT ? 6 : 12;
+  const int f0 = beg + sub;
+  const bool h0 = f0 < end, h1 = f0 + 8 < end;
+  const int f0c = h0 ? f0 : 0, f1 = h1 ? f0 + 8 : f0c;
+  double A0[kA], A1[kA], R0[6], R1[6];
+  int2 t0 = fac_t[f0c];
+  pose_row_load<COMPACT>(J, f0c, A0);
+  if (no_cr) row6_load(JB, 6, f0c, R0); else row6_load(CR, 8, f0c, R0);
+  double2 r0 = r[f0c];
+  int2 t1 = t0;
+  double2 r1 = r0;
+  if constexpr (COMPACT) { t1 = fac_t[f1]; pose_row_load<true>(J, f1, A1); row6_load(JB, 6, f1, R1); r1 = r[f1]; pin(A1); pin(R1); pin(r1, t1); }
+  else {
+#pragma unroll
+    for (int k = 0; k < 6; ++k) R1[k] = R0[k];
+  }
+  pin(A0); pin(R0); pin(r0, t0);
+  if constexpr (Y_LDS) __syncthreads();
+  double a0 = 0, a1 = 0, a2 = 0;
+  double jk0[2] = {0.0, 0.0}, jk1[2] = {0.0, 0.0};
+  if (h0) {
+    pose_row_dot<Y_LDS, COMPACT>(A0, R0, t0.x, t0.y, y_pose, jk0[0], jk1[0]);
+    a0 += R0[0] * jk0[0] + R0[3] * jk1[0]; a1 += R0[1] * jk0[0] + R0[4] * jk1[0]; a2 += R0[2] * jk0[0] + R0[5] * jk1[0];
+    if (h1) {
+      if constexpr (!COMPACT) {
+        t1 = fac_t[f1]; pose_row_load<false>(J, f1, A0); r1 = r[f1];
+        if (no_cr) row6_load(JB, 6, f1, R1); else row6_load(CR, 8, f1, R1);
+        pin(A0); pin(r1, t1);
+        pose_row_dot<Y_LDS, false>(A0, R1, t1.x, t1.y, y_pose, jk0[1], jk1[1]);
+      } else pose_row_dot<Y_LDS, true>(A1, R1, t1.x, t1.y, y_pose, jk0[1], jk1[1]);
+      a0 += R1[0] * jk0[1] + R1[3] * jk1[1]; a1 += R1[1] * jk0[1] + R1[4] * jk1[1]; a2 += R1[2] * jk0[1] + R1[5] * jk1[1];
+    }
+  }
+  for (int f = f0 + 16; f < end; f += 8) {
+    double C[6], A[kA];
+    if (no_cr) row6_load(JB, 6, f, C); else row6_load(CR, 8, f, C);
+    const int2 t = fac_t[f];
+    pose_row_load<COMPACT>(J, f, A);
+    double j0, j1;
+    pose_row_dot<Y_LDS, COMPACT>(A, C, t.x, t.y, y_pose, j0, j1);
+    a0 += C[0] * j0 + C[3] * j1; a1 += C[1] * j0 + C[4] * j1; a2 += C[2] * j0 + C[5] * j1;
+  }
+#pragma unroll
+  for (int o = 4; o > 0; o >>= 1) { a0 += __shfl_xor(a0, o, 8); a1 += __shfl_xor(a1, o, 8); a2 += __shfl_xor(a2, o, 8); }
+  if (no_cr) {
+    const double b0 = a0, b1 = a1, b2 = a2;
+    a0 = Li0 * b0; a1 = Li1 * b0 + Li2 * b1; a2 = Li3 * b0 + Li4 * b1 + Li5 * b2;
+  }
+  if (!valid) return;
+  const double w0 = zl0 - a0, w1 = zl1 - a1, w2 = zl2 - a2;
+  const double y0 = Li0 * w0 + Li1 * w1 + Li3 * w2;
+  const double y1 = Li2 * w1 + Li4 * w2;
+  const double y2 = Li5 * w2;
+  if (sub == 0) {
+    const int to = n_pose + 3 * l;
+    delta[to] = -y0; delta[to + 1] = -y1; delta[to + 2] = -y2;
+    if (up.n_blocks > 0) {
+      const int xo = up.lm_xoff[l];
+      const double x0 = up.x[xo], x1 = up.x[xo + 1], x2v = up.x[xo + 2];
+      const double c0 = x0 + (-y0), c1 = x1 + (-y1), c2 = x2v + (-y2);
+      up.x_cand[xo] = c0; up.x_cand[xo + 1] = c1; up.x_cand[xo + 2] = c2;
+      const double e0 = x0 - c0, e1 = x1 - c1, e2 = x2v - c2;
+      upd_d2 = e0 * e0 + e1 * e1 + e2 * e2; upd_x2 = x0 * x0 + x1 * x1 + x2v * x2v;
+    }
+  }
+  if (h0) {
+    if constexpr (!COMPACT) { row6_load(JB, 6, f0, R0); if (h1) row6_load(JB, 6, f1, R1); }
+    const double d0 = -(jk0[0] + R0[0] * y0 + R0[1] * y1 + R0[2] * y2), d1 = -(jk1[0] + R0[3] * y0 + R0[4] * y1 + R0[5] * y2);
+    acc -= d0 * (r0.x + 0.5 * d0) + d1 * (r0.y + 0.5 * d1);
+  }
+  if (h1) {
+    const double d0 = -(jk0[1] + R1[0] * y0 + R1[1] * y1 + R1[2] * y2), d1 = -(jk1[1] + R1[3] * y0 + R1[4] * y1 + R1[5] * y2);
+    acc -= d0 * (r1.x + 0.5 * d0) + d1 * (r1.y + 0.5 * d1);
+  }
+  for (int f = f0 + 16; f < end; f += 8) {
+    double Bf[6], A[kA];
+    row6_load(JB, 6, f, Bf);
+    const int2 t = fac_t[f];
+    pose_row_load<COMPACT>(J, f, A);
+    double j0, j1;
+    pose_row_dot<Y_LDS, COMPACT>(A, Bf, t.x, t.y, y_pose, j0, j1);
+    const double d0 = -(j0 + Bf[0] * y0 + Bf[1] * y1 + Bf[2] * y2), d1 = -(j1 + Bf[3] * y0 + Bf[4] * y1 + Bf[5] * y2);
+    const double2 rf = r[f];
+    acc -= d0 * (rf.x + 0.5 * d0) + d1 * (rf.y + 0.5 * d1);
+  }
+}
+__device__ __forceinline__ void backsub_mcc_kernel_body(const int bsg_bx, const int bsg_gx, int n_lm, int n_lm_groups, int n_elim, int n, const int* __restrict__ lm_start, const double* __restrict__ J, int ja, const double* __restrict__ JB, const double2* __restrict__ r, const double* __restrict__ CR, const int2* __restrict__ fac_t, const double* __restrict__ Linv, const double* __restrict__ z, int n_pose, const double* __restrict__ y_pose, int y_lds, double* __restrict__ delta, double* __restrict__ mcc_part, int n_vis_blocks, const SmallGroupSet& small, int n_small_units, const UpdateRide& up, int first_update_block) {
   __shared__ double sred[4];
   if (up.n_blocks > 0 && bsg_bx >= first_update_block) {
     const int unit = bsg_bx - first_update_block, i = unit * 256 + (int)threadIdx.x;
@@ -546,77 +685,20 @@
   }
   double acc = 0.0, upd_d2 = 0.0, upd_x2 = 0.0;
   if (bsg_bx < n_lm_groups) {
-    const int gid = bsg_bx * 256 + threadIdx.x;
-    const int l = gid >> 3, sub = gid & 7;
-    const bool valid = l < n_lm;
-    int beg = 0, end = 0;
-    if (valid) { beg = lm_start[l]; end = lm_start[l + 1]; }
-    const int lc = valid ? l : 0;
-    const double* Li = Linv + (size_t)lc * kLmRec;
-    const double Li0 = Li[0], Li1 = Li[1], Li2 = Li[2], Li3 = Li[3], Li4 = Li[4], Li5 = Li[5];
-    const double* zl = z + (size_t)lc * kLmRec;
-    const double zl0 = zl[0], zl1 = zl[1], zl2 = zl[2];
-    double a0 = 0, a1 = 0, a2 = 0;
-    double jk0[2] = {0.0, 0.0}, jk1[2] = {0.0, 0.0};
-    int it = 0;
-    const bool no_cr = CR == nullptr;
     const bool compact = ja == kJACompact;
-    for (int f = beg + sub; f < end; f += 8, ++it) {
-      const double2* C2 = no_cr ? reinterpret_cast<const double2*>(JB + (size_t)f * 6) : reinterpret_cast<const double2*>(CR + (size_t)f * 8);
-      const double2 ca = C2[0], cb = C2[1], cc = C2[2];
-      const double C[6] = {ca.x, ca.y, cb.x, cb.y, cc.x, cc.y};
-      const int cp = cam_pose[f];
-      double j0, j1;
-      if (compact) pose_part_compact(J + (size_t)f * kJACompact, C, cp_tq[cp], cp_tp[cp], y_pose, j0, j1);
-      else pose_part(J + (size_t)f * kJAStride, cp_tq[cp], cp_tp[cp], y_pose, j0, j1);
-      if (it == 0) { jk0[0] = j0; jk1[0] = j1; } else if (it == 1) { jk0[1] = j0; jk1[1] = j1; }
-      a0 += C[0] * j0 + C[3] * j1; a1 += C[1] * j0 + C[4] * j1; a2 += C[2] * j0 + C[5] * j1;
-    }
-#pragma unroll
-    for (int o = 4; o > 0; o >>= 1) { a0 += __shfl_xor(a0, o, 8); a1 += __shfl_xor(a1, o, 8); a2 += __shfl_xor(a2, o, 8); }
-    if (no_cr) {
-      const double b0 = a0, b1 = a1, b2 = a2;
-      a0 = Li0 * b0; a1 = Li1 * b0 + Li2 * b1; a2 = Li3 * b0 + Li4 * b1 + Li5 * b2;
-    }
-    if (valid) {
-      const double w0 = zl0 - a0, w1 = zl1 - a1, w2 = zl2 - a2;
-      const double y0 = Li0 * w0 + Li1 * w1 + Li3 * w2;
-      const double y1 = Li2 * w1 + Li4 * w2;
-      const double y2 = Li5 * w2;
-      if (sub == 0) {
-        const int to = n_pose + 3 * l;
-        delta[to] = -y0; delta[to + 1] = -y1; delta[to + 2] = -y2;
-        if (up.n_blocks > 0) {
-          const int xo = up.lm_xoff[l];
-          const double x0 = up.x[xo], x1 = up.x[xo + 1], x2v = up.x[xo + 2];
-          const double c0 = x0 + (-y0), c1 = x1 + (-y1), c2 = x2v + (-y2);
-          up.x_cand[xo] = c0; up.x_cand[xo + 1] = c1; up.x_cand[xo + 2] = c2;
-          const double e0 = x0 - c0, e1 = x1 - c1, e2 = x2v - c2;
-          upd_d2 = e0 * e0 + e1 * e1 + e2 * e2; upd_x2 = x0 * x0 + x1 * x1 + x2v * x2v;
-        }
-      }
-      it = 0;
-      for (int f = beg + sub; f < end; f += 8, ++it) {
-        const double2* B2 = reinterpret_cast<const double2*>(JB + (size_t)f * 6);
-        const double2 ba = B2[0], bb = B2[1], bc = B2[2];
-        const double Bf[6] = {ba.x, ba.y, bb.x, bb.y, bc.x, bc.y};
-        double j0, j1;
-        if (it == 0) { j0 = jk0[0]; j1 = jk1[0]; }
-        else if (it == 1) { j0 = jk0[1]; j1 = jk1[1]; }
-        else if (compact) { const int cp = cam_pose[f]; pose_part_compact(J + (size_t)f * kJACompact, Bf, cp_tq[cp], cp_tp[cp], y_pose, j0, j1); }
-        else { const int cp = cam_pose[f]; pose_part(J + (size_t)f * kJAStride, cp_tq[cp], cp_tp[cp], y_pose, j0, j1); }
-        const double d0 = -(j0 + Bf[0] * y0 + Bf[1] * y1 + Bf[2] * y2), d1 = -(j1 + Bf[3] * y0 + Bf[4] * y1 + Bf[5] * y2);
-        const double2 rf = r[f];
-        acc -= d0 * (rf.x + 0.5 * d0) + d1 * (rf.y + 0.5 * d1);
-      }
-    }
+    if (y_lds && compact) backsub_lm_group<true, true>(bsg_bx, n_lm, lm_start, J, JB, r, CR, fac_t, Linv, z, n_pose, y_pose, delta, up, acc, upd_d2, upd_x2);
+    else if (y_lds) backsub_lm_group<true, false>(bsg_bx, n_lm, lm_start, J, JB, r, CR, fac_t, Linv, z, n_pose, y_pose, delta, up, acc, upd_d2, upd_x2);
+    else if (compact) backsub_lm_group<false, true>(bsg_bx, n_lm, lm_start, J, JB, r, CR, fac_t, Linv, z, n_pose, y_pose, delta, up, acc, upd_d2, upd_x2);
+    else backsub_lm_group<false, false>(bsg_bx, n_lm, lm_start, J, JB, r, CR, fac_t, Linv, z, n_pose, y_pose, delta, up, acc, upd_d2, upd_x2);
   } else {
     const int f = n_elim + (bsg_bx - n_lm_groups) * 256 + (int)threadIdx.x;
     if (f < n) {
-      const int cp = cam_pose[f];
-      double j0, j1;
-      pose_part(J + (size_t)f * kJAStride, cp_tq[cp], cp_tp[cp], y_pose, j0, j1);
+      const int2 t = fac_t[f];
+      double A[12], j0, j1;
+      const double none[6] = {0.0, 0.0, 0.0, 0.0, 0.0, 0.0};
+      pose_row_load<false>(J, f, A);
       const double2 rf = r[f];
+      pose_row_dot<false, false>(A, none, t.x, t.y, y_pose, j0, j1);
       acc = -((-j0) * (rf.x - 0.5 * j0) + (-j1) * (rf.y - 0.5 * j1));
     }
   }
@@ -629,8 +711,8 @@
     if (threadIdx.x == 0) { up.part[2 * slot] = a; up.part[2 * slot + 1] = c; }
   }
 }
-__global__ __launch_bounds__(256) void backsub_mcc_kernel(int n_lm, int n_lm_groups, int n_elim, int n, const int* __restrict__ lm_start, const double* __restrict__ J, int ja, const double* __restrict__ JB, const double2* __restrict__ r, const double* __restrict__ CR, const int* __restrict__ cam_pose, const int* __restrict__ cp_tq, const int* __restrict__ cp_tp, const double* __restrict__ Linv, const double* __restrict__ z, int n_pose, const double* __restrict__ y_pose, double* __restrict__ delta, double* __restrict__ mcc_part, int n_vis_blocks, SmallGroupSet small, int n_small_units, UpdateRide up, int first_update_block) {
-  backsub_mcc_kernel_body((int)blockIdx.x, (int)gridDim.x, n_lm, n_lm_groups, n_elim, n, lm_start, J, ja, JB, r, CR, cam_pose, cp_tq, cp_tp, Linv, z, n_pose, y_pose, delta, mcc_part, n_vis_blocks, small, n_small_units, up, first_update_block);
+__global__ __launch_bounds__(256) __attribute__((amdgpu_waves_per_eu(4, 4))) void backsub_mcc_kernel(int n_lm, int n_lm_groups, int n_elim, int n, const int* __restrict__ lm_start, const double* __restrict__ J, int ja, const double* __restrict__ JB, const double2* __restrict__ r, const double* __restrict__ CR, const int2* __restrict__ fac_t, const double* __restrict__ Linv, const double* __restrict__ z, int n_pose, const double* __restrict__ y_pose, int y_lds, double* __restrict__ delta, double* __restrict__ mcc_part, int n_vis_blocks, SmallGroupSet small, int n_small_units, UpdateRide up, int first_update_block) {
+  backsub_mcc_kernel_body((int)blockIdx.x, (int)gridDim.x, n_lm, n_lm_groups, n_elim, n, lm_start, J, ja, JB, r, CR, fac_t, Linv, z, n_pose, y_pose, y_lds, delta, mcc_part, n_vis_blocks, small, n_small_units, up, first_update_block);
 }
 struct backsub_mcc_kernel_Args {
   int bsg_grid;
@@ -644,9 +726,7 @@
   const double* JB;
   const double2* r;
   const double* CR;
-  const int* cam_pose;
-  const int* cp_tq;
-  const int* cp_tp;
+  const int2* fac_t;
   const double* Linv;
   const double* z;
   int n_pose;
@@ -671,9 +751,7 @@
   const double __attribute__((address_space(1)))* JB;
   const double2 __attribute__((address_space(1)))* r;
   const double __attribute__((address_space(1)))* CR;
-  const int __attribute__((address_space(1)))* cam_pose;
-  const int __attribute__((address_space(1)))* cp_tq;
-  const int __attribute__((address_space(1)))* cp_tp;
+  const int2 __attribute__((address_space(1)))* fac_t;
   const double __attribute__((address_space(1)))* Linv;
   const double __attribute__((address_space(1)))* z;
   int n_pose;
@@ -688,11 +766,11 @@
 };
 static_assert(sizeof(backsub_mcc_kernel_ArgsG) == sizeof(backsub_mcc_kernel_Args), "layout");
 
-__global__ __launch_bounds__(256) void backsub_mcc_kernel_batch(const backsub_mcc_kernel_Args* __restrict__ bsg_A, const BatchDyn* __restrict__ bsg_dyn, int bsg_list) {
+__global__ __launch_bounds__(256) __attribute__((amdgpu_waves_per_eu(4, 4))) void backsub_mcc_kernel_batch(const backsub_mcc_kernel_Args* __restrict__ bsg_A, const BatchDyn* __restrict__ bsg_dyn, int bsg_list, int bsg_y_lds) {
   const int bsg_w = bsg_dyn->idx[bsg_list][blockIdx.y];
   const backsub_mcc_kernel_ArgsG& a = reinterpret_cast<const backsub_mcc_kernel_ArgsG*>(bsg_A)[bsg_w];
   if ((int)blockIdx.x >= a.bsg_grid) return;
-  backsub_mcc_kernel_body((int)blockIdx.x, a.bsg_grid, a.n_lm, a.n_lm_groups, a.n_elim, a.n, (const int*)a.lm_start, (const double*)a.J, a.ja, (const double*)a.JB, (const double2*)a.r, (double*)a.CR, (const int*)a.cam_pose, (const int*)a.cp_tq, (const int*)a.cp_tp, (const double*)a.Linv, (const double*)a.z, a.n_pose, (const double*)a.y_pose, (double*)a.delta, (double*)a.mcc_part, a.n_vis_blocks, a.small, a.n_small_units, a.up, a.first_update_block);
+  backsub_mcc_kernel_body((int)blockIdx.x, a.bsg_grid, a.n_lm, a.n_lm_groups, a.n_elim, a.n, (const int*)a.lm_start, (const double*)a.J, a.ja, (const double*)a.JB, (const double2*)a.r, (double*)a.CR, (const int2*)a.fac_t, (const double*)a.Linv, (const double*)a.z, a.n_pose, (const double*)a.y_pose, bsg_y_lds, (double*)a.delta, (double*)a.mcc_part, a.n_vis_blocks, a.small, a.n_small_units, a.up, a.first_update_block);
 }
 
 void batchargs_landmark(BatchArgTable& t, BatchArgTable& t_tail, const Visual& v, int n_pose, int jacobi, double lm_lo, double lm_hi, double* scale, double* dcl,
@@ -738,19 +816,24 @@
   const int extra = small ? (n_small_units + 1) / 2 : 0;
   const int upd_units = (upd && upd->n_blocks > 0) ? (upd->n_blocks + 255) / 256 : 0;
   a.bsg_grid = grid > 0 ? grid + extra + upd_units : 0;
-  a.n_lm = v.n_lm; a.n_lm_groups = g_lm; a.n_elim = v.n_elim; a.n = v.n; a.lm_start = v.lm_start; a.J = v.J; a.ja = v.ja; a.JB = v.JB; a.r = v.r; a.CR = v.no_cr ? nullptr : v.CR; a.cam_pose = v.cam_pose;
-  a.cp_tq = v.cp_tq; a.cp_tp = v.cp_tp; a.Linv = v.Linv; a.z = v.z; a.n_pose = n_pose; a.y_pose = y_pose; a.delta = delta; a.mcc_part = mcc_part; a.n_vis_blocks = grid;
+  a.n_lm = v.n_lm; a.n_lm_groups = g_lm; a.n_elim = v.n_elim; a.n = v.n; a.lm_start = v.lm_start; a.J = v.J; a.ja = v.ja; a.JB = v.JB; a.r = v.r; a.CR = v.no_cr ? nullptr : v.CR; a.fac_t = v.fac_t;
+  a.Linv = v.Linv; a.z = v.z; a.n_pose = n_pose; a.y_pose = y_pose; a.delta = delta; a.mcc_part = mcc_part; a.n_vis_blocks = grid;
   a.small = small ? *small : SmallGroupSet(); a.n_small_units = small ? n_small_units : 0; a.up = upd_units ? *upd : UpdateRide(); a.first_update_block = grid + extra;
   t.push(a);
+  if (a.bsg_grid > 0 && g_lm > 0) {
+    const size_t lds = backsub_stage_bytes(n_pose);
+    if (lds == 0) t.lds_over = true; else t.lds = std::max(t.lds, lds);
+  }
 }
 void launch_backsub_mcc_batch(hipStream_t s, const BatchArgTable& t, const BatchDyn* dyn, int list, int n) {
   if (n <= 0 || t.max_grid <= 0) return;
-  hipLaunchKernelGGL(backsub_mcc_kernel_batch, dim3(t.max_grid, n), dim3(256), 0, s, static_cast<const backsub_mcc_kernel_Args*>(t.dev), dyn, list);
+  const size_t lds = t.lds_over ? 0 : t.lds;
+  hipLaunchKernelGGL(backsub_mcc_kernel_batch, dim3(t.max_grid, n), dim3(256), lds, s, static_cast<const backsub_mcc_kernel_Args*>(t.dev), dyn, list, lds > 0 ? 1 : 0);
 }
 int backsub_mcc_groups(const Visual& v) { return (v.n_lm * 8 + 255) / 256 + (v.n - v.n_elim + 255) / 256; }
-__global__ __launch_bounds__(256) void backsub_mcc_marg_kernel(int n_lm, int n_lm_groups, int n_elim, int n, const int* __restrict__ lm_start, const double* __restrict__ J, int ja, const double* __restrict__ JB, const double2* __restrict__ r, const double* __restrict__ CR, const int* __restrict__ cam_pose, const int* __restrict__ cp_tq, const int* __restrict__ cp_tp, const double* __restrict__ Linv, const double* __restrict__ z, int n_pose, const double* __restrict__ y_pose, double* __restrict__ delta, double* __restrict__ mcc_part, int n_vis_blocks, SmallGroupSet small, int n_small_units, UpdateRide up, int first_update_block, MargDev m, double* __restrict__ marg_part, int first_marg_block) {
+__global__ __launch_bounds__(256) __attribute__((amdgpu_waves_per_eu(4, 4))) void backsub_mcc_marg_kernel(int n_lm, int n_lm_groups, int n_elim, int n, const int* __restrict__ lm_start, const double* __restrict__ J, int ja, const double* __restrict__ JB, const double2* __restrict__ r, const double* __restrict__ CR, const int2* __restrict__ fac_t, const double* __restrict__ Linv, const double* __restrict__ z, int n_pose, const double* __restrict__ y_pose, int y_lds, double* __restrict__ delta, double* __restrict__ mcc_part, int n_vis_blocks, SmallGroupSet small, int n_small_units, UpdateRide up, int first_update_block, MargDev m, double* __restrict__ marg_part, int first_marg_block) {
   if ((int)blockIdx.x >= first_marg_block) { marg_mcc_kernel_body(4 * ((int)blockIdx.x - first_marg_block), m, delta, marg_part); return; }
-  backsub_mcc_kernel_body((int)blockIdx.x, first_marg_block, n_lm, n_lm_groups, n_elim, n, lm_start, J, ja, JB, r, CR, cam_pose, cp_tq, cp_tp, Linv, z, n_pose, y_pose, delta, mcc_part, n_vis_blocks, small, n_small_units, up, first_update_block);
+  backsub_mcc_kernel_body((int)blockIdx.x, first_marg_block, n_lm, n_lm_groups, n_elim, n, lm_start, J, ja, JB, r, CR, fac_t, Linv, z, n_pose, y_pose, y_lds, delta, mcc_part, n_vis_blocks, small, n_small_units, up, first_update_block);
 }
 bool launch_backsub_mcc(hipStream_t s, const Visual& v, int n_pose, const double* y_pose, double* delta, double* mcc_part,
                         const SmallGroupSet* small, int n_small_units, const UpdateRide* upd, const MargDev* marg, double* marg_part) {
@@ -758,17 +841,28 @@
   if (grid == 0) return false;
   const int extra = small ? (n_small_units + 1) / 2 : 0;
   const int upd_units = (upd && upd->n_blocks > 0) ? (upd->n_blocks + 255) / 256 : 0;
+  const size_t lds = g_lm > 0 ? backsub_stage_bytes(n_pose) : 0;
   if (marg && marg_part && marg->rows > 0) {
     const int own = grid + extra + upd_units;
-    hipLaunchKernelGGL(backsub_mcc_marg_kernel, dim3(own + (marg->rows + 3) / 4), dim3(256), 0, s, v.n_lm, g_lm, v.n_elim, v.n, v.lm_start, v.J, v.ja, v.JB, v.r, v.no_cr ? nullptr : v.CR, v.cam_pose,
-                       v.cp_tq, v.cp_tp, v.Linv, v.z, n_pose, y_pose, delta, mcc_part, grid, small ? *small : SmallGroupSet(), small ? n_small_units : 0,
+    hipLaunchKernelGGL(backsub_mcc_marg_kernel, dim3(own + (marg->rows + 3) / 4), dim3(256), lds, s, v.n_lm, g_lm, v.n_elim, v.n, v.lm_start, v.J, v.ja, v.JB, v.r, v.no_cr ? nullptr : v.CR, v.fac_t,
+                       v.Linv, v.z, n_pose, y_pose, lds > 0 ? 1 : 0, delta, mcc_part, grid, small ? *small : SmallGroupSet(), small ? n_small_units : 0,
                        upd_units ? *upd : UpdateRide(), grid + extra, *marg, marg_part, own);
     return true;
   }
-  hipLaunchKernelGGL(backsub_mcc_kernel, dim3(grid + extra + upd_units), dim3(256), 0, s, v.n_lm, g_lm, v.n_elim, v.n, v.lm_start, v.J, v.ja, v.JB, v.r, v.no_cr ? nullptr : v.CR, v.cam_pose,
-                     v.cp_tq, v.cp_tp, v.Linv, v.z, n_pose, y_pose, delta, mcc_part, grid, small ? *small : SmallGroupSet(), small ? n_small_units : 0,
+  hipLaunchKernelGGL(backsub_mcc_kernel, dim3(grid + extra + upd_units), dim3(256), lds, s, v.n_lm, g_lm, v.n_elim, v.n, v.lm_start, v.J, v.ja, v.JB, v.r, v.no_cr ? nullptr : v.CR, v.fac_t,
+                     v.Linv, v.z, n_pose, y_pose, lds > 0 ? 1 : 0, delta, mcc_part, grid, small ? *small : SmallGroupSet(), small ? n_small_units : 0,
                      upd_units ? *upd : UpdateRide(), grid + extra);
   return false;
 }
 
-}
+__global__ void fac_t_kernel(int n, const int* __restrict__ cam_pose, const int* __restrict__ cp_tq, const int* __restrict__ cp_tp, int2* __restrict__ fac_t) {
+  const int f = blockIdx.x * 256 + threadIdx.x;
+  if (f >= n) return;
+  const int cp = cam_pose[f];
+  fac_t[f] = make_int2(cp_tq[cp], cp_tp[cp]);
+}
+void launch_fac_t(hipStream_t s, const Visual& v) {
+  if (v.n > 0) hipLaunchKernelGGL(fac_t_kernel, dim3((v.n + 255) / 256), dim3(256), 0, s, v.n, v.cam_pose, v.cp_tq, v.cp_tp, v.fac_t);
+}
+
+}
diff --git a/beam_slam_amd/gpu.py b/beam_slam_amd/gpu.py
--- a/beam_slam_amd/gpu.py
+++ b/beam_slam_amd/gpu.py
@@ -141,6 +141,14 @@
         fn.argtypes = [ctypes.c_void_p, ctypes.c_void_p]
         self._chk(fn(self._ctx, out.ctypes.data))
         return out
+
+    def backsub_tangent_table(self, n):
+        import numpy as np
+        ft, jn = np.full((n, 2), -2, np.int32), np.full((n, 2), -2, np.int32)
+        fn = lib().bsgpu_backsub_tangent_table
+        fn.argtypes = [ctypes.c_void_p, ctypes.c_void_p, ctypes.c_void_p]
+        self._chk(fn(self._ctx, ft.ctypes.data, jn.ctypes.data))
+        return ft, jn
 
     def triangulate(self, track_start, q_block, p_block, pixels, camera=0, truncate_pixels=True, max_dist=-1.0, max_reproj=-1.0):
         import numpy as np
diff --git a/include/bsgpu.h b/include/bsgpu.h
--- a/include/bsgpu.h
+++ b/include/bsgpu.h
@@ -198,6 +198,8 @@
 
 int bsgpu_reprojection_errors(bsgpu_ctx* ctx, double* err);
 
+int bsgpu_backsub_tangent_table(bsgpu_ctx* ctx, int32_t* fac_t, int32_t* joined);
+
 int bsgpu_preintegrate(int device, int32_t n_intervals, const int32_t* sample_start, const double* t, const double* w,
                        const double* a, const double* t_end, const double* bg, const double* ba, const double* cov_w,
                        const double* cov_a, const double* cov_bg, const double* cov_ba, double info_weight,
```

After: 3830 LM iterations/s (median of 6 runs). 1.02x the previous value.
